# NicoNeureiter/sBayes

Hardware: AMD Instinct MI355X
Metric: log-likelihood evals/sec at 1000 sites x 200 feats x 10 states; 1/2/4/8-GPU chains (higher is better)
Workload: dtype f64; 1 GPU; headline synthetic 1000x200x10, K=5, C=2 (BASELINE.json configs[2]); chains_per_gpu=4096, kernel=packed, log_mode=product, parallelism=1 independent engine(s), one per GPU, no collectives

## Files before the change

### sbayes_amd/csrc/sbe_engine_internal.hip.h

```cpp
#pragma once
#include "sbe_kernels.hip.h"
#include "sbe_unit.hip.h"
#include "../../include/sbe_engine.h"
#include "../../include/sbe_engine_steps.h"
#include "../../include/sbe_engine_diag.h"
#include "sbe_host_helpers.h"
#include "sbe_pool.h"

#include <sched.h>
#include <algorithm>
#include <cstdarg>
#include <cstdio>
#include <cstring>
#include <chrono>
#include <atomic>
#include <condition_variable>
#include <functional>
#include <mutex>
#include <string>
#include <thread>
#include <vector>

using namespace sbe;

inline thread_local std::string g_last_error;

namespace {

struct Slot {
    std::vector<uint16_t> h_gid;
    std::vector<uint8_t> h_pid;
    std::vector<uint32_t> patterns;
    int n_tuples = 0;
    std::vector<uint8_t> h_tid;
    std::vector<uint32_t> h_toff;
    std::vector<uint16_t> h_tuple_g;
    std::vector<uint8_t> h_tuple_p;
    bool share_ok = false;
    bool groups_set = false, weights_set = false, source_set = false;
    std::vector<uint8_t> probs_set, counts_set;
    bool patterns_dirty = true;
    uint32_t gid_pending = 0;
    bool tables_follow = false;
    std::vector<int32_t> pat_cnt;
    std::vector<int32_t> tup_cnt;
    bool inc_ok = false;
    uint64_t group_epoch = 0;
    uint32_t overlap_mask = 0;
    int32_t ov_obj = -1, ov_g1 = 0, ov_g2 = 0, ov_comp = 0;
};

}

static int fuse_tables_default() {
    static const int on = [] { const char* v = getenv("SBE_FUSE_TABLES"); return (v && atoi(v) == 0) ? 0 : 1; }();
    return on;
}

struct sbe_engine : sbe::MixShape {
    int device = 0;
    hipStream_t stream = nullptr;
    hipEvent_t ev0 = nullptr, ev1 = nullptr;
    std::vector<hipEvent_t> ev_pool;
    bool ev_timing = false;  int ev_used = 0;
    int Fp = 0, rs_pitch = 0;
    uint64_t rng_seed = 0, rng_draw = 0;
    std::vector<int> G, goff;
    int64_t n_na = 0;
    int64_t hbm_bytes = 0;
    std::string last_error;
    char device_name[64] = {0};
    char last_kernel[128] = "none";

    sbe::MixTuning tune;
    int opt_log = SBE_LOG_PRODUCT;
    int opt_fuse_tables = fuse_tables_default();
    bool ws_lds_allowed[2] = {false, false};

    uint8_t* d_onehot = nullptr;
    uint8_t* d_state = nullptr;
    uint8_t* d_state_q = nullptr;
    float* d_probs_t = nullptr;
    double* d_wpat_t = nullptr;
    uint16_t* d_gid = nullptr;
    uint8_t* d_pid = nullptr;
    uint8_t* d_src = nullptr;
    int32_t* d_counts = nullptr;
    float* d_probs = nullptr;
    float* d_weights = nullptr;
    float* d_wpat = nullptr;
    uint32_t* d_patbits = nullptr;
    uint16_t* d_state_h = nullptr;
    double2* d_logtab = nullptr;
    uint32_t* d_toff = nullptr;
    uint32_t* d_rowoff = nullptr;
    std::vector<uint64_t> rowoff_epoch;
    uint32_t* d_rowoff_s = nullptr;  int rs_nq_max = 0;
    int32_t* d_rs_nq = nullptr;
    uint8_t* d_state_s = nullptr;
    std::vector<uint64_t> rowsort_epoch;
    std::atomic<uint64_t> epoch_counter{0};
    double2* d_logtab_fine = nullptr;
    unsigned* d_arrive = nullptr;
    uint8_t* d_xt = nullptr;
    int xt_NT = 0, xt_KBp = 0;  size_t xt_bytes = 0;
    uint8_t* d_tid = nullptr;
    uint16_t* d_tuple_g = nullptr;
    uint8_t* d_tuple_p = nullptr;
    double* d_conc = nullptr;
    double* d_unif = nullptr;
    double* d_lg_conc = nullptr; double* d_sum_a = nullptr; double* d_lg_sum_a = nullptr;
    double* d_unif_res = nullptr;  bool unif_set = false;
    int32_t* d_comp_of_group = nullptr;
    std::vector<uint8_t> conc_set;
    double* d_partials = nullptr;
    double* d_results = nullptr;
    double* h_results = nullptr;
    int* d_status = nullptr;
    int* h_status = nullptr;
    int* h_flag = nullptr;  int* d_flag = nullptr;
    unsigned long long* h_done = nullptr;  unsigned long long* d_done = nullptr;
    unsigned* d_ticket = nullptr;  unsigned long long done_seq = 0;
    static constexpr int kMaxChunks = 16;
    unsigned long long* h_chunk_flags = nullptr;  unsigned long long* d_chunk_flags = nullptr;
    unsigned* d_chunk_tickets = nullptr;  unsigned long long chunk_seq = 0;
    uint8_t* h_stream = nullptr;  uint8_t* d_stream = nullptr;  size_t stream_bytes = 0;
    uint8_t* d_changed = nullptr;
    uint32_t* d_step_stamp = nullptr;  uint32_t step_id = 0;
    float* d_step_pf = nullptr;
    double* d_step_pg = nullptr;
    struct StepLayout { size_t ids, pid, tid, toff, tuple_g, tuple_p, patbits, weights, row_of, subset, stale, objects, rows, total; } sl{};
    int step_max_rows = 0;
    uint8_t* h_step_payload = nullptr; uint8_t* d_step_payload = nullptr;
    uint8_t* h_io = nullptr; uint8_t* d_io = nullptr; size_t io_bytes = 0;
    uint8_t* h_step = nullptr;     uint8_t* d_step_host = nullptr;
    struct Lane { uint8_t* h_payload; uint8_t* d_payload; uint8_t* h_step; uint8_t* d_step_host; float* d_pf;
                  uint32_t* d_stamp; uint32_t step_id;
                  int* d_status; };
    std::vector<Lane> lanes;
    uint8_t* d_batch_meta = nullptr; size_t batch_meta_bytes = 0;
    uint8_t* h_batch_payload = nullptr; uint8_t* d_batch_payload = nullptr; size_t batch_payload_bytes = 0;
    std::vector<Slot> batch_cands;
    std::vector<std::vector<int32_t>> batch_moved;
    std::vector<int32_t> step_moved;
    struct Pool;
    Pool* pool = nullptr;
    uint8_t* d_scratch = nullptr;  size_t scratch_bytes = 0;
    uint8_t* h_pinned = nullptr;   size_t pinned_bytes = 0;
    uint8_t* h_arena = nullptr;    uint8_t* d_arena = nullptr;   size_t arena_bytes = 0, arena_off = 0;
    SetterJobs* batch = nullptr;
    int opt_step_form = 0;
    int opt_step_derive = 0;
    int opt_deferred = 0;
    bool status_pending = false;
    const char* pending_origin[2] = {nullptr, nullptr};
    int pending_calls = 0;
    std::vector<Slot> slots;
    struct SrcSync { uint64_t version = 1; int peer = -1; uint64_t peer_version = 0, own_version = 0; std::vector<int32_t> diff; };
    std::vector<SrcSync> src_sync;
    std::vector<SrcSync> ids_sync;

    int64_t probs_t_elems() const { return (int64_t)n_ftiles * tile_tab_elems(); }
    int64_t wpat_tile_elems() const { return (int64_t)Pmax * C * ft; }
    int64_t wpat_t_elems() const { return (int64_t)n_ftiles * wpat_tile_elems(); }
};

namespace {
inline void bump_src(sbe_engine* e, int slot) { ++e->src_sync[slot].version; }
inline void bump_ids(sbe_engine* e, int slot) { ++e->ids_sync[slot].version; }
}

struct sbe_engine::Pool : sbe_host::StepPool { using sbe_host::StepPool::StepPool; };

namespace {

int fail(sbe_engine* e, int code, const char* fmt, ...) {
    char buf[512];
    va_list ap;
    va_start(ap, fmt);
    vsnprintf(buf, sizeof buf, fmt, ap);
    va_end(ap);
    g_last_error = buf;
    if (e) e->last_error = buf;
    return code;
}

#define CHECK_ENGINE(e) \
    if (!(e)) return fail(nullptr, SBE_ERR_ARG, "null engine handle")
#define CHECK_SLOT(e, s) \
    if ((s) < 0 || (s) >= (e)->n_slots) return fail(e, SBE_ERR_ARG, "slot %d out of range [0,%d)", (s), (e)->n_slots)
#define CHECK_COMP(e, c) \
    if ((c) < 0 || (c) >= (e)->C) return fail(e, SBE_ERR_ARG, "component %d out of range [0,%d)", (c), (e)->C)
#define CHECK_PTR(e, p) \
    if (!(p)) return fail(e, SBE_ERR_ARG, "null pointer argument: %s", #p)

inline int round_up(int a, int b) { return (a + b - 1) / b * b; }

template <class T>
int dmalloc(sbe_engine* e, T** p, int64_t n) {
    const size_t bytes = std::max<int64_t>(n, 1) * sizeof(T);
    HIPCHK(e, hipMalloc((void**)p, bytes));
    e->hbm_bytes += (int64_t)bytes;
    return SBE_OK;
}

inline size_t al256(size_t v) { return (v + 255) / 256 * 256; }

int ensure_scratch(sbe_engine* e, size_t bytes) {
    if (bytes <= e->scratch_bytes) return SBE_OK;
    if (e->d_scratch) { HIPCHK(e, hipStreamSynchronize(e->stream)); HIPCHK(e, hipFree(e->d_scratch)); }
    e->scratch_bytes = bytes + bytes / 4 + 4096;
    HIPCHK(e, hipMalloc((void**)&e->d_scratch, e->scratch_bytes));
    return SBE_OK;
}

int ensure_io(sbe_engine* e, size_t bytes) {
    if (bytes <= e->io_bytes) return SBE_OK;
    if (e->h_io) { HIPCHK(e, hipStreamSynchronize(e->stream)); HIPCHK(e, hipHostFree(e->h_io)); e->h_io = nullptr; e->io_bytes = 0; }
    const size_t want = bytes + bytes / 4 + 4096;
    HIPCHK(e, hipHostMalloc((void**)&e->h_io, want, hipHostMallocMapped));
    HIPCHK(e, hipHostGetDevicePointer((void**)&e->d_io, e->h_io, 0));
    e->io_bytes = want;
    return SBE_OK;
}

int ensure_pinned(sbe_engine* e, size_t bytes) {
    if (bytes <= e->pinned_bytes) return SBE_OK;
    if (e->h_pinned) { HIPCHK(e, hipStreamSynchronize(e->stream)); HIPCHK(e, hipHostFree(e->h_pinned)); }
    e->pinned_bytes = bytes + bytes / 4 + 4096;
    HIPCHK(e, hipHostMalloc((void**)&e->h_pinned, e->pinned_bytes, hipHostMallocDefault));
    return SBE_OK;
}

int upload(sbe_engine* e, void* dst_dev, const void* src, size_t bytes);
int synced(sbe_engine* e);

int ensure_step_pool(sbe_engine* e);

int ensure_stream(sbe_engine* e, size_t bytes) {
    if (bytes <= e->stream_bytes) return SBE_OK;
    if (e->h_stream) { HIPCHK(e, hipStreamSynchronize(e->stream)); HIPCHK(e, hipHostFree(e->h_stream)); e->h_stream = nullptr; e->stream_bytes = 0; }
    const size_t want = bytes + bytes / 4 + 4096;
    HIPCHK(e, hipHostMalloc((void**)&e->h_stream, want, hipHostMallocMapped));
    HIPCHK(e, hipHostGetDevicePointer((void**)&e->d_stream, e->h_stream, 0));
    e->stream_bytes = want;
    return SBE_OK;
}

struct StreamPlan { ChunkSig sig; int n_chunks; size_t chunk_bytes; size_t bytes; unsigned grid; };

StreamPlan plan_stream(sbe_engine* e, unsigned n_blocks, size_t bytes_per_block, size_t bytes) {
    static const int max_chunks = [] { const char* v = getenv("SBE_STREAM_CHUNKS"); const int n = v ? atoi(v) : 0;
                                       return n >= 1 && n <= sbe_engine::kMaxChunks ? n : 8; }();
    unsigned per = std::max<unsigned>(1, (unsigned)div_up((int64_t)n_blocks, max_chunks));
    per = std::max<unsigned>(per, (unsigned)div_up((int64_t)128 << 10, (int64_t)bytes_per_block));
    const int n_chunks = (int)div_up((int64_t)n_blocks, (int64_t)per);
    static const bool ordered = [] { const char* v = getenv("SBE_STREAM_ORDERED"); return !(v && atoi(v) == 0); }();
    ChunkSig sig{e->d_chunk_tickets, e->d_chunk_flags, ++e->chunk_seq, per, n_blocks, (unsigned)n_chunks, 0};
    unsigned grid = n_blocks;
    if (ordered && n_chunks > 1) {
        sig.chunk_elems = (long long)per * (long long)(bytes_per_block / sizeof(double));
        grid = per;
    }
    return StreamPlan{sig, n_chunks, (size_t)per * bytes_per_block, bytes, grid};
}

template <class JobBegin, class JobEnd, class Work>
int stream_result(sbe_engine* e, const StreamPlan& plan, int n_jobs, JobBegin job_begin, JobEnd job_end, Work work) {
    static const bool single_thread = [] { const char* v = getenv("SBE_D2H_THREADS"); return v && atoi(v) == 1; }();
    if (!single_thread) { int rc = ensure_step_pool(e); if (rc) return rc; }
    std::atomic<bool> all_landed{false};
    hipError_t sync_err = hipSuccess;
    const volatile unsigned long long* flags = e->h_chunk_flags;
    const unsigned long long seq = plan.sig.seq;
    const size_t chunk_bytes = plan.chunk_bytes;
    const auto t_limit = std::chrono::steady_clock::now() + std::chrono::microseconds(2000 + (int64_t)(plan.bytes / 10000));
    unsigned spins = 0;
    sbe_host::run_as_chunks_land(
        single_thread ? nullptr : e->pool, n_jobs,
        [=](int j) { return (int)(job_begin(j) / chunk_bytes); },
        [=](int j) { return (int)((job_end(j) - 1) / chunk_bytes); },
        [&, flags, seq](int k) { return flags[k] == seq || all_landed.load(std::memory_order_acquire); },
        [&] {
            if ((++spins & 1023u) == 0 && !all_landed.load(std::memory_order_relaxed) && std::chrono::steady_clock::now() > t_limit) {
                sync_err = hipStreamSynchronize(e->stream);
                all_landed.store(true, std::memory_order_release);
            }
        },
        work);
    if (sync_err != hipSuccess) return fail(e, SBE_ERR_HIP, "hipStreamSynchronize (streamed result): %s", hipGetErrorString(sync_err));
    return SBE_OK;
}

int d2h(sbe_engine* e, void* dst, const void* src_dev, size_t bytes) {
    int rc = ensure_pinned(e, bytes);
    if (rc) return rc;
    HIPCHK(e, hipMemcpyAsync(e->h_pinned, src_dev, bytes, hipMemcpyDeviceToHost, e->stream));
    HIPCHK(e, hipStreamSynchronize(e->stream));
    static const bool single_copy = [] { const char* v = getenv("SBE_D2H_THREADS"); return v && atoi(v) == 1; }();
    if (bytes >= ((size_t)1 << 20) && !single_copy) {
        rc = ensure_step_pool(e);
        if (rc) return rc;
        constexpr size_t kJob = (size_t)64 << 10;
        uint8_t* out = (uint8_t*)dst;
        const uint8_t* stage = e->h_pinned;
        e->pool->run((int)((bytes + kJob - 1) / kJob),
                     [=](int j) { const size_t o = (size_t)j * kJob; memcpy(out + o, stage + o, std::min(kJob, bytes - o)); });
        return synced(e);
    }
    memcpy(dst, e->h_pinned, bytes);
    return synced(e);
}

constexpr size_t kMappedOutMax = (size_t)1 << 18;
int out_target(sbe_engine* e, size_t bytes, void* dev_fallback, void** target) {
    *target = dev_fallback;
    if (bytes > kMappedOutMax) return SBE_OK;
    int rc = ensure_io(e, bytes);
    if (rc) return rc;
    *target = e->d_io;
    return SBE_OK;
}
int wait_done(sbe_engine* e, const DoneSig& d);
DoneSig next_done(sbe_engine* e, unsigned n_blocks);
DoneSig out_done(sbe_engine* e, const void* target, unsigned n_blocks) {
    return target == (const void*)e->d_io ? next_done(e, n_blocks) : DoneSig{};
}
int out_fetch(sbe_engine* e, void* host_out, const void* target, size_t bytes, const DoneSig& done = DoneSig{}) {
    if (target != (const void*)e->d_io) return d2h(e, host_out, target, bytes);
    int rc = wait_done(e, done);
    if (rc) return rc;
    memcpy(host_out, e->h_io, bytes);
    return synced(e);
}

int h2d(sbe_engine* e, void* dst_dev, const void* src, size_t bytes) { return upload(e, dst_dev, src, bytes); }

int upload(sbe_engine* e, void* dst_dev, const void* src, size_t bytes) {
    if (bytes == 0) return SBE_OK;
    if (e->h_arena && bytes <= e->arena_bytes / 4) {
        const size_t need = (bytes + 63) / 64 * 64;
        if (e->arena_off + need > e->arena_bytes) {
            HIPCHK(e, hipStreamSynchronize(e->stream));
            e->arena_off = 0;
        }
        uint8_t* stage = e->h_arena + e->arena_off;
        e->arena_off += need;
        memcpy(stage, src, bytes);
        HIPCHK(e, hipMemcpyAsync(dst_dev, stage, bytes, hipMemcpyHostToDevice, e->stream));
        return SBE_OK;
    }
    HIPCHK(e, hipMemcpyAsync(dst_dev, src, bytes, hipMemcpyHostToDevice, e->stream));
    HIPCHK(e, hipStreamSynchronize(e->stream));
    return SBE_OK;
}

int stage(sbe_engine* e, const void* src, size_t bytes, void* dev_fallback, const void** out) {
    constexpr size_t kDirect = (size_t)64 << 10;
    *out = dev_fallback;
    if (bytes == 0) return SBE_OK;
    if (!e->d_arena || bytes > kDirect) return upload(e, dev_fallback, src, bytes);
    const size_t need = (bytes + 63) / 64 * 64;
    if (e->arena_off + need > e->arena_bytes) {
        HIPCHK(e, hipStreamSynchronize(e->stream));
        e->arena_off = 0;
    }
    memcpy(e->h_arena + e->arena_off, src, bytes);
    *out = e->d_arena + e->arena_off;
    e->arena_off += need;
    return SBE_OK;
}

struct UploadSeg { void* dst; const void* src; size_t bytes; };
struct FusedWeightPatterns { WeightPatternArgs args; int bits_seg; const float* new_weights; bool done; };
int upload_segments(sbe_engine* e, const UploadSeg* segs, int n, FusedWeightPatterns* wp = nullptr) {
    size_t total = 0, largest = 0;
    for (int i = 0; i < n; ++i) { total += (segs[i].bytes + 63) / 64 * 64; largest = std::max(largest, segs[i].bytes); }
    if (wp) wp->done = false;
    if (total == 0) return SBE_OK;
    if (!e->d_arena || n > 8 || total > ((size_t)64 << 10)) {
        for (int i = 0; i < n; ++i) { int rc = upload(e, segs[i].dst, segs[i].src, segs[i].bytes); if (rc) return rc; }
        return SBE_OK;
    }
    const size_t w_bytes = wp && wp->new_weights ? (size_t)wp->args.F * wp->args.C * sizeof(float) : 0;
    const bool fuse = wp && segs[wp->bits_seg].bytes > 0 && w_bytes <= ((size_t)64 << 10);
    const size_t reserve = total + (fuse ? (w_bytes + 63) / 64 * 64 : 0);
    if (e->arena_off + reserve > e->arena_bytes) {
        HIPCHK(e, hipStreamSynchronize(e->stream));
        e->arena_off = 0;
    }
    ScatterSegs sg{};
    size_t off = 0;
    for (int i = 0; i < n; ++i) {
        if (segs[i].bytes == 0) continue;
        memcpy(e->h_arena + e->arena_off + off, segs[i].src, segs[i].bytes);
        sg.dst[sg.n] = (uint8_t*)segs[i].dst; sg.off[sg.n] = (uint32_t)off; sg.bytes[sg.n] = (uint32_t)segs[i].bytes;
        ++sg.n;
        if (fuse && i == wp->bits_seg) wp->args.pattern_bits = (const uint32_t*)(e->d_arena + e->arena_off + off);
        off += (segs[i].bytes + 63) / 64 * 64;
    }
    const unsigned sx = (unsigned)std::min<size_t>(div_up((int64_t)largest, 1024), 16);
    unsigned wx = 0;
    if (fuse) {
        if (w_bytes) {
            memcpy(e->h_arena + e->arena_off + off, wp->new_weights, w_bytes);
            wp->args.weights = (const float*)(e->d_arena + e->arena_off + off);
        }
        wx = (unsigned)div_up((int64_t)wp->args.P * wp->args.F, 256);
        wp->done = true;
    }
    if (e->batch && e->batch->n_group_blocks == 0 && (fuse || !wp)) {
        SetterJobs& j = *e->batch;
        j.group_base = e->d_arena + e->arena_off; j.sg = sg; j.has_wp = fuse ? 1 : 0;
        if (fuse) j.wp = wp->args;
        j.group_gx = std::max(sx, wx); j.n_group_blocks = j.group_gx * (unsigned)(sg.n + (fuse ? 1 : 0));
    } else if (fuse) {
        k_scatter_weight_patterns<<<dim3(std::max(sx, wx), sg.n + 1), 256, 0, e->stream>>>(e->d_arena + e->arena_off, sg, wp->args);
    } else {
        k_scatter_bytes<<<dim3(sx, sg.n), 256, 0, e->stream>>>(e->d_arena + e->arena_off, sg);
    }
    HIPCHK(e, hipGetLastError());
    e->arena_off += reserve;
    return SBE_OK;
}

bool poll_done_enabled() {
    static const bool on = [] { const char* v = getenv("SBE_POLL_DONE"); return !(v && atoi(v) == 0); }();
    return on;
}
DoneSig next_done(sbe_engine* e, unsigned n_blocks) {
    if (!poll_done_enabled()) return DoneSig{};
    return DoneSig{e->d_ticket, e->d_done, ++e->done_seq, n_blocks};
}
int wait_done(sbe_engine* e, const DoneSig& d) {
    if (d.flag) {
        const volatile unsigned long long* f = e->h_done;
        const auto t0 = std::chrono::steady_clock::now();
        for (unsigned spins = 1;; ++spins) {
            if (*f == d.seq) { std::atomic_thread_fence(std::memory_order_acquire); return SBE_OK; }
            if ((spins & 127u) == 0u) sched_yield(); else __builtin_ia32_pause();
            if ((spins & 255u) == 0 && std::chrono::steady_clock::now() - t0 > std::chrono::microseconds(300)) break;
        }
    }
    HIPCHK(e, hipStreamSynchronize(e->stream));
    return SBE_OK;
}

bool status_raised(const sbe_engine* e) {
    const volatile int* f = e->h_flag;
    return (f[ST_BAD_NORMALIZE] | f[ST_MULTI_SOURCE]) != 0;
}

int fetch_and_clear_status(sbe_engine* e) {
    HIPCHK(e, hipMemcpyAsync(e->h_status, e->d_status, ST_FLAG_PTR * sizeof(int), hipMemcpyDeviceToHost, e->stream));
    HIPCHK(e, hipMemsetAsync(e->d_status + ST_BAD_NORMALIZE, 0, 2 * sizeof(int), e->stream));
    HIPCHK(e, hipStreamSynchronize(e->stream));
    e->h_flag[ST_BAD_NORMALIZE] = e->h_flag[ST_MULTI_SOURCE] = 0;
    return SBE_OK;
}

int report_status(sbe_engine* e, bool deferred = false) {
    const int n_calls = e->pending_calls;
    const char* origin[2] = {e->pending_origin[0], e->pending_origin[1]};
    e->pending_calls = 0;
    e->pending_origin[0] = e->pending_origin[1] = nullptr;
    if (!status_raised(e)) return SBE_OK;
    int rc = fetch_and_clear_status(e);
    if (rc) return rc;
    const int bad_norm = e->h_status[ST_BAD_NORMALIZE], multi_src = e->h_status[ST_MULTI_SOURCE];
    e->h_status[ST_BAD_NORMALIZE] = e->h_status[ST_MULTI_SOURCE] = 0;
    char where[200] = "";
    const char* who = origin[bad_norm ? 0 : 1];
    if (deferred && who)
        snprintf(where, sizeof where, " [deferred data check: raised by %s (%d state-setting call%s queued since the last report), "
                 "reported by the first call that waited for the device]", who, n_calls, n_calls == 1 ? "" : "s");
    if (bad_norm)
        return fail(e, SBE_ERR_DATA, "normalize: %d rows have a non-positive sum (sbayes/util.py:1006 assert)%s", bad_norm, where);
    return fail(e, SBE_ERR_DATA, "source is not one-hot over components in %d observations%s", multi_src, where);
}

int check_after(sbe_engine* e, int word, const char* who = __builtin_FUNCTION()) {
    if (e->opt_deferred) {
        e->status_pending = true;
        e->pending_origin[word == ST_BAD_NORMALIZE ? 0 : 1] = who;
        ++e->pending_calls;
        return SBE_OK;
    }
    HIPCHK(e, hipStreamSynchronize(e->stream));
    e->status_pending = false;
    return report_status(e);
}

int synced(sbe_engine* e) {
    if (!e->status_pending) return SBE_OK;
    e->status_pending = false;
    return report_status(e, true);
}

int read_status(sbe_engine* e) {
    HIPCHK(e, hipStreamSynchronize(e->stream));
    int rc = synced(e);
    if (rc) return rc;
    e->h_status[ST_BAD_NORMALIZE] = e->h_status[ST_MULTI_SOURCE] = 0;
    if (status_raised(e)) return fetch_and_clear_status(e);
    return SBE_OK;
}

int take_status(sbe_engine* e) {
    e->h_status[ST_BAD_NORMALIZE] = e->h_status[ST_MULTI_SOURCE] = 0;
    if (status_raised(e)) return fetch_and_clear_status(e);
    return SBE_OK;
}

int clear_status_word(sbe_engine* e, int word) {
    if (e->status_pending) return SBE_OK;
    if (!e->h_flag[word]) return SBE_OK;
    HIPCHK(e, hipStreamSynchronize(e->stream));
    HIPCHK(e, hipMemsetAsync(e->d_status + word, 0, sizeof(int), e->stream));
    e->h_flag[word] = 0;
    return SBE_OK;
}

void derive_patterns(sbe_engine* e, Slot& s) {
    const int N = e->N, C = e->C;
    static thread_local std::vector<uint8_t> bits;
    bits.resize(N);
    bool seen[256] = {false};
    s.pat_cnt.assign(256, 0);
    for (int n = 0; n < N; ++n) {
        uint32_t b = 0;
        for (int c = 0; c < C; ++c)
            if (s.h_gid[(size_t)c * N + n] != kNoGroup) b |= 1u << c;
        bits[n] = (uint8_t)b;
        seen[b] = true;
        ++s.pat_cnt[b];
    }
    auto key = [C](uint32_t b) {
        uint32_t k = 0;
        for (int c = 0; c < C; ++c) k |= ((b >> c) & 1u) << (C - 1 - c);
        return k;
    };
    std::vector<uint32_t> uniq;
    for (uint32_t b = 0; b < 256; ++b) if (seen[b]) uniq.push_back(b);
    std::sort(uniq.begin(), uniq.end(), [&](uint32_t a, uint32_t b) { return key(a) < key(b); });
    uint8_t index_of[256] = {0};
    for (size_t i = 0; i < uniq.size(); ++i) index_of[uniq[i]] = (uint8_t)i;
    s.patterns = uniq;
    s.h_pid.resize(N);
    for (int n = 0; n < N; ++n) s.h_pid[n] = index_of[bits[n]];
}

bool tuples_share_operands(const sbe_engine* e, const Slot& s) {
    if (e->C != 2 || s.n_tuples == 0 || (int)s.h_tuple_p.size() != kMaxTuples) return false;
    int first = -1, pb = -1;
    for (int t = 0; t < kMaxTuples; ++t) {
        const int pat = s.h_tuple_p[t];
        if (pat == 0xFF) continue;
        if (first < 0) { first = t; continue; }
        if (s.h_tuple_g[(size_t)t * kMaxComponents + 1] != s.h_tuple_g[(size_t)first * kMaxComponents + 1]) return false;
        const int pa = s.h_tuple_p[first];
        if (pat != pa) {
            if (pb < 0) pb = pat;
            else if (pat != pb) return false;
        }
    }
    return first >= 0;
}

void derive_tuples(sbe_engine* e, Slot& s) {
    const int N = e->N, C = e->C;
    s.h_tid.assign(e->Np, 0);
    s.h_toff.assign(e->Np, 0);
    s.h_tuple_g.assign((size_t)kMaxTuples * kMaxComponents, (uint16_t)e->Gtot);
    s.h_tuple_p.assign(kMaxTuples, 0xFF);
    uint16_t tuples[kMaxTuples][kMaxComponents];
    int n_tup = 0;
    bool ok = true;
    s.tup_cnt.assign(kMaxTuples, 0);
    uint64_t packed[kMaxTuples];
    int last = 0;
    for (int n = 0; n < N && ok; ++n) {
        uint16_t key[kMaxComponents];
        for (int c = 0; c < C; ++c) key[c] = s.h_gid[(size_t)c * N + n];
        int t = 0;
        if (C <= 4) {
            uint64_t k64 = 0;
            for (int c = 0; c < C; ++c) k64 |= (uint64_t)key[c] << (16 * c);
            if (n_tup && packed[last] == k64) t = last;
            else for (; t < n_tup; ++t) if (packed[t] == k64) break;
            if (t == n_tup && n_tup < kMaxTuples) packed[n_tup] = k64;
        } else {
            for (; t < n_tup; ++t) if (memcmp(tuples[t], key, (size_t)C * sizeof(uint16_t)) == 0) break;
        }
        last = t;
        if (t == n_tup) {
            if (n_tup == kMaxTuples) { ok = false; break; }
            memcpy(tuples[n_tup++], key, (size_t)C * sizeof(uint16_t));
            for (int c = 0; c < C; ++c) s.h_tuple_g[(size_t)t * kMaxComponents + c] = key[c] == kNoGroup ? (uint16_t)e->Gtot : key[c];
            s.h_tuple_p[t] = s.h_pid[n];
        }
        s.h_tid[n] = (uint8_t)t;
        s.h_toff[n] = (uint32_t)t * (uint32_t)(e->S + 1) * 512u;
        ++s.tup_cnt[t];
    }
    s.n_tuples = ok ? n_tup : 0;
    s.inc_ok = ok;
    s.share_ok = tuples_share_operands(e, s);
}

bool update_patterns_and_tuples(sbe_engine* e, Slot& s, const int32_t* moved, const uint16_t* old_gid0, int n_moved) {
    const int N = e->N, C = e->C;
    if (!s.inc_ok || s.n_tuples == 0 || (int)s.pat_cnt.size() != 256 || (int)s.tup_cnt.size() != kMaxTuples) return false;
    auto bits_rest = [&](int n) { uint32_t b = 0; for (int c = 1; c < C; ++c) if (s.h_gid[(size_t)c * N + n] != kNoGroup) b |= 1u << c; return b; };
    for (int i = 0; i < n_moved; ++i) {
        const int n = moved[i];
        const uint32_t rest = bits_rest(n);
        const uint32_t b0 = rest | (old_gid0[i] != kNoGroup ? 1u : 0u), b1 = rest | (s.h_gid[n] != kNoGroup ? 1u : 0u);
        if (b0 == b1) continue;
        --s.pat_cnt[b0]; ++s.pat_cnt[b1];
    }
    {
        size_t live = 0;
        for (uint32_t b = 0; b < 256; ++b) if (s.pat_cnt[b] > 0) ++live;
        bool same = live == s.patterns.size();
        for (size_t i = 0; same && i < s.patterns.size(); ++i) same = s.pat_cnt[s.patterns[i]] > 0;
        if (!same) return false;
    }
    uint8_t rank_of[256];
    for (size_t i = 0; i < s.patterns.size(); ++i) rank_of[s.patterns[i]] = (uint8_t)i;
    for (int i = 0; i < n_moved; ++i) {
        const int n = moved[i];
        const uint32_t b1 = bits_rest(n) | (s.h_gid[n] != kNoGroup ? 1u : 0u);
        s.h_pid[n] = rank_of[b1];
        uint16_t key[kMaxComponents];
        for (int c = 0; c < C; ++c) { const uint16_t g = s.h_gid[(size_t)c * N + n]; key[c] = g == kNoGroup ? (uint16_t)e->Gtot : g; }
        const int t0 = s.h_tid[n];
        int t1 = -1, free_t = -1;
        for (int t = 0; t < s.n_tuples; ++t) {
            if (s.tup_cnt[t] == 0) { if (free_t < 0 && t != t0) free_t = t; continue; }
            if (memcmp(&s.h_tuple_g[(size_t)t * kMaxComponents], key, (size_t)C * sizeof(uint16_t)) == 0) { t1 = t; break; }
        }
        if (t1 < 0) {
            if (s.tup_cnt[t0] == 1) t1 = t0;
            else if (free_t >= 0) t1 = free_t;
            else if (s.n_tuples < kMaxTuples) t1 = s.n_tuples++;
            else return false;
            for (int c = 0; c < C; ++c) s.h_tuple_g[(size_t)t1 * kMaxComponents + c] = key[c];
        }
        if (t1 != t0) {
            if (--s.tup_cnt[t0] == 0) s.h_tuple_p[t0] = 0xFF;
            ++s.tup_cnt[t1];
        }
        s.h_tuple_p[t1] = s.h_pid[n];
        s.h_tid[n] = (uint8_t)t1;
        s.h_toff[n] = (uint32_t)t1 * (uint32_t)(e->S + 1) * 512u;
    }
    while (s.n_tuples > 0 && s.tup_cnt[s.n_tuples - 1] == 0) --s.n_tuples;
    s.share_ok = tuples_share_operands(e, s);
    for (int t = 0; t < s.n_tuples; ++t)
        if (s.tup_cnt[t] == 0) return false;
    return s.n_tuples > 0;
}

int upload_patterns_and_weights(sbe_engine* e, int slot, const float* new_weights = nullptr, bool eager = false) {
    Slot& s = e->slots[slot];
    float* d_w = e->d_weights + (int64_t)slot * e->F * e->C;
    auto gid_seg = [&](int c) { return UploadSeg{e->d_gid + ((int64_t)slot * e->C + c) * e->Np, s.h_gid.data() + (size_t)c * e->N, (size_t)e->N * sizeof(uint16_t)}; };
    bool patterns_done = false;
    if (s.patterns_dirty) {
        const bool follow = s.tables_follow;
        s.tables_follow = false;
        if (!follow) derive_patterns(e, s);
        if ((int)s.patterns.size() > e->Pmax) {
            if (eager) {
                for (int c = 0; c < e->C; ++c)
                    if (s.gid_pending >> c & 1u) { const UploadSeg g = gid_seg(c); int rc = upload(e, g.dst, g.src, g.bytes); if (rc) return rc; }
                s.gid_pending = 0;
                return SBE_OK;
            }
            return fail(e, SBE_ERR_ARG, "%zu distinct has_components patterns exceed capacity %d",
                        s.patterns.size(), e->Pmax);
        }
        if (!follow) derive_tuples(e, s);
        UploadSeg segs[6 + kMaxComponents] = {{e->d_pid + (int64_t)slot * e->Np, s.h_pid.data(), (size_t)e->N},
                                              {e->d_patbits + (int64_t)slot * e->Pmax, s.patterns.data(), s.patterns.size() * sizeof(uint32_t)}};
        int n_segs = 2;
        if (s.n_tuples) {
            segs[n_segs++] = {e->d_tid + (int64_t)slot * e->Np, s.h_tid.data(), (size_t)e->Np};
            segs[n_segs++] = {e->d_toff + (int64_t)slot * e->Np, s.h_toff.data(), (size_t)e->Np * sizeof(uint32_t)};
            segs[n_segs++] = {e->d_tuple_g + (int64_t)slot * kMaxTuples * kMaxComponents, s.h_tuple_g.data(), s.h_tuple_g.size() * sizeof(uint16_t)};
            segs[n_segs++] = {e->d_tuple_p + (int64_t)slot * kMaxTuples, s.h_tuple_p.data(), s.h_tuple_p.size()};
        }
        for (int c = 0; c < e->C; ++c) if (s.gid_pending >> c & 1u) segs[n_segs++] = gid_seg(c);
        const int P = (int)s.patterns.size();
        FusedWeightPatterns wp{};
        const bool want_wp = (s.weights_set || new_weights) && P > 0;
        if (want_wp) {
            wp.args = WeightPatternArgs{d_w, nullptr, e->d_wpat + (int64_t)slot * e->Pmax * e->F * e->C, new_weights ? d_w : nullptr,
                                        e->d_wpat_t + (int64_t)slot * e->wpat_t_elems(), P, e->F, e->C, e->Pmax, e->ft};
            wp.bits_seg = 1;
            wp.new_weights = new_weights;
        }
        { int _urc = upload_segments(e, segs, n_segs, want_wp ? &wp : nullptr); if (_urc) return _urc; }
        patterns_done = wp.done;
        s.patterns_dirty = false;
        s.gid_pending = 0;
    }
    const int P = (int)s.patterns.size();
    if (new_weights && P == 0) {
        int rc = upload(e, d_w, new_weights, (size_t)e->F * e->C * sizeof(float));
        if (rc) return rc;
    }
    if ((s.weights_set || new_weights) && P > 0 && !patterns_done) {
        const void* w_in = d_w;
        if (new_weights) { int rc = stage(e, new_weights, (size_t)e->F * e->C * sizeof(float), d_w, &w_in); if (rc) return rc; }
        k_weight_patterns<<<div_up((int64_t)P * e->F, 256), 256, 0, e->stream>>>(
            (const float*)w_in, e->d_patbits + (int64_t)slot * e->Pmax, e->d_wpat + (int64_t)slot * e->Pmax * e->F * e->C, P, e->F, e->C,
            w_in != d_w ? d_w : nullptr, e->d_wpat_t + (int64_t)slot * e->wpat_t_elems(), e->Pmax, e->ft);
        HIPCHK(e, hipGetLastError());
    }
    return SBE_OK;
}

int retile_probs(sbe_engine* e, int slot, int component) {
    const int g_lo = e->goff[component], g_hi = g_lo + e->G[component];
    const int64_t n = (int64_t)(g_hi - g_lo) * e->S * e->ft * e->n_ftiles;
    if (n == 0) return SBE_OK;
    k_tile_probs<<<div_up(n, 256), 256, 0, e->stream>>>(
        e->d_probs + (int64_t)slot * e->table_elems(), e->d_probs_t + (int64_t)slot * e->probs_t_elems(),
        g_lo, g_hi, e->Gtot, e->F, e->S, e->ft, e->n_ftiles);
    HIPCHK(e, hipGetLastError());
    return SBE_OK;
}

int check_slot_ready(sbe_engine* e, int slot, bool need_weights) {
    Slot& s = e->slots[slot];
    if (!s.groups_set) return fail(e, SBE_ERR_STATE, "slot %d: groups not set for every component", slot);
    for (int c = 0; c < e->C; ++c)
        if (!s.probs_set[c]) return fail(e, SBE_ERR_STATE, "slot %d: probability tables of component %d not set", slot, c);
    if (need_weights && !s.weights_set) return fail(e, SBE_ERR_STATE, "slot %d: weights not set", slot);
    return SBE_OK;
}

int check_collapsed_ready(sbe_engine* e, int slot, int c_lo, int c_hi) {
    Slot& s = e->slots[slot];
    for (int c = c_lo; c < c_hi; ++c) {
        if (e->G[c] == 0) continue;
        if (!s.counts_set[c]) return fail(e, SBE_ERR_STATE, "slot %d: counts of component %d not set", slot, c);
        if (!e->conc_set[c]) return fail(e, SBE_ERR_STATE, "concentration of component %d not set", c);
    }
    return SBE_OK;
}

constexpr size_t kCollapsedLdsMax = (size_t)96 << 10;
inline size_t collapsed_lds_bytes(const sbe_engine* e) { return (size_t)e->F * e->S * sizeof(double) + (size_t)e->F * sizeof(float); }

template <class TC>
int enqueue_dcl(sbe_engine* e, const TC* counts, const double* conc, int conc_per_group, int g_lo, int G, float* d_pf, double* d_pg) {
    k_dcl<TC><<<div_up((int64_t)G * e->F, 256), 256, 0, e->stream>>>(counts, conc, d_pf, g_lo, g_lo + G, e->F, e->S, conc_per_group);
    HIPCHK(e, hipGetLastError());
    if (!d_pg) return SBE_OK;
    k_group_sum_f32<<<div_up((int64_t)G * 8, 64), 64, 0, e->stream>>>(d_pf, d_pg, G, e->F);
    HIPCHK(e, hipGetLastError());
    return SBE_OK;
}

int ensure_xt(sbe_engine* e) {
    if (e->d_xt) return SBE_OK;
    const int NT = div_up((int64_t)e->F * e->S, 32), KBp = round_up(div_up(e->N, kTupleMfmaKBlockObjects), 4);
    const size_t bytes = ((size_t)(NT + 1) * KBp + 4) * 1024;
    uint8_t* xt = nullptr;
    double2* logtab = nullptr;
    auto build = [&]() -> int {
        HIPCHK(e, hipMalloc((void**)&xt, bytes));
        HIPCHK(e, hipMemsetAsync(xt, 0, bytes, e->stream));
        std::vector<double> tab(2 * kFineLogEntries);
        fine_log_table(tab.data());
        HIPCHK(e, hipMalloc((void**)&logtab, tab.size() * sizeof(double) + column_tables_bytes(NT)));
        HIPCHK(e, hipMemcpy(logtab, tab.data(), tab.size() * sizeof(double), hipMemcpyHostToDevice));
        launch_column_tables(e->d_state, reinterpret_cast<int32_t*>(logtab + kFineLogEntries), e->N, e->F, e->S, e->Fp, NT, e->stream);
        HIPCHK(e, hipGetLastError());
        launch_xt_frags(e->d_state, xt, e->N, e->F, e->S, e->Fp, NT, KBp, e->stream);
        HIPCHK(e, hipGetLastError());
        return SBE_OK;
    };
    const int rc = build();
    if (rc) {
        (void)hipStreamSynchronize(e->stream);
        if (xt) (void)hipFree(xt);
        if (logtab) (void)hipFree(logtab);
        return rc;
    }
    e->d_xt = xt; e->d_logtab_fine = logtab;
    e->hbm_bytes += (int64_t)bytes;
    e->xt_NT = NT; e->xt_KBp = KBp; e->xt_bytes = bytes;
    return SBE_OK;
}

int next_timing_events(sbe_engine* e, hipEvent_t* ev_a, hipEvent_t* ev_b) {
    *ev_a = *ev_b = nullptr;
    if (!e->ev_timing) return SBE_OK;
    while ((int)e->ev_pool.size() < 2 * (e->ev_used + 1)) {
        hipEvent_t ev;
        HIPCHK(e, hipEventCreate(&ev));
        e->ev_pool.push_back(ev);
    }
    *ev_a = e->ev_pool[2 * e->ev_used]; *ev_b = e->ev_pool[2 * e->ev_used + 1];
    ++e->ev_used;
    return SBE_OK;
}

struct MixCall {
    int first_slot = 0, n = 1;
    const int32_t* slots = nullptr;  const int32_t* d_slots = nullptr;
    const StepFinish* fin = nullptr;
    const StepFinish* d_fins = nullptr;
    DoneSig* done_out = nullptr;
    hipEvent_t ev_a = nullptr, ev_b = nullptr;
    int slot_at(int i) const { return slots ? (int)slots[i] : first_slot + i; }
};

MixFacts mixture_facts(const sbe_engine* e, const MixCall& c) {
    MixFacts f;
    f.n = c.n;
    f.share_ok = true;
    bool tuples = true;
    for (int i = 0; i < c.n; ++i) {
        const Slot& s = e->slots[c.slot_at(i)];
        f.P = std::max<int>(f.P, (int)s.patterns.size());
        f.KT = std::max(f.KT, s.n_tuples);
        tuples &= s.n_tuples != 0;
        f.share_ok &= s.share_ok;
    }
    if (!tuples) f.KT = 0;
    f.epilogue = c.fin || c.d_fins;
    f.waits = c.done_out != nullptr;
    return f;
}

MixTuning launch_tuning(const sbe_engine* e, const MixFacts& f) {
    MixTuning t = e->tune;
    if (considers_tuple_mfma(*e, t, f))
        if (const char* env = getenv("SBE_MFMA_SPLIT")) t.mfma_split = atoi(env);
    t.shared_allowed = tuple_mfma_shared();
    static const bool in_kernel_opt = !(getenv("SBE_REDUCE_IN_KERNEL") && atoi(getenv("SBE_REDUCE_IN_KERNEL")) == 0);
    t.in_kernel_allowed = in_kernel_opt;
    return t;
}

int prepare_mixture(sbe_engine* e, const MixPlan& pl, const MixCall& c) {
    if (pl.form == MixForm::TupleMfma) return ensure_xt(e);
    if (pl.form != MixForm::Rows && pl.form != MixForm::RowsSorted) return SBE_OK;
    const bool sorted = pl.form == MixForm::RowsSorted;
    const int rft = pl.ft;
    if (sorted && !e->d_rowoff_s) {
        e->rs_nq_max = pl.rs_nq_max;
        int rc = dmalloc(e, &e->d_rowoff_s, (int64_t)e->n_slots * e->rs_nq_max * (e->C + 1) * 4); if (rc) return rc;
        rc = dmalloc(e, &e->d_rs_nq, e->n_slots); if (rc) return rc;
        rc = dmalloc(e, &e->d_state_s, (int64_t)(e->N + 1) * e->Fq); if (rc) return rc;
        launch_state_s(e->d_state, e->d_state_s, e->N, e->F, e->Fp, e->Fq, e->S, e->stream);
        HIPCHK(e, hipGetLastError());
        e->rowsort_epoch.assign(e->n_slots, ~0ull);
    }
    std::vector<uint64_t>& built = sorted ? e->rowsort_epoch : e->rowoff_epoch;
    bool stale = false;
    for (int i = 0; i < c.n; ++i) stale |= built[c.slot_at(i)] != e->slots[c.slot_at(i)].group_epoch;
    if (!stale) return SBE_OK;
    if (sorted) {
        launch_rowsort(e->d_gid, e->d_pid, e->d_rowoff_s, e->d_rs_nq, (int64_t)e->C * e->Np, e->Np,
                       (int64_t)e->rs_nq_max * (e->C + 1) * 4, c.first_slot, c.d_slots, c.n, e->N, e->Np, e->C, e->Gtot, e->Pmax,
                       (uint32_t)((e->S + 1) * rft * 4), (uint32_t)e->Fq, 4 * (kWave / rft), e->stream);
    } else {
        const int cells = (e->C + 1) * e->Np;
        k_rowoff<<<dim3(div_up(cells, 256), c.n), 256, 0, e->stream>>>(
            e->d_gid, e->d_pid, e->d_rowoff, (int64_t)e->C * e->Np, e->Np, (int64_t)cells, c.first_slot, c.d_slots, e->N, e->Np,
            e->C, e->Gtot, (uint32_t)((e->S + 1) * rft * 4), (uint32_t)(((e->C + 1) / 2) * rft * 16));
    }
    HIPCHK(e, hipGetLastError());
    for (int i = 0; i < c.n; ++i) built[c.slot_at(i)] = e->slots[c.slot_at(i)].group_epoch;
    return SBE_OK;
}

int launch_mfma_form(sbe_engine* e, const MixCall& c, const MixPlan& pl, const DoneSig& done) {
    MfmaMixParams p{};
    p.F = e->F; p.S = e->S; p.FS = e->F * e->S; p.Gtot = e->Gtot; p.Np = e->Np;
    p.NT = e->xt_NT; p.KBp = e->xt_KBp; p.KT = pl.KT; p.SL = pl.SL; p.shared = pl.shared ? 1 : 0;
    p.n_batch = c.n; p.n_split = pl.n_split; p.nt_per_split = pl.nt_per_split;
    p.first_slot = c.first_slot; p.slot_list = c.d_slots;
    p.xt = e->d_xt; p.xt_bytes = (uint32_t)e->xt_bytes;
    p.tid = e->d_tid; p.tid_stride = e->Np;
    p.tuple_g = e->d_tuple_g; p.tuple_g_stride = (int64_t)kMaxTuples * kMaxComponents;
    p.tuple_p = e->d_tuple_p; p.tuple_p_stride = kMaxTuples;
    p.probs = e->d_probs; p.probs_stride = e->table_elems();
    p.probs_ones_off = (uint32_t)((int64_t)e->n_slots * e->table_elems() * 4);
    p.probs_bytes = p.probs_ones_off + (uint32_t)(e->F * e->S * 4);
    p.wpat = e->d_wpat; p.wpat_stride = (int64_t)e->Pmax * e->F * e->C;
    p.wpat_ones_off = (uint32_t)((int64_t)e->n_slots * e->Pmax * e->F * e->C * 4);
    p.wpat_bytes = p.wpat_ones_off + (uint32_t)(e->F * e->C * 4);
    p.logtab = e->d_logtab_fine;
    p.colcount = reinterpret_cast<const int32_t*>(e->d_logtab_fine + kFineLogEntries);
    p.colfeat = p.colcount + (size_t)(e->xt_NT + 1) * 32;
    p.tile_prefix = p.colcount + (size_t)(e->xt_NT + 1) * 64;
    p.partials = e->d_partials; p.partials_stride = e->partials_stride;
    if (pl.in_kernel) { p.results = e->d_results; p.arrive = e->d_arrive; p.done = done; }
    if (!launch_tuple_mfma(e->C, p, dim3(pl.grid_x), pl.lds_bytes, e->stream))
        return fail(e, SBE_ERR_STATE, "k_mixture_tuple_mfma was built with static LDS: its log table must sit at LDS address 0 "
                                      "(toolchain change; rebuild without static __shared__ in sbe_mixture_mfma.hip)");
    return SBE_OK;
}

void launch_tile_form(sbe_engine* e, const MixCall& c, const MixPlan& pl, const DoneSig& done) {
    Mix2Params p{};
    p.N = e->N; p.NQ = e->NQ; p.Np = e->Np; p.F = e->F; p.Fq = e->Fq; p.S = e->S; p.C = e->C;
    p.Gtot = e->Gtot; p.P = pl.P; p.n_ftiles = pl.n_ftiles; p.quads_per_chunk = pl.quads_per_chunk;
    p.state_q = reinterpret_cast<const uint32_t*>(e->d_state_q);
    p.onehot = e->d_onehot; p.rs_pitch = e->rs_pitch;
    p.gid = e->d_gid; p.gid_stride = (int64_t)e->C * e->Np;
    p.pid = e->d_pid; p.pid_stride = e->Np;
    p.probs_t = e->d_probs_t; p.probs_t_stride = e->probs_t_elems();
    p.wpat_t = e->d_wpat_t; p.wpat_t_stride = e->wpat_t_elems(); p.wpat_tile_stride = (int)e->wpat_tile_elems();
    p.partials = e->d_partials; p.partials_stride = e->partials_stride; p.first_slot = c.first_slot;
    if (pl.in_kernel) { p.results = e->d_results; p.arrive = e->d_arrive; p.done = done; }
    p.slot_list = c.d_slots;
    p.n_work = pl.n_partials; p.n_batch = c.n;
    p.slot_groups = pl.slot_groups; p.slots_per_group = pl.slots_per_group;
    p.tid = e->d_tid; p.tid_stride = e->Np;
    p.state_h = reinterpret_cast<const uint2*>(e->d_state_h);
    p.toff = e->d_toff; p.toff_stride = e->Np;
    p.logtab = e->d_logtab;
    p.ragged_w = pl.ragged_w; p.gen_slots = pl.gen_slots;
    p.tuple_g = e->d_tuple_g; p.tuple_g_stride = (int64_t)kMaxTuples * kMaxComponents;
    p.tuple_p = e->d_tuple_p; p.tuple_p_stride = kMaxTuples;
    p.combo_w_off = pl.combo_w_off; p.combo_tab_off = pl.combo_tab_off;
    p.KT = pl.KT;
    p.eft = e->ft;
    p.wpat = e->d_wpat; p.wpat_stride = (int64_t)e->Pmax * e->F * e->C;
    p.rowoff = e->d_rowoff; p.rowoff_stride = (int64_t)(e->C + 1) * e->Np;
    p.rowoff_s = e->d_rowoff_s; p.rowoff_s_stride = (int64_t)e->rs_nq_max * (e->C + 1) * 4;
    p.rs_nq = e->d_rs_nq; p.state_s = e->d_state_s; p.state_s_pitch = e->Fq;
    {
        constexpr int split[4] = {450, 270, 170, 110};
        p.rows_cum[0] = 0;
        for (int i = 0; i < 4; ++i) p.rows_cum[i + 1] = p.rows_cum[i] + split[i];
    }
    const int mode = e->opt_log == SBE_LOG_PRODUCT ? LOG_PRODUCT : LOG_PER_OBS;
    const dim3 grid(pl.grid_x, 1);
    switch (pl.form) {
        case MixForm::Tuple64: launch_tuple64(e->C, p, grid, pl.lds_bytes, e->stream); break;
        case MixForm::Combo: launch_combo(pl.onehot, pl.ft, e->C, p, grid, pl.lds_bytes, e->stream); break;
        case MixForm::Rows: case MixForm::RowsSorted:
            launch_rows(mode, pl.ft, e->C, p, grid, pl.lds_bytes, e->stream, pl.form == MixForm::RowsSorted); break;
        case MixForm::OnehotV2: launch_oh2(mode, pl.ft, e->C, p, grid, pl.lds_bytes, e->stream, e->direct); break;
        default: launch_v2(mode, pl.ft, e->C, p, grid, pl.lds_bytes, e->stream, e->direct); break;
    }
}

int launch_mixture(sbe_engine* e, const MixCall& c) {
    const MixFacts facts = mixture_facts(e, c);
    const MixPlan pl = plan_mixture(*e, launch_tuning(e, facts), facts);
    if (pl.err) return fail(e, pl.err, "%s", pl.msg);
    int rc = prepare_mixture(e, pl, c);
    if (rc) return rc;
    if (c.ev_a) HIPCHK(e, hipEventRecord(c.ev_a, e->stream));
    DoneSig done_k{};
    if (pl.in_kernel && c.done_out) *c.done_out = done_k = next_done(e, pl.done_blocks);
    plan_name(pl, *e, e->last_kernel, sizeof e->last_kernel);
    if (pl.form == MixForm::TupleMfma) { rc = launch_mfma_form(e, c, pl, done_k); if (rc) return rc; }
    else launch_tile_form(e, c, pl, done_k);
    if (c.ev_b) HIPCHK(e, hipEventRecord(c.ev_b, e->stream));
    HIPCHK(e, hipGetLastError());
    if (pl.in_kernel) return SBE_OK;
    const unsigned n_red = (unsigned)(c.n + (c.d_fins ? c.n : (c.fin ? 1 : 0)));
    const DoneSig done = c.done_out ? next_done(e, n_red) : DoneSig{};
    if (c.done_out) *c.done_out = done;
    k_reduce_partials<<<n_red, kBlock, 0, e->stream>>>(e->d_partials, e->partials_stride, pl.n_partials,
                                                       e->d_results, c.first_slot, c.n, c.fin ? *c.fin : StepFinish{},
                                                       c.d_slots, c.d_fins, done);
    HIPCHK(e, hipGetLastError());
    return SBE_OK;
}

int enqueue_mixture(sbe_engine* e, int first_slot, int n, DoneSig* done_out = nullptr) {
    for (int s = first_slot; s < first_slot + n; ++s) {
        int rc = check_slot_ready(e, s, true);
        if (rc) return rc;
        if (e->slots[s].patterns_dirty) { rc = upload_patterns_and_weights(e, s); if (rc) return rc; }
    }
    MixCall c;
    c.first_slot = first_slot; c.n = n; c.done_out = done_out;
    { int rc = next_timing_events(e, &c.ev_a, &c.ev_b); if (rc) return rc; }
    return launch_mixture(e, c);
}

int counts_launch(sbe_engine* e, int slot_a, int sign_a, int slot_b, int sign_b, const int32_t* d_objects,
                  int n_listed, int dst_slot, bool single_chunk, uint8_t* d_changed) {
    CountSide A{e->d_gid + (int64_t)slot_a * e->C * e->Np, e->d_src + (int64_t)slot_a * e->N * e->Fp, sign_a};
    CountSide B{e->d_gid + (int64_t)slot_b * e->C * e->Np, e->d_src + (int64_t)slot_b * e->N * e->Fp, sign_b};
    int32_t* counts = e->d_counts + (int64_t)dst_slot * e->table_elems();
    int ft = 32;
    auto lds_for = [&](int t) { return (size_t)e->Gtot * t * e->S * sizeof(int32_t); };
    while (ft > 4 && lds_for(ft) > 96 * 1024) ft >>= 1;
    if (lds_for(ft) > 150 * 1024) {
        k_counts_global<<<div_up((int64_t)n_listed * e->F, 256), 256, 0, e->stream>>>(
            e->d_state, A, B, d_objects, n_listed, e->Np, e->F, e->S, e->C, e->Fp, counts, d_changed);
        HIPCHK(e, hipGetLastError());
        return SBE_OK;
    }
    const int n_ftiles = div_up(e->F, ft);
    int chunks = 1;
    if (!single_chunk) chunks = std::max(1, std::min(div_up(n_listed, 32), div_up(2 * e->compute_units, n_ftiles)));
    const int opc = div_up(n_listed, chunks);
    chunks = div_up(n_listed, opc);
    k_counts<<<dim3(n_ftiles, chunks), kBlock, lds_for(ft), e->stream>>>(
        e->d_state, A, B, d_objects, n_listed, opc, e->Np, e->F, e->S, e->C, e->Fp, e->Gtot, ft, counts, d_changed);
    HIPCHK(e, hipGetLastError());
    return SBE_OK;
}

}

namespace {

int set_gid_common(sbe_engine* e, int slot, int component, const std::vector<uint16_t>& ids) {
    Slot& s = e->slots[slot];
    s.tables_follow = false;
    static const bool follow_on = [] { const char* v = getenv("SBE_FOLLOW_TABLES"); return !(v && atoi(v) == 0); }();
    if (follow_on && component == 0 && !s.patterns_dirty && s.inc_ok) {
        static thread_local std::vector<int32_t> moved;
        static thread_local std::vector<uint16_t> old_ids;
        moved.clear(); old_ids.clear();
        const int N = e->N;
        for (int n = 0; n < N; ++n)
            if (ids[n] != s.h_gid[n]) { moved.push_back(n); old_ids.push_back(s.h_gid[n]); }
        std::copy(ids.begin(), ids.end(), s.h_gid.begin());
        s.tables_follow = (int)moved.size() * 8 <= N &&
                          update_patterns_and_tuples(e, s, moved.data(), old_ids.data(), (int)moved.size());
    } else {
        std::copy(ids.begin(), ids.end(), s.h_gid.begin() + (size_t)component * e->N);
    }
    s.gid_pending |= 1u << component;
    s.patterns_dirty = true;
    s.group_epoch = ++e->epoch_counter;
    bump_ids(e, slot);
    s.groups_set = true;
    return upload_patterns_and_weights(e, slot, nullptr, true);
}

void overlap_message(char* buf, size_t len, int n, int g1, int g2, int component) {
    snprintf(buf, len, "object %d is in groups %d and %d of component %d: resident slot state keeps one group id per object "
             "and component (counts.py:28-30 would count it in both); counts of overlapping groups come from the caller or "
             "the stateless sbe_effect_counts", n, g1, g2, component);
}

struct OverlapNote { bool found = false; int obj = -1, g1 = 0, g2 = 0; };

bool matrix_to_ids(const uint8_t* groups, int G, int N, int off, int component, uint16_t* ids, char* msg, size_t msg_len,
                   OverlapNote* note = nullptr) {
    std::fill(ids, ids + N, kNoGroup);
    auto hit = [&](int n, int g) -> bool {
        if (ids[n] != kNoGroup) {
            if (!note) { overlap_message(msg, msg_len, n, (int)ids[n] - off, g, component); return false; }
            if (!note->found) { note->found = true; note->obj = n; note->g1 = (int)ids[n] - off; note->g2 = g; }
        }
        ids[n] = (uint16_t)(off + g);
        return true;
    };
    for (int g = 0; g < G; ++g) {
        const uint8_t* row = groups + (size_t)g * N;
        int n = 0;
        for (; n + 8 <= N; n += 8) {
            uint64_t w8;
            memcpy(&w8, row + n, 8);
            if (!w8) continue;
            for (int k = 0; k < 8; ++k) if (row[n + k] && !hit(n + k, g)) return false;
        }
        for (; n < N; ++n) if (row[n] && !hit(n, g)) return false;
    }
    return true;
}

int reject_overlap(sbe_engine* e, int slot, const char* what) {
    const Slot& s = e->slots[slot];
    if (!s.overlap_mask) return SBE_OK;
    char msg[320];
    overlap_message(msg, sizeof msg, s.ov_obj, s.ov_g1, s.ov_g2, s.ov_comp);
    return fail(e, SBE_ERR_DATA, "%s (slot %d, %s)", msg, slot, what);
}


int enqueue_lh_exact(sbe_engine* e, int slot, const char* who) {
    Slot& s = e->slots[slot];
    if (!s.groups_set || !s.source_set || !s.weights_set) return fail(e, SBE_ERR_STATE, "slot %d: groups / source / weights not set", slot);
    { int orc = reject_overlap(e, slot, who); if (orc) return orc; }
    for (int c = 0; c < e->C; ++c)
        if (!s.counts_set[c] || !e->conc_set[c]) return fail(e, SBE_ERR_STATE, "slot %d: counts / concentration of component %d not set", slot, c);
    HIPCHK(e, hipSetDevice(e->device));
    int rc = SBE_OK;
    if (s.patterns_dirty) { rc = upload_patterns_and_weights(e, slot); if (rc) return rc; }
    const int64_t n = (int64_t)e->N * e->F;
    rc = ensure_scratch(e, n * sizeof(double));
    if (rc) return rc;
    rc = clear_status_word(e, ST_BAD_NORMALIZE);
    if (rc) return rc;
    k_lh_exact<<<div_up(n, 256), 256, 0, e->stream>>>(
        e->d_state, e->d_src + (int64_t)slot * e->N * e->Fp, e->d_gid + (int64_t)slot * e->C * e->Np,
        e->d_counts + (int64_t)slot * e->table_elems(), e->d_conc, (double*)e->d_scratch, e->N, e->Np, e->F, e->S, e->C,
        e->Fp, e->d_status, e->d_wpat + (int64_t)slot * e->Pmax * e->F * e->C, e->d_pid + (int64_t)slot * e->Np);
    HIPCHK(e, hipGetLastError());
    return SBE_OK;
}

int lh_exact_report(sbe_engine* e) {
    int rc = read_status(e);
    if (rc) return rc;
    if (e->h_status[ST_BAD_NORMALIZE]) return fail(e, SBE_ERR_DATA, "normalize: non-positive row sum in leave-one-out tables (sbayes/util.py:1006 assert)");
    return SBE_OK;
}

int sync_and_report(sbe_engine* e, const DoneSig& done = DoneSig{}) {
    { int rc = wait_done(e, done); if (rc) return rc; }
    const bool was_pending = e->status_pending;
    e->status_pending = false;
    return report_status(e, was_pending);
}

int check_objects(sbe_engine* e, const int32_t* objects, int n) {
    for (int i = 0; i < n; ++i)
        if (objects[i] < 0 || objects[i] >= e->N) return fail(e, SBE_ERR_ARG, "object index %d out of range", objects[i]);
    return SBE_OK;
}

SrcPostArgs src_post_args(sbe_engine* e, int slot, const int32_t* d_objects, int n_sub, double temperature, double prior_temperature,
                          int from_prior) {
    const double inv_t = 1.0 / temperature, inv_tp = 1.0 / prior_temperature;
    return SrcPostArgs{e->d_state, e->d_gid + (int64_t)slot * e->C * e->Np, e->d_pid + (int64_t)slot * e->Np,
                       e->d_probs + (int64_t)slot * e->table_elems(), e->d_wpat + (int64_t)slot * e->Pmax * e->F * e->C,
                       d_objects, n_sub, e->Np, e->F, e->S, e->C, e->Fp, inv_t, (float)inv_tp, inv_t != 1.0, inv_tp != 1.0,
                       from_prior != 0};
}

ClusterOpArgs cluster_op_args(sbe_engine* e, int slot, double prior_temperature, const int32_t* d_objects, int n, double* d_out) {
    const double inv = 1.0 / prior_temperature;
    return ClusterOpArgs{e->d_state, e->d_gid + (int64_t)slot * e->C * e->Np, e->d_pid + (int64_t)slot * e->Np,
                         e->d_weights + (int64_t)slot * e->F * e->C, e->d_patbits + (int64_t)slot * e->Pmax, (float)inv,
                         inv != 1.0 ? 1 : 0, d_objects, n, d_out, reinterpret_cast<const f64x2_t*>(e->d_logtab),
                         e->Np, e->F, e->S, e->C, e->Fp};
}

constexpr size_t kGuFusedLdsMax = (size_t)96 << 10;

}

namespace {
int ensure_step_pool(sbe_engine* e) {
    if (!e->pool) {
        int nt = 7;
        if (const char* env = getenv("SBE_STEP_THREADS")) nt = std::max(0, atoi(env) - 1);
        int cpus = (int)std::thread::hardware_concurrency();
        cpu_set_t set;
        if (sched_getaffinity(0, sizeof set, &set) == 0) cpus = std::min(cpus > 0 ? cpus : CPU_COUNT(&set), CPU_COUNT(&set));
        if (FILE* f = fopen("/sys/fs/cgroup/cpu.max", "r")) {
            long long quota = 0, period = 0;
            if (fscanf(f, "%lld %lld", &quota, &period) == 2 && quota > 0 && period > 0)
                cpus = std::min<int>(cpus, (int)std::max<long long>(1, quota / period));
            fclose(f);
        }
        int local_world = 1;
        if (const char* env = getenv("LOCAL_WORLD_SIZE")) local_world = std::max(1, atoi(env));
        nt = std::min<int>(nt, std::max(0, cpus / local_world - 1));
        e->pool = new sbe_engine::Pool(nt);
    }
    return SBE_OK;
}
}
```

### sbayes_amd/csrc/sbe_engine_steps.hip

```cpp
#include "sbe_engine_internal.hip.h"

extern "C" {

namespace {
struct CoreInputs {
    const void* ids_new = nullptr;
    const void* pid = nullptr; const void* tid = nullptr; const void* toff = nullptr;
    const void* tuple_g = nullptr; const void* tuple_p = nullptr; const void* patbits = nullptr;
    const void* weights = nullptr;
    const int16_t* row_of = nullptr;
    const uint8_t* rows = nullptr; const int32_t* objects = nullptr; int n_changed = 0;
    const uint8_t* src_new = nullptr;
    const int32_t* subset = nullptr; int n_subset = 0;
    int P = 1;
    bool full_src_copy = true; const int32_t* stale = nullptr; int n_stale = 0;
    const int32_t* patch_n = nullptr; const uint16_t* patch_gid = nullptr; const uint8_t* patch_pid = nullptr;
    const uint8_t* patch_tid = nullptr; int n_patch = -1;
    const int16_t* sub_row = nullptr; const uint16_t* sub_gid0 = nullptr;
};

sbe_engine::Lane lane0(sbe_engine* e) {
    return sbe_engine::Lane{e->h_step_payload, e->d_step_payload, e->h_step, e->d_step_host, e->d_step_pf, e->d_step_stamp, e->step_id,
                            e->d_status};
}

int build_step_core(sbe_engine* e, sbe_engine::Lane& lane, int cur_slot, int cand_slot, const CoreInputs& in,
                    StepCore& a, size_t& lds_out, int& n_blocks_out, int n_chains = 1) {
    const int N = e->N, Np = e->Np, F = e->F, C = e->C;
    const bool regroup = in.ids_new != nullptr;
    a = StepCore{};
    uint32_t run = 0;
    auto seg = [&](auto* base, int64_t elems, const void* other_src) {
        const int64_t bytes = elems * (int64_t)sizeof(*base);
        a.cs.src[a.cs.n] = other_src ? reinterpret_cast<const uint32_t*>(other_src)
                                     : reinterpret_cast<const uint32_t*>(base + (int64_t)cur_slot * elems);
        a.cs.dst[a.cs.n] = reinterpret_cast<uint32_t*>(base + (int64_t)cand_slot * elems);
        run += (uint32_t)(bytes / 4);
        a.cs.end[a.cs.n++] = run;
    };
    uint16_t* g_cur = e->d_gid + (int64_t)cur_slot * C * Np;
    const bool delta = in.n_patch >= 0;
    if (!delta) {
        uint16_t* g_cand = e->d_gid + (int64_t)cand_slot * C * Np;
        a.cs.src[a.cs.n] = reinterpret_cast<const uint32_t*>(regroup ? in.ids_new : (const void*)g_cur);
        a.cs.dst[a.cs.n] = reinterpret_cast<uint32_t*>(g_cand);
        run += (uint32_t)(Np * 2 / 4); a.cs.end[a.cs.n++] = run;
        if (C > 1) {
            a.cs.src[a.cs.n] = reinterpret_cast<const uint32_t*>(g_cur + Np);
            a.cs.dst[a.cs.n] = reinterpret_cast<uint32_t*>(g_cand + Np);
            run += (uint32_t)((int64_t)(C - 1) * Np * 2 / 4); a.cs.end[a.cs.n++] = run;
        }
        seg(e->d_pid, (int64_t)Np, regroup ? in.pid : nullptr);
        seg(e->d_tid, (int64_t)Np, regroup ? in.tid : nullptr);
        seg(e->d_toff, (int64_t)Np, regroup ? in.toff : nullptr);
    }
    a.n_patch = in.n_patch; a.patch_n = in.patch_n; a.patch_gid = in.patch_gid; a.patch_pid = in.patch_pid; a.patch_tid = in.patch_tid;
    a.gid_dst = e->d_gid + (int64_t)cand_slot * C * Np; a.pid_dst = e->d_pid + (int64_t)cand_slot * Np;
    a.tid_dst = e->d_tid + (int64_t)cand_slot * Np; a.toff_dst = e->d_toff + (int64_t)cand_slot * Np;
    a.toff_mul = (uint32_t)(e->S + 1) * 512u;
    a.sub_row = in.sub_row; a.sub_gid0 = in.sub_gid0;
    seg(e->d_tuple_g, (int64_t)kMaxTuples * kMaxComponents, in.tuple_g);
    seg(e->d_tuple_p, (int64_t)kMaxTuples, in.tuple_p);
    seg(e->d_patbits, (int64_t)e->Pmax, in.patbits);
    seg(e->d_weights, (int64_t)F * C, in.weights);
    a.src_seg = a.cs.n;
    if (in.full_src_copy) seg(e->d_src, (int64_t)N * e->Fp, nullptr);
    a.stale = in.stale; a.n_stale = in.full_src_copy ? 0 : in.n_stale;
    a.src_cur_rows = e->d_src + (int64_t)cur_slot * N * e->Fp;
    a.row_of = in.row_of;
    a.rows = in.rows;
    a.objects = in.objects;
    a.src_dst = e->d_src + (int64_t)cand_slot * N * e->Fp;
    a.n_changed = in.n_changed; a.F = F; a.C = C; a.Fp = e->Fp; a.status = lane.d_status;
    a.state = e->d_state; a.gid_cur = g_cur;
    a.ids_new = reinterpret_cast<const uint16_t*>(in.ids_new);
    a.src_cur = e->d_src + (int64_t)cur_slot * N * e->Fp;
    a.src_new = in.src_new;
    a.subset = in.subset; a.n_subset = in.n_subset;
    a.counts_cur = e->d_counts + (int64_t)cur_slot * e->table_elems();
    a.counts_new = e->d_counts + (int64_t)cand_slot * e->table_elems();
    a.conc = e->d_conc; a.lg_conc = e->d_lg_conc; a.sum_a = e->d_sum_a; a.lg_sum_a = e->d_lg_sum_a;
    a.probs = e->d_probs + (int64_t)cand_slot * e->table_elems();
    a.probs_t = e->d_probs_t + (int64_t)cand_slot * e->probs_t_elems();
    a.per_feature = lane.d_pf;
    if (++lane.step_id == 0) {
        HIPCHK(e, hipMemsetAsync(lane.d_stamp, 0, e->Gtot * sizeof(uint32_t), e->stream));
        lane.step_id = 1;
    }
    a.stamp = lane.d_stamp; a.step_id = lane.step_id;
    a.Np = Np; a.S = e->S; a.Gtot = e->Gtot; a.ft = e->ft;
    a.ftc = (int)std::max<int64_t>(1, std::min<int64_t>(8, 2048 / ((int64_t)e->Gtot * e->S)));
    a.n_tile_blocks = div_up(F, a.ftc);
    a.weights = in.weights ? reinterpret_cast<const float*>(in.weights) : e->d_weights + (int64_t)cur_slot * F * C;
    a.pattern_bits = in.patbits ? reinterpret_cast<const uint32_t*>(in.patbits) : e->d_patbits + (int64_t)cur_slot * e->Pmax;
    a.wpat = e->d_wpat + (int64_t)cand_slot * e->Pmax * F * C;
    a.wpat_t = e->d_wpat_t + (int64_t)cand_slot * e->wpat_t_elems();
    a.P = in.P; a.Pmax = e->Pmax; a.n_weight_blocks = div_up((int64_t)in.P * F, kBlock);
    const int64_t E = (int64_t)e->Gtot * a.ftc * e->S, R = (int64_t)e->Gtot * a.ftc;
    const size_t lds = (size_t)((E * 4 + 15) / 16 * 16) + (size_t)(2 * E + R) * sizeof(double);
    a.n_copy_blocks = std::max(1, (int)std::min<int64_t>(div_up(run, 1024), std::max(4, 2 * e->compute_units / std::max(1, n_chains))));
    lds_out = lds;
    n_blocks_out = a.n_tile_blocks + a.n_weight_blocks + a.n_copy_blocks;
    return SBE_OK;
}

int launch_step_core(sbe_engine* e, int cur_slot, int cand_slot, const CoreInputs& in) {
    sbe_engine::Lane lane = lane0(e);
    StepCore a; size_t lds = 0; int n_blocks = 0;
    int rc = build_step_core(e, lane, cur_slot, cand_slot, in, a, lds, n_blocks);
    e->step_id = lane.step_id;
    if (rc) return rc;
    k_step_core<<<n_blocks, kBlock, lds, e->stream>>>(a);
    HIPCHK(e, hipGetLastError());
    return SBE_OK;
}

inline size_t step_host_lq_offset(const sbe_engine* e) {
    return ((size_t)e->Gtot * sizeof(double) + ST_WORDS * sizeof(int) + (size_t)e->Gtot + 7) / 8 * 8;
}

StepFinish make_step_finish_lane(sbe_engine* e, const sbe_engine::Lane& lane) {
    StepFinish fin{};
    fin.per_feature = lane.d_pf;
    fin.group_out = reinterpret_cast<double*>(lane.d_step_host);
    fin.status = lane.d_status;
    fin.status_out = reinterpret_cast<int*>(lane.d_step_host + (size_t)e->Gtot * sizeof(double));
    fin.changed = nullptr; fin.stamp = lane.d_stamp; fin.step_id = lane.step_id;
    fin.changed_out = lane.d_step_host + (size_t)e->Gtot * sizeof(double) + ST_WORDS * sizeof(int);
    fin.Gtot = e->Gtot; fin.F = e->F;
    return fin;
}
StepFinish make_step_finish(sbe_engine* e) { return make_step_finish_lane(e, lane0(e)); }

int read_step_results_lane(sbe_engine* e, const uint8_t* h_step, int cand_slot, double* group_logliks_out, double* mixture_out,
                      uint8_t* changed_groups_out, const char* bad_norm_what, int* d_status = nullptr, int chain = -1) {
    const int* hst = reinterpret_cast<const int*>(h_step + (size_t)e->Gtot * sizeof(double));
    if (hst[ST_BAD_NORMALIZE] || hst[ST_MULTI_SOURCE]) {
        const int bad_norm = hst[ST_BAD_NORMALIZE], multi_src = hst[ST_MULTI_SOURCE];
        (void)hipMemsetAsync((d_status ? d_status : e->d_status) + ST_BAD_NORMALIZE, 0, 2 * sizeof(int), e->stream);
        if (!d_status || d_status == e->d_status) e->h_flag[ST_BAD_NORMALIZE] = e->h_flag[ST_MULTI_SOURCE] = 0;
        char who[32] = "";
        if (chain >= 0) snprintf(who, sizeof who, "chain %d: ", chain);
        if (bad_norm) return fail(e, SBE_ERR_DATA, "%snormalize: %d %s have a non-positive sum (sbayes/util.py:1006 assert)", who, bad_norm, bad_norm_what);
        return fail(e, SBE_ERR_DATA, "%ssource is not one-hot over components in %d observations", who, multi_src);
    }
    memcpy(group_logliks_out, h_step, (size_t)e->Gtot * sizeof(double));
    if (changed_groups_out) memcpy(changed_groups_out, h_step + (size_t)e->Gtot * sizeof(double) + ST_WORDS * sizeof(int), (size_t)e->Gtot);
    *mixture_out = e->h_results[cand_slot];
    return SBE_OK;
}
int read_step_results(sbe_engine* e, int cand_slot, double* group_logliks_out, double* mixture_out,
                      uint8_t* changed_groups_out, const char* bad_norm_what) {
    return read_step_results_lane(e, e->h_step, cand_slot, group_logliks_out, mixture_out, changed_groups_out, bad_norm_what);
}

}

static int step_lean(sbe_engine* e, int cur_slot, int cand_slot, const uint8_t* clusters, const int32_t* changed_objects,
                     int n_changed, const uint8_t* source_rows, const float* weights, double* group_logliks_out,
                     double* mixture_out, uint8_t* changed_groups_out);
static int step_general(sbe_engine* e, int cur_slot, int cand_slot, const uint8_t* clusters, const int32_t* changed_objects,
                        int n_changed, const uint8_t* source_rows, const float* weights, double* group_logliks_out,
                        double* mixture_out, uint8_t* changed_groups_out);

int sbe_step(sbe_engine* e, int cur_slot, int cand_slot, const uint8_t* clusters, const int32_t* changed_objects,
             int n_changed, const uint8_t* source_rows, const float* weights, double* group_logliks_out,
             double* mixture_out, uint8_t* changed_groups_out) {
    CHECK_ENGINE(e); CHECK_SLOT(e, cur_slot); CHECK_SLOT(e, cand_slot);
    CHECK_PTR(e, group_logliks_out); CHECK_PTR(e, mixture_out);
    if (cur_slot == cand_slot) return fail(e, SBE_ERR_ARG, "current and candidate slot must differ");
    if (n_changed < 0 || (n_changed > 0 && (!changed_objects || !source_rows)))
        return fail(e, SBE_ERR_ARG, "changed_objects / source_rows missing for n_changed=%d", n_changed);
    Slot& cur = e->slots[cur_slot];
    if (!cur.groups_set || !cur.source_set || !cur.weights_set) return fail(e, SBE_ERR_STATE, "slot %d: groups / source / weights not set", cur_slot);
    { int orc = reject_overlap(e, cur_slot, "one-call step"); if (orc) return orc; }
    for (int c = 0; c < e->C; ++c)
        if (!cur.counts_set[c] || !e->conc_set[c]) return fail(e, SBE_ERR_STATE, "slot %d: counts / concentration of component %d not set", cur_slot, c);
    for (int i = 0; i < n_changed; ++i)
        if (changed_objects[i] < 0 || changed_objects[i] >= e->N) return fail(e, SBE_ERR_ARG, "object index %d out of range", changed_objects[i]);
    HIPCHK(e, hipSetDevice(e->device));
    static const bool force_general = getenv("SBE_STEP_GENERAL") && atoi(getenv("SBE_STEP_GENERAL")) == 1;
    if (!force_general && e->opt_step_form == 0 && n_changed <= e->step_max_rows && !cur.patterns_dirty &&
        (int64_t)e->Gtot * e->S * 28 <= 60 * 1024)
        return step_lean(e, cur_slot, cand_slot, clusters, changed_objects, n_changed, source_rows, weights,
                         group_logliks_out, mixture_out, changed_groups_out);
    return step_general(e, cur_slot, cand_slot, clusters, changed_objects, n_changed, source_rows, weights,
                        group_logliks_out, mixture_out, changed_groups_out);
}

static int prepare_step(sbe_engine* e, const sbe_engine::Lane& lane, int cur_slot, int cand_slot, const uint8_t* clusters,
                        const int32_t* changed_objects, int n_changed, const uint8_t* source_rows, const float* weights,
                        Slot& cd, CoreInputs& in, std::string* err, std::vector<int32_t>* moved_out = nullptr) {
    const int N = e->N, Np = e->Np, F = e->F, C = e->C;
    const Slot& cur = e->slots[cur_slot];
    cd = cur;
    static thread_local std::vector<int32_t> mv;
    static thread_local std::vector<uint16_t> mv_old;
    mv.clear(); mv_old.clear();
    bool full_derive = false;
    const bool regroup = clusters != nullptr;
    if (regroup) {
        const int K = e->G[0];
        uint16_t* ids = cd.h_gid.data();
        {
            char msg[320];
            if (!matrix_to_ids(clusters, K, N, 0, 0, ids, msg, sizeof msg)) { *err = msg; return SBE_ERR_DATA; }
        }
        const uint16_t* old_ids = cur.h_gid.data();
        for (int n = 0; n < N; ++n) if (ids[n] != old_ids[n]) { mv.push_back(n); mv_old.push_back(old_ids[n]); }
        if (e->opt_step_derive == 1 || (int)mv.size() > N / 8 ||
            !update_patterns_and_tuples(e, cd, mv.data(), mv_old.data(), (int)mv.size())) {
            full_derive = true;
            derive_patterns(e, cd);
            if ((int)cd.patterns.size() > e->Pmax) {
                char buf[160];
                snprintf(buf, sizeof buf, "%zu distinct has_components patterns exceed capacity %d", cd.patterns.size(), e->Pmax);
                *err = buf;
                return SBE_ERR_ARG;
            }
            derive_tuples(e, cd);
        }
        cd.patterns_dirty = false;
        cd.group_epoch = ++e->epoch_counter;
    }
    if (moved_out) {
        *moved_out = mv;
        if (full_derive) moved_out->assign(1, -1);
    }
    const auto& L = e->sl;
    uint8_t* st = lane.h_payload;
    int n_subset = 0;
    {
        int32_t* sub = reinterpret_cast<int32_t*>(st + L.subset);
        if (n_changed == 0) { memcpy(sub, mv.data(), mv.size() * sizeof(int32_t)); n_subset = (int)mv.size(); }
        else {
            static thread_local std::vector<int32_t> ch;
            ch.assign(changed_objects, changed_objects + n_changed);
            std::sort(ch.begin(), ch.end());
            ch.erase(std::unique(ch.begin(), ch.end()), ch.end());
            n_subset = (int)(std::set_union(mv.begin(), mv.end(), ch.begin(), ch.end(), sub) - sub);
        }
    }
    if (regroup) {
        memcpy(st + L.ids, cd.h_gid.data(), (size_t)N * 2);
        if (Np > N) memset(st + L.ids + (size_t)N * 2, 0xFF, (size_t)(Np - N) * 2);
        memset(st + L.pid, 0, Np); memcpy(st + L.pid, cd.h_pid.data(), N);
        memcpy(st + L.tid, cd.h_tid.data(), Np);
        memcpy(st + L.toff, cd.h_toff.data(), (size_t)Np * 4);
        memcpy(st + L.tuple_g, cd.h_tuple_g.data(), (size_t)kMaxTuples * kMaxComponents * 2);
        memcpy(st + L.tuple_p, cd.h_tuple_p.data(), kMaxTuples);
        memset(st + L.patbits, 0, (size_t)e->Pmax * 4);
        memcpy(st + L.patbits, cd.patterns.data(), cd.patterns.size() * 4);
    }
    if (weights) memcpy(st + L.weights, weights, (size_t)F * C * 4);
    if (n_changed > 0) {
        int16_t* row_of = reinterpret_cast<int16_t*>(st + L.row_of);
        std::fill(row_of, row_of + Np, (int16_t)-1);
        for (int i = 0; i < n_changed; ++i) row_of[changed_objects[i]] = (int16_t)i;
        memcpy(st + L.objects, changed_objects, (size_t)n_changed * 4);
        memcpy(st + L.rows, source_rows, (size_t)n_changed * F * C);
    }
    const uint8_t* pl = lane.d_payload;
    in = CoreInputs{};
    if (regroup) {
        in.ids_new = pl + L.ids; in.pid = pl + L.pid; in.tid = pl + L.tid; in.toff = pl + L.toff;
        in.tuple_g = pl + L.tuple_g; in.tuple_p = pl + L.tuple_p; in.patbits = pl + L.patbits;
    }
    if (weights) in.weights = pl + L.weights;
    if (n_changed > 0) {
        in.row_of = reinterpret_cast<const int16_t*>(pl + L.row_of);
        in.rows = pl + L.rows;
        in.objects = reinterpret_cast<const int32_t*>(pl + L.objects);
        in.n_changed = n_changed;
    }
    in.subset = reinterpret_cast<const int32_t*>(pl + L.subset); in.n_subset = n_subset;
    in.P = (int)cd.patterns.size();
    {
        const sbe_engine::SrcSync& rec = e->src_sync[cand_slot];
        const sbe_engine::SrcSync& cs = e->src_sync[cur_slot];
        if (rec.peer == cur_slot && rec.peer_version == cs.version && rec.own_version == rec.version &&
            (int)rec.diff.size() <= e->step_max_rows) {
            int32_t* stale = reinterpret_cast<int32_t*>(st + L.stale);
            const int16_t* row_of = n_changed > 0 ? reinterpret_cast<const int16_t*>(st + L.row_of) : nullptr;
            int ns = 0;
            for (int32_t n : rec.diff)
                if (!row_of || row_of[n] < 0) stale[ns++] = n;
            in.full_src_copy = false;
            in.stale = reinterpret_cast<const int32_t*>(pl + L.stale);
            in.n_stale = ns;
        }
    }
    std::fill(cd.probs_set.begin(), cd.probs_set.end(), 1);
    cd.weights_set = true;
    return SBE_OK;
}

static void commit_ids_sync(sbe_engine* e, int cur_slot, int cand_slot, const std::vector<int32_t>& moved) {
    sbe_engine::SrcSync& rc = e->ids_sync[cand_slot];
    sbe_engine::SrcSync& cu = e->ids_sync[cur_slot];
    ++rc.version;
    if (moved.size() == 1 && moved[0] < 0) {
        rc.peer = cu.peer = -1;
        rc.diff.clear(); cu.diff.clear();
        return;
    }
    rc.peer = cur_slot; rc.peer_version = cu.version; rc.own_version = rc.version; rc.diff = moved;
    cu.peer = cand_slot; cu.peer_version = rc.version; cu.own_version = cu.version; cu.diff = moved;
}

static void commit_src_sync(sbe_engine* e, int cur_slot, int cand_slot, const int32_t* changed_objects, int n_changed) {
    sbe_engine::SrcSync& rc = e->src_sync[cand_slot];
    sbe_engine::SrcSync& cu = e->src_sync[cur_slot];
    ++rc.version;
    rc.peer = cur_slot; rc.peer_version = cu.version; rc.own_version = rc.version;
    rc.diff.assign(changed_objects, changed_objects + n_changed);
    cu.peer = cand_slot; cu.peer_version = rc.version; cu.own_version = cu.version;
    cu.diff = rc.diff;
}

static int step_lean(sbe_engine* e, int cur_slot, int cand_slot, const uint8_t* clusters, const int32_t* changed_objects,
                     int n_changed, const uint8_t* source_rows, const float* weights, double* group_logliks_out,
                     double* mixture_out, uint8_t* changed_groups_out) {
    if (e->status_pending) {
        HIPCHK(e, hipStreamSynchronize(e->stream));
        int rc = synced(e);
        if (rc) return rc;
    }
    static const bool timing = getenv("SBE_STEP_TIMING") && atoi(getenv("SBE_STEP_TIMING")) == 1;
    static double t_acc[3] = {0, 0, 0};
    static int t_n = 0;
    const auto t0 = std::chrono::steady_clock::now();
    Slot cd;
    CoreInputs in;
    {
        std::string err;
        int rc = prepare_step(e, lane0(e), cur_slot, cand_slot, clusters, changed_objects, n_changed, source_rows, weights, cd, in, &err,
                              &e->step_moved);
        if (rc) return fail(e, rc, "%s", err.c_str());
    }
    const auto t1 = std::chrono::steady_clock::now();
    int rc = launch_step_core(e, cur_slot, cand_slot, in);
    if (rc) return rc;
    commit_src_sync(e, cur_slot, cand_slot, changed_objects, n_changed);
    commit_ids_sync(e, cur_slot, cand_slot, e->step_moved);
    e->slots[cand_slot] = cd;
    StepFinish fin = make_step_finish(e);
    DoneSig done;
    MixCall mix;
    mix.first_slot = cand_slot; mix.fin = &fin; mix.done_out = &done;
    rc = launch_mixture(e, mix);
    if (rc) return rc;
    const auto t2 = std::chrono::steady_clock::now();
    rc = wait_done(e, done);
    if (rc) return rc;
    if (timing) {
        const auto t3 = std::chrono::steady_clock::now();
        t_acc[0] += std::chrono::duration<double, std::micro>(t1 - t0).count();
        t_acc[1] += std::chrono::duration<double, std::micro>(t2 - t1).count();
        t_acc[2] += std::chrono::duration<double, std::micro>(t3 - t2).count();
        if (++t_n == 2000) {
            fprintf(stderr, "[sbe_step] host prepare %.1f us, enqueue %.1f us, wait %.1f us per step\n", t_acc[0] / t_n, t_acc[1] / t_n, t_acc[2] / t_n);
            t_acc[0] = t_acc[1] = t_acc[2] = 0; t_n = 0;
        }
    }
    return read_step_results(e, cand_slot, group_logliks_out, mixture_out, changed_groups_out, "rows");
}

namespace {
int ensure_lanes(sbe_engine* e, int n) {
    const size_t hb = step_host_lq_offset(e) + 2 * sizeof(double);
    while ((int)e->lanes.size() < n) {
        sbe_engine::Lane ln{};
        HIPCHK(e, hipHostMalloc((void**)&ln.h_step, hb, hipHostMallocMapped));
        memset(ln.h_step, 0, hb);
        HIPCHK(e, hipHostGetDevicePointer((void**)&ln.d_step_host, ln.h_step, 0));
        HIPCHK(e, hipMalloc((void**)&ln.d_pf, (size_t)e->Gtot * e->F * sizeof(float)));
        HIPCHK(e, hipMalloc((void**)&ln.d_stamp, (size_t)e->Gtot * sizeof(uint32_t)));
        HIPCHK(e, hipMemsetAsync(ln.d_stamp, 0, (size_t)e->Gtot * sizeof(uint32_t), e->stream));
        HIPCHK(e, hipMalloc((void**)&ln.d_status, ST_WORDS * sizeof(int)));
        HIPCHK(e, hipMemsetAsync(ln.d_status, 0, ST_WORDS * sizeof(int), e->stream));
        ln.step_id = 0;
        e->lanes.push_back(ln);
    }
    return SBE_OK;
}
}


int sbe_step_batch(sbe_engine* e, int n_chains, const int32_t* cur_slots, const int32_t* cand_slots,
                   const uint8_t* clusters, const uint8_t* clusters_mask, const int32_t* rows_ptr,
                   const int32_t* changed_objects, const uint8_t* source_rows, const float* weights,
                   const uint8_t* weights_mask, double* group_logliks_out, double* mixture_out,
                   uint8_t* changed_groups_out) {
    CHECK_ENGINE(e); CHECK_PTR(e, cur_slots); CHECK_PTR(e, cand_slots); CHECK_PTR(e, rows_ptr);
    CHECK_PTR(e, group_logliks_out); CHECK_PTR(e, mixture_out);
    if (n_chains < 1 || n_chains > e->n_slots / 2) return fail(e, SBE_ERR_ARG, "n_chains=%d (1..%d: two slots per chain)", n_chains, e->n_slots / 2);
    if ((int64_t)e->Gtot * e->S * 28 > 60 * 1024) return fail(e, SBE_ERR_ARG, "sbe_step_batch: tables too large for the one-launch step (G_total=%d, S=%d)", e->Gtot, e->S);
    const int N = e->N, F = e->F, C = e->C, K = e->G[0];
    if (rows_ptr[0] != 0) return fail(e, SBE_ERR_ARG, "rows_ptr[0] must be 0");
    static const bool timing = getenv("SBE_STEP_TIMING") && atoi(getenv("SBE_STEP_TIMING")) != 0;
    using clk = std::chrono::steady_clock;
    clk::time_point tp[12]; int ntp = 0;
    auto mark = [&] { if (timing && ntp < 12) tp[ntp++] = clk::now(); };
    mark();
    {
        std::vector<uint8_t> used(e->n_slots, 0);
        for (int i = 0; i < n_chains; ++i) {
            const int a = cur_slots[i], b = cand_slots[i];
            if (a < 0 || a >= e->n_slots || b < 0 || b >= e->n_slots || a == b) return fail(e, SBE_ERR_ARG, "chain %d: bad slots (%d, %d)", i, a, b);
            if (used[a] || used[b]) return fail(e, SBE_ERR_ARG, "chain %d: slot used by another chain of the batch", i);
            used[a] = used[b] = 1;
            const int nr = rows_ptr[i + 1] - rows_ptr[i];
            if (nr < 0 || nr > e->step_max_rows) return fail(e, SBE_ERR_ARG, "chain %d: %d changed source rows (0..%d per chain in a batched step)", i, nr, e->step_max_rows);
            if (nr > 0 && (!changed_objects || !source_rows)) return fail(e, SBE_ERR_ARG, "changed_objects / source_rows missing");
            for (int k = rows_ptr[i]; k < rows_ptr[i + 1]; ++k)
                if (changed_objects[k] < 0 || changed_objects[k] >= N) return fail(e, SBE_ERR_ARG, "chain %d: object index %d out of range", i, changed_objects[k]);
            const Slot& cur = e->slots[a];
            if (!cur.groups_set || !cur.source_set || !cur.weights_set) return fail(e, SBE_ERR_STATE, "slot %d: groups / source / weights not set", a);
            { int orc = reject_overlap(e, a, "one-call step"); if (orc) return orc; }
            for (int c = 0; c < C; ++c)
                if (!cur.counts_set[c] || !e->conc_set[c]) return fail(e, SBE_ERR_STATE, "slot %d: counts / concentration of component %d not set", a, c);
        }
    }
    HIPCHK(e, hipSetDevice(e->device));
    if (e->status_pending) {
        HIPCHK(e, hipStreamSynchronize(e->stream));
        int rc = synced(e);
        if (rc) return rc;
    }
    for (int i = 0; i < n_chains; ++i)
        if (e->slots[cur_slots[i]].patterns_dirty) { int rc = upload_patterns_and_weights(e, cur_slots[i]); if (rc) return rc; }
    int rc = ensure_lanes(e, n_chains);
    if (rc) return rc;
    rc = ensure_step_pool(e);
    if (rc) return rc;
    mark();
    if ((int)e->batch_cands.size() < n_chains) e->batch_cands.resize(n_chains);
    if ((int)e->batch_moved.size() < n_chains) e->batch_moved.resize(n_chains);
    std::vector<Slot>& cds = e->batch_cands;
    std::vector<CoreInputs> ins(n_chains);
    std::vector<size_t> pay_off(n_chains + 1, 0);
    for (int i = 0; i < n_chains; ++i)
        pay_off[i + 1] = pay_off[i] + (e->sl.rows + (size_t)(rows_ptr[i + 1] - rows_ptr[i]) * F * C + 255) / 256 * 256;
    if (pay_off[n_chains] > e->batch_payload_bytes) {
        HIPCHK(e, hipStreamSynchronize(e->stream));
        if (e->h_batch_payload) { HIPCHK(e, hipHostFree(e->h_batch_payload)); e->h_batch_payload = nullptr; }
        if (e->d_batch_payload) { HIPCHK(e, hipFree(e->d_batch_payload)); e->d_batch_payload = nullptr; }
        e->batch_payload_bytes = pay_off[n_chains] + pay_off[n_chains] / 2;
        HIPCHK(e, hipHostMalloc((void**)&e->h_batch_payload, e->batch_payload_bytes, hipHostMallocDefault));
        HIPCHK(e, hipMalloc((void**)&e->d_batch_payload, e->batch_payload_bytes));
    }
    int n_parts = n_chains >= 128 ? 2 : 1;
    if (const char* env = getenv("SBE_STEP_PARTS")) n_parts = std::max(1, std::min(atoi(env), n_chains));
    const int per_part = div_up(n_chains, n_parts);
    const size_t part_cores = ((size_t)per_part * sizeof(StepCore) + 255) / 256 * 256;
    const size_t part_fins = ((size_t)per_part * sizeof(StepFinish) + 255) / 256 * 256;
    const size_t part_bytes = part_cores + part_fins + ((size_t)per_part * sizeof(int32_t) + 255) / 256 * 256;
    const size_t meta_bytes = part_bytes * n_parts;
    if (meta_bytes > e->batch_meta_bytes) {
        if (e->d_batch_meta) { HIPCHK(e, hipStreamSynchronize(e->stream)); HIPCHK(e, hipFree(e->d_batch_meta)); }
        e->batch_meta_bytes = meta_bytes + meta_bytes / 2;
        HIPCHK(e, hipMalloc((void**)&e->d_batch_meta, e->batch_meta_bytes));
    }
    std::vector<uint8_t> meta(meta_bytes);
    std::vector<int> rcs(n_chains, SBE_OK);
    std::vector<std::string> errs(n_chains);
    DoneSig batch_done{};
    for (int part = 0; part < n_parts; ++part) {
        const int i0 = part * per_part, i1 = std::min(n_chains, i0 + per_part), np = i1 - i0;
        if (np <= 0) break;
        constexpr int kCopyChunk = 16;
        const int n_copy_chunks = div_up(np, kCopyChunk);
        std::vector<std::atomic<int>> chunk_done(n_copy_chunks);
        for (auto& c : chunk_done) c.store(0, std::memory_order_relaxed);
        int next_copy = 0;
        hipError_t copy_err = hipSuccess;
        auto send_ready = [&]() {
            while (next_copy < n_copy_chunks) {
                const int c0 = i0 + next_copy * kCopyChunk, c1 = std::min(i1, c0 + kCopyChunk);
                if (chunk_done[next_copy].load(std::memory_order_acquire) < c1 - c0) break;
                const hipError_t he = hipMemcpyAsync(e->d_batch_payload + pay_off[c0], e->h_batch_payload + pay_off[c0],
                                                     pay_off[c1] - pay_off[c0], hipMemcpyHostToDevice, e->stream);
                if (he != hipSuccess) copy_err = he;
                ++next_copy;
            }
        };
        const std::function<void()> poll = send_ready;
        e->pool->run(np, [&](int j) {
            const int i = i0 + j;
            const bool regroup = clusters && (!clusters_mask || clusters_mask[i]);
            const bool reweight = weights && (!weights_mask || weights_mask[i]);
            const int r0 = rows_ptr[i], nr = rows_ptr[i + 1] - r0;
            sbe_engine::Lane lane = e->lanes[i];
            lane.h_payload = e->h_batch_payload + pay_off[i];
            lane.d_payload = e->d_batch_payload + pay_off[i];
            rcs[i] = prepare_step(e, lane, cur_slots[i], cand_slots[i], regroup ? clusters + (size_t)i * K * N : nullptr,
                                  nr ? changed_objects + r0 : nullptr, nr, nr ? source_rows + (size_t)r0 * F * C : nullptr,
                                  reweight ? weights + (size_t)i * F * C : nullptr, cds[i], ins[i], &errs[i], &e->batch_moved[i]);
            chunk_done[j / kCopyChunk].fetch_add(1, std::memory_order_release);
        }, &poll);
        send_ready();
        HIPCHK(e, copy_err);
        for (int i = i0; i < i1; ++i)
            if (rcs[i]) { (void)hipStreamSynchronize(e->stream); return fail(e, rcs[i], "chain %d: %s", i, errs[i].c_str()); }
        if (part == 0) mark();
        uint8_t* pm = meta.data() + (size_t)part * part_bytes;
        StepCore* cores = reinterpret_cast<StepCore*>(pm);
        StepFinish* fins = reinterpret_cast<StepFinish*>(pm + part_cores);
        int32_t* slot_list = reinterpret_cast<int32_t*>(pm + part_cores + part_fins);
        size_t lds = 0; int max_blocks = 0;
        for (int i = i0; i < i1; ++i) {
            size_t l = 0; int nb = 0;
            rc = build_step_core(e, e->lanes[i], cur_slots[i], cand_slots[i], ins[i], cores[i - i0], l, nb, n_chains);
            if (rc) return rc;
            lds = std::max(lds, l); max_blocks = std::max(max_blocks, nb);
            fins[i - i0] = make_step_finish_lane(e, e->lanes[i]);
            slot_list[i - i0] = cand_slots[i];
        }
        if (part == 0) mark();
        uint8_t* dm = e->d_batch_meta + (size_t)part * part_bytes;
        rc = upload(e, dm, pm, part_bytes);
        if (rc) return rc;
        if (part == 0) mark();
        k_step_core_batch<<<dim3(max_blocks, np), kBlock, lds, e->stream>>>(reinterpret_cast<const StepCore*>(dm));
        HIPCHK(e, hipGetLastError());
        if (part == 0) mark();
        for (int i = i0; i < i1; ++i) {
            commit_src_sync(e, cur_slots[i], cand_slots[i], changed_objects ? changed_objects + rows_ptr[i] : nullptr,
                            rows_ptr[i + 1] - rows_ptr[i]);
            commit_ids_sync(e, cur_slots[i], cand_slots[i], e->batch_moved[i]);
            std::swap(e->slots[cand_slots[i]], cds[i]);
        }
        if (part == 0) mark();
        MixCall mix;
        mix.n = np; mix.slots = cand_slots + i0; mix.d_slots = reinterpret_cast<const int32_t*>(dm + part_cores + part_fins);
        mix.d_fins = reinterpret_cast<const StepFinish*>(dm + part_cores); mix.done_out = part == n_parts - 1 ? &batch_done : nullptr;
        rc = launch_mixture(e, mix);
        if (rc) return rc;
    }
    mark();
    { int wrc = wait_done(e, batch_done); if (wrc) return wrc; }
    mark();
    int first_bad = SBE_OK;
    std::string first_msg;
    for (int i = 0; i < n_chains; ++i) {
        rc = read_step_results_lane(e, e->lanes[i].h_step, cand_slots[i], group_logliks_out + (size_t)i * e->Gtot, mixture_out + i,
                               changed_groups_out ? changed_groups_out + (size_t)i * e->Gtot : nullptr, "rows", e->lanes[i].d_status, i);
        if (rc && !first_bad) { first_bad = rc; first_msg = e->last_error; }
    }
    if (first_bad) return fail(e, first_bad, "%s", first_msg.c_str());
    mark();
    if (timing && ntp == 10) {
        auto us = [&](int a, int b) { return std::chrono::duration<double, std::micro>(tp[b] - tp[a]).count(); };
        fprintf(stderr, "[sbe_step_batch] %d chains (first part): checks %.1f | prepare (pool) %.1f | step cores %.1f | upload %.1f | launch core %.1f | "
                        "slot moves %.1f | mixture + reduce launches and the other parts %.1f | wait for the device %.1f | read results %.1f us\n", n_chains,
                us(0, 1), us(1, 2), us(2, 3), us(3, 4), us(4, 5), us(5, 6), us(6, 7), us(7, 8), us(8, 9));
    }
    return SBE_OK;
}

namespace {

struct DeltaPlan {
    size_t subset, sub_row, sub_gid0, patch_n, patch_gid, patch_pid, patch_tid, stale, objects, tuple_g, tuple_p, patbits, weights, rows, total;
};

inline size_t al16(size_t v) { return (v + 15) / 16 * 16; }

DeltaPlan plan_delta(const sbe_engine* e, int n_mv, int n_changed, int n_last_ids, int n_last_src, bool reweight) {
    DeltaPlan p{};
    const size_t n_sub = (size_t)n_mv + n_changed, n_patch = (size_t)n_mv + n_last_ids;
    size_t o = 0;
    p.subset = o;    o = al16(o + n_sub * 4);
    p.sub_row = o;   o = al16(o + n_sub * 2);
    p.sub_gid0 = o;  o = al16(o + n_sub * 2);
    p.patch_n = o;   o = al16(o + n_patch * 4);
    p.patch_gid = o; o = al16(o + n_patch * 2);
    p.patch_pid = o; o = al16(o + n_patch);
    p.patch_tid = o; o = al16(o + n_patch);
    p.stale = o;     o = al16(o + (size_t)n_last_src * 4);
    p.objects = o;   o = al16(o + (size_t)n_changed * 4);
    p.tuple_g = o;   o = al16(o + (size_t)kMaxTuples * kMaxComponents * 2);
    p.tuple_p = o;   o = al16(o + (size_t)kMaxTuples);
    p.patbits = o;   o = al16(o + (size_t)e->Pmax * 4);
    p.weights = o;   o = al16(o + (reweight ? (size_t)e->F * e->C * 4 : 0));
    p.rows = o;      o = al16(o + (size_t)n_changed * e->F * e->C);
    p.total = (o + 255) / 256 * 256;
    return p;
}

int prepare_step_delta(sbe_engine* e, uint8_t* h_base, const uint8_t* d_base, const DeltaPlan& L, int cur_slot, int cand_slot,
                       const int32_t* mv_objects, const int32_t* mv_cluster, int n_mv, const int32_t* changed_objects, int n_changed,
                       const uint8_t* source_rows, const float* weights, CoreInputs& in, std::vector<int32_t>& moved_out) {
    const int F = e->F, C = e->C;
    const Slot& cur = e->slots[cur_slot];
    Slot& cd = e->slots[cand_slot];
    const sbe_engine::SrcSync& irec = e->ids_sync[cand_slot];
    for (int32_t n : irec.diff) {
        cd.h_gid[n] = cur.h_gid[n]; cd.h_pid[n] = cur.h_pid[n]; cd.h_tid[n] = cur.h_tid[n]; cd.h_toff[n] = cur.h_toff[n];
    }
    cd.patterns = cur.patterns; cd.n_tuples = cur.n_tuples;
    cd.h_tuple_g = cur.h_tuple_g; cd.h_tuple_p = cur.h_tuple_p; cd.pat_cnt = cur.pat_cnt; cd.tup_cnt = cur.tup_cnt;
    cd.share_ok = cur.share_ok;
    cd.inc_ok = cur.inc_ok; cd.patterns_dirty = false;
    cd.groups_set = cur.groups_set; cd.weights_set = true; cd.source_set = cur.source_set;
    cd.counts_set = cur.counts_set;
    static thread_local std::vector<int32_t> mv;
    static thread_local std::vector<uint16_t> mv_old;
    mv.clear(); mv_old.clear();
    for (int i = 0; i < n_mv; ++i) {
        const int n = mv_objects[i];
        const uint16_t g_new = mv_cluster[i] < 0 ? kNoGroup : (uint16_t)mv_cluster[i];
        if (cd.h_gid[n] == g_new) continue;
        mv.push_back(n); mv_old.push_back(cd.h_gid[n]);
        cd.h_gid[n] = g_new;
    }
    if (!mv.empty()) {
        if (e->opt_step_derive == 1 || !update_patterns_and_tuples(e, cd, mv.data(), mv_old.data(), (int)mv.size())) return 1;
        cd.group_epoch = ++e->epoch_counter;
    } else cd.group_epoch = cur.group_epoch;
    std::fill(cd.probs_set.begin(), cd.probs_set.end(), 1);
    moved_out = mv;
    uint8_t* st = h_base;
    in = CoreInputs{};
    int32_t* sub = reinterpret_cast<int32_t*>(st + L.subset);
    int16_t* sub_row = reinterpret_cast<int16_t*>(st + L.sub_row);
    uint16_t* sub_gid0 = reinterpret_cast<uint16_t*>(st + L.sub_gid0);
    int n_subset = 0;
    {
        static thread_local std::vector<std::pair<int32_t, int32_t>> ch;
        ch.clear();
        for (int i = 0; i < n_changed; ++i) ch.emplace_back(changed_objects[i], i);
        std::sort(ch.begin(), ch.end());
        std::sort(mv.begin(), mv.end());
        size_t a = 0, b = 0;
        while (a < mv.size() || b < ch.size()) {
            int32_t n; int r = -1;
            if (b == ch.size() || (a < mv.size() && mv[a] < ch[b].first)) n = mv[a++];
            else { n = ch[b].first; r = ch[b].second; if (a < mv.size() && mv[a] == n) ++a; ++b; }
            sub[n_subset] = n; sub_row[n_subset] = (int16_t)r; sub_gid0[n_subset] = cd.h_gid[n];
            ++n_subset;
        }
    }
    int n_patch = 0;
    {
        int32_t* pn = reinterpret_cast<int32_t*>(st + L.patch_n);
        uint16_t* pg = reinterpret_cast<uint16_t*>(st + L.patch_gid);
        uint8_t* pp = st + L.patch_pid; uint8_t* pt = st + L.patch_tid;
        auto put = [&](int32_t n) { pn[n_patch] = n; pg[n_patch] = cd.h_gid[n]; pp[n_patch] = cd.h_pid[n]; pt[n_patch] = cd.h_tid[n]; ++n_patch; };
        for (int32_t n : irec.diff) put(n);
        for (int32_t n : mv) put(n);
    }
    const bool tables_changed = cd.patterns != cur.patterns || cd.h_tuple_p != cur.h_tuple_p || cd.h_tuple_g != cur.h_tuple_g;
    if (tables_changed) {
        memcpy(st + L.tuple_g, cd.h_tuple_g.data(), (size_t)kMaxTuples * kMaxComponents * 2);
        memcpy(st + L.tuple_p, cd.h_tuple_p.data(), kMaxTuples);
        memset(st + L.patbits, 0, (size_t)e->Pmax * 4);
        memcpy(st + L.patbits, cd.patterns.data(), cd.patterns.size() * 4);
        in.tuple_g = d_base + L.tuple_g; in.tuple_p = d_base + L.tuple_p; in.patbits = d_base + L.patbits;
    }
    if (weights) { memcpy(st + L.weights, weights, (size_t)F * C * 4); in.weights = d_base + L.weights; }
    if (n_changed > 0) {
        memcpy(st + L.objects, changed_objects, (size_t)n_changed * 4);
        memcpy(st + L.rows, source_rows, (size_t)n_changed * F * C);
        in.rows = d_base + L.rows;
        in.objects = reinterpret_cast<const int32_t*>(d_base + L.objects);
        in.n_changed = n_changed;
    }
    in.subset = reinterpret_cast<const int32_t*>(d_base + L.subset); in.n_subset = n_subset;
    in.sub_row = reinterpret_cast<const int16_t*>(d_base + L.sub_row);
    in.sub_gid0 = reinterpret_cast<const uint16_t*>(d_base + L.sub_gid0);
    in.patch_n = reinterpret_cast<const int32_t*>(d_base + L.patch_n);
    in.patch_gid = reinterpret_cast<const uint16_t*>(d_base + L.patch_gid);
    in.patch_pid = d_base + L.patch_pid; in.patch_tid = d_base + L.patch_tid; in.n_patch = n_patch;
    in.P = (int)cd.patterns.size();
    {
        const sbe_engine::SrcSync& rec = e->src_sync[cand_slot];
        int32_t* stale = reinterpret_cast<int32_t*>(st + L.stale);
        int ns = 0;
        for (int32_t n : rec.diff) {
            bool rewritten = false;
            for (int i = 0; i < n_changed && !rewritten; ++i) rewritten = changed_objects[i] == n;
            if (!rewritten) stale[ns++] = n;
        }
        in.full_src_copy = false;
        in.stale = reinterpret_cast<const int32_t*>(d_base + L.stale);
        in.n_stale = ns;
    }
    return 0;
}

bool sync_valid(const sbe_engine::SrcSync& rec, const sbe_engine::SrcSync& peer, int peer_slot, int cap) {
    return rec.peer == peer_slot && rec.peer_version == peer.version && rec.own_version == rec.version && (int)rec.diff.size() <= cap;
}

}

int sbe_step_batch_delta(sbe_engine* e, int n_chains, const int32_t* cur_slots, const int32_t* cand_slots,
                         const int32_t* moved_ptr, const int32_t* moved_objects, const int32_t* moved_cluster,
                         const int32_t* rows_ptr, const int32_t* changed_objects, const uint8_t* source_rows,
                         const float* weights, const uint8_t* weights_mask, double* group_logliks_out, double* mixture_out,
                         uint8_t* changed_groups_out) {
    CHECK_ENGINE(e); CHECK_PTR(e, cur_slots); CHECK_PTR(e, cand_slots); CHECK_PTR(e, moved_ptr); CHECK_PTR(e, rows_ptr);
    CHECK_PTR(e, group_logliks_out); CHECK_PTR(e, mixture_out);
    const auto t_start = std::chrono::steady_clock::now();
    std::chrono::steady_clock::time_point tq[8]; int nq = 0;
    auto markd = [&] { if (nq < 8) tq[nq++] = std::chrono::steady_clock::now(); };
    if (n_chains < 1 || n_chains > e->n_slots / 2) return fail(e, SBE_ERR_ARG, "n_chains=%d (1..%d: two slots per chain)", n_chains, e->n_slots / 2);
    if ((int64_t)e->Gtot * e->S * 28 > 60 * 1024) return fail(e, SBE_ERR_ARG, "sbe_step_batch_delta: tables too large for the one-launch step (G_total=%d, S=%d)", e->Gtot, e->S);
    const int N = e->N, F = e->F, C = e->C, K = e->G[0];
    if (rows_ptr[0] != 0 || moved_ptr[0] != 0) return fail(e, SBE_ERR_ARG, "rows_ptr[0] / moved_ptr[0] must be 0");
    {
        std::vector<uint8_t> used(e->n_slots, 0);
        std::vector<uint32_t> seen(N, 0), seen_mv(N, 0);
        for (int i = 0; i < n_chains; ++i) {
            const int a = cur_slots[i], b = cand_slots[i];
            if (a < 0 || a >= e->n_slots || b < 0 || b >= e->n_slots || a == b) return fail(e, SBE_ERR_ARG, "chain %d: bad slots (%d, %d)", i, a, b);
            if (used[a] || used[b]) return fail(e, SBE_ERR_ARG, "chain %d: slot used by another chain of the batch", i);
            used[a] = used[b] = 1;
            const int nr = rows_ptr[i + 1] - rows_ptr[i], nm = moved_ptr[i + 1] - moved_ptr[i];
            if (nr < 0 || nr > e->step_max_rows) return fail(e, SBE_ERR_ARG, "chain %d: %d changed source rows (0..%d per chain in a batched step)", i, nr, e->step_max_rows);
            if (nm < 0 || nm > N) return fail(e, SBE_ERR_ARG, "chain %d: %d moved objects", i, nm);
            if ((nr > 0 && (!changed_objects || !source_rows)) || (nm > 0 && (!moved_objects || !moved_cluster))) return fail(e, SBE_ERR_ARG, "chain %d: delta arrays missing", i);
            for (int k = rows_ptr[i]; k < rows_ptr[i + 1]; ++k) {
                const int n = changed_objects[k];
                if (n < 0 || n >= N) return fail(e, SBE_ERR_ARG, "chain %d: object index %d out of range", i, n);
                if (seen[n] == (uint32_t)(2 * i + 1)) return fail(e, SBE_ERR_ARG, "chain %d: object %d listed twice in changed_objects", i, n);
                seen[n] = (uint32_t)(2 * i + 1);
            }
            for (int k = moved_ptr[i]; k < moved_ptr[i + 1]; ++k) {
                const int n = moved_objects[k];
                if (n < 0 || n >= N) return fail(e, SBE_ERR_ARG, "chain %d: moved object index %d out of range", i, n);
                if (moved_cluster[k] < -1 || moved_cluster[k] >= K) return fail(e, SBE_ERR_ARG, "chain %d: cluster %d out of range [-1,%d)", i, moved_cluster[k], K);
                if (seen_mv[n] == (uint32_t)(i + 1)) return fail(e, SBE_ERR_ARG, "chain %d: object %d listed twice in moved_objects", i, n);
                seen_mv[n] = (uint32_t)(i + 1);
            }
            const Slot& cur = e->slots[a];
            if (!cur.groups_set || !cur.source_set || !cur.weights_set) return fail(e, SBE_ERR_STATE, "slot %d: groups / source / weights not set", a);
            { int orc = reject_overlap(e, a, "one-call step"); if (orc) return orc; }
            for (int c = 0; c < C; ++c)
                if (!cur.counts_set[c] || !e->conc_set[c]) return fail(e, SBE_ERR_STATE, "slot %d: counts / concentration of component %d not set", a, c);
        }
    }
    HIPCHK(e, hipSetDevice(e->device));
    if (e->status_pending) {
        HIPCHK(e, hipStreamSynchronize(e->stream));
        int rc = synced(e);
        if (rc) return rc;
    }
    for (int i = 0; i < n_chains; ++i)
        if (e->slots[cur_slots[i]].patterns_dirty) { int rc = upload_patterns_and_weights(e, cur_slots[i]); if (rc) return rc; }
    int rc = ensure_lanes(e, n_chains);
    if (rc) return rc;
    rc = ensure_step_pool(e);
    if (rc) return rc;
    if ((int)e->batch_moved.size() < n_chains) e->batch_moved.resize(n_chains);
    markd();
    std::vector<int> fast, slow;
    std::vector<DeltaPlan> plans(n_chains);
    std::vector<size_t> pay_off(n_chains + 1, 0);
    for (int i = 0; i < n_chains; ++i) {
        const int a = cur_slots[i], b = cand_slots[i];
        const bool ok = sync_valid(e->ids_sync[b], e->ids_sync[a], a, e->step_max_rows) &&
                        sync_valid(e->src_sync[b], e->src_sync[a], a, e->step_max_rows) &&
                        e->slots[a].inc_ok && e->slots[a].n_tuples > 0 && e->slots[b].h_gid.size() == e->slots[a].h_gid.size();
        if (ok) {
            const bool reweight = weights && (!weights_mask || weights_mask[i]);
            plans[i] = plan_delta(e, moved_ptr[i + 1] - moved_ptr[i], rows_ptr[i + 1] - rows_ptr[i], (int)e->ids_sync[b].diff.size(),
                                  (int)e->src_sync[b].diff.size(), reweight);
            pay_off[i + 1] = pay_off[i] + plans[i].total;
            fast.push_back(i);
        } else { pay_off[i + 1] = pay_off[i]; slow.push_back(i); }
    }
    auto run_classic = [&](const std::vector<int>& which, int& rc_out, std::string& msg_out) {
        rc_out = SBE_OK;
        if (which.empty()) return;
        const int ns = (int)which.size();
        std::vector<int32_t> s_cur(ns), s_cand(ns), s_ptr(ns + 1, 0), s_objs;
        std::vector<uint8_t> s_cl((size_t)ns * K * N, 0), s_rows, s_wm(ns, 0);
        std::vector<float> s_w(weights ? (size_t)ns * F * C : 0);
        for (int j = 0; j < ns; ++j) {
            const int i = which[j];
            s_cur[j] = cur_slots[i]; s_cand[j] = cand_slots[i];
            const Slot& cur = e->slots[cur_slots[i]];
            std::vector<uint16_t> ids(cur.h_gid.begin(), cur.h_gid.begin() + N);
            for (int k = moved_ptr[i]; k < moved_ptr[i + 1]; ++k) ids[moved_objects[k]] = moved_cluster[k] < 0 ? kNoGroup : (uint16_t)moved_cluster[k];
            uint8_t* cl = s_cl.data() + (size_t)j * K * N;
            for (int n = 0; n < N; ++n) if (ids[n] != kNoGroup) cl[(size_t)ids[n] * N + n] = 1;
            const int r0 = rows_ptr[i], nr = rows_ptr[i + 1] - r0;
            s_ptr[j + 1] = s_ptr[j] + nr;
            if (nr) {
                s_objs.insert(s_objs.end(), changed_objects + r0, changed_objects + r0 + nr);
                s_rows.insert(s_rows.end(), source_rows + (size_t)r0 * F * C, source_rows + (size_t)(r0 + nr) * F * C);
            }
            if (weights && (!weights_mask || weights_mask[i])) { s_wm[j] = 1; memcpy(&s_w[(size_t)j * F * C], weights + (size_t)i * F * C, (size_t)F * C * 4); }
        }
        std::vector<double> s_glh((size_t)ns * e->Gtot), s_mix(ns);
        std::vector<uint8_t> s_chg((size_t)ns * e->Gtot);
        rc_out = sbe_step_batch(e, ns, s_cur.data(), s_cand.data(), s_cl.data(), nullptr, s_ptr.data(), s_objs.empty() ? nullptr : s_objs.data(),
                                s_rows.empty() ? nullptr : s_rows.data(), weights ? s_w.data() : nullptr, weights ? s_wm.data() : nullptr,
                                s_glh.data(), s_mix.data(), s_chg.data());
        if (rc_out) { msg_out = e->last_error; return; }
        for (int j = 0; j < ns; ++j) {
            const int i = which[j];
            memcpy(group_logliks_out + (size_t)i * e->Gtot, &s_glh[(size_t)j * e->Gtot], (size_t)e->Gtot * sizeof(double));
            mixture_out[i] = s_mix[j];
            if (changed_groups_out) memcpy(changed_groups_out + (size_t)i * e->Gtot, &s_chg[(size_t)j * e->Gtot], (size_t)e->Gtot);
        }
    };
    int slow_rc = SBE_OK; std::string slow_msg;
    run_classic(slow, slow_rc, slow_msg);
    markd();
    std::vector<CoreInputs> ins(n_chains);
    std::vector<int> fb(n_chains, 0);
    const int nf = (int)fast.size();
    const size_t part_cores = ((size_t)std::max(nf, 1) * sizeof(StepCore) + 255) / 256 * 256;
    const size_t part_fins = ((size_t)std::max(nf, 1) * sizeof(StepFinish) + 255) / 256 * 256;
    const size_t meta_bytes = part_cores + part_fins + ((size_t)std::max(nf, 1) * sizeof(int32_t) + 255) / 256 * 256;
    const size_t meta_off = pay_off[n_chains];
    if (meta_off + meta_bytes > e->batch_payload_bytes) {
        HIPCHK(e, hipStreamSynchronize(e->stream));
        if (e->h_batch_payload) { HIPCHK(e, hipHostFree(e->h_batch_payload)); e->h_batch_payload = nullptr; }
        if (e->d_batch_payload) { HIPCHK(e, hipFree(e->d_batch_payload)); e->d_batch_payload = nullptr; }
        e->batch_payload_bytes = (meta_off + meta_bytes) * 3 / 2;
        HIPCHK(e, hipHostMalloc((void**)&e->h_batch_payload, e->batch_payload_bytes, hipHostMallocDefault));
        HIPCHK(e, hipMalloc((void**)&e->d_batch_payload, e->batch_payload_bytes));
    }
    if (nf > 0) {
        e->pool->run(nf, [&](int j) {
            const int i = fast[j];
            const bool reweight = weights && (!weights_mask || weights_mask[i]);
            const int r0 = rows_ptr[i], nr = rows_ptr[i + 1] - r0, m0 = moved_ptr[i], nm = moved_ptr[i + 1] - m0;
            fb[i] = prepare_step_delta(e, e->h_batch_payload + pay_off[i], e->d_batch_payload + pay_off[i], plans[i], cur_slots[i], cand_slots[i],
                                       nm ? moved_objects + m0 : nullptr, nm ? moved_cluster + m0 : nullptr, nm,
                                       nr ? changed_objects + r0 : nullptr, nr, nr ? source_rows + (size_t)r0 * F * C : nullptr,
                                       reweight ? weights + (size_t)i * F * C : nullptr, ins[i], e->batch_moved[i]);
        });
    }
    markd();
    std::vector<int> go, late;
    for (int i : fast) { if (fb[i]) { late.push_back(i); bump_ids(e, cand_slots[i]); } else go.push_back(i); }
    const int ng = (int)go.size();
    DoneSig fast_done{};
    if (ng > 0) {
        uint8_t* pm = e->h_batch_payload + meta_off;
        uint8_t* dm = e->d_batch_payload + meta_off;
        StepCore* cores = reinterpret_cast<StepCore*>(pm);
        StepFinish* fins = reinterpret_cast<StepFinish*>(pm + part_cores);
        int32_t* slot_list = reinterpret_cast<int32_t*>(pm + part_cores + part_fins);
        std::vector<int32_t> cand_go(ng);
        size_t lds = 0; int max_blocks = 0;
        for (int j = 0; j < ng; ++j) {
            const int i = go[j];
            size_t l = 0; int nb = 0;
            rc = build_step_core(e, e->lanes[i], cur_slots[i], cand_slots[i], ins[i], cores[j], l, nb, ng);
            if (rc) return rc;
            lds = std::max(lds, l); max_blocks = std::max(max_blocks, nb);
            fins[j] = make_step_finish_lane(e, e->lanes[i]);
            slot_list[j] = cand_go[j] = cand_slots[i];
        }
        HIPCHK(e, hipMemcpyAsync(e->d_batch_payload, e->h_batch_payload, meta_off + meta_bytes, hipMemcpyHostToDevice, e->stream));
        k_step_core_batch<<<dim3(max_blocks, ng), kBlock, lds, e->stream>>>(reinterpret_cast<const StepCore*>(dm));
        HIPCHK(e, hipGetLastError());
        markd();
        MixCall mix;
        mix.n = ng; mix.slots = cand_go.data(); mix.d_slots = reinterpret_cast<const int32_t*>(dm + part_cores + part_fins);
        mix.d_fins = reinterpret_cast<const StepFinish*>(dm + part_cores); mix.done_out = &fast_done;
        rc = next_timing_events(e, &mix.ev_a, &mix.ev_b);
        if (rc) return rc;
        rc = launch_mixture(e, mix);
        for (int j = 0; j < ng; ++j) {
            const int i = go[j];
            commit_src_sync(e, cur_slots[i], cand_slots[i], changed_objects ? changed_objects + rows_ptr[i] : nullptr, rows_ptr[i + 1] - rows_ptr[i]);
            commit_ids_sync(e, cur_slots[i], cand_slots[i], e->batch_moved[i]);
        }
        if (rc) return rc;
    }
    static const bool timing_d = getenv("SBE_STEP_TIMING") && atoi(getenv("SBE_STEP_TIMING")) != 0;
    const auto t_enq = std::chrono::steady_clock::now();
    { int wrc = wait_done(e, fast_done); if (wrc) return wrc; }
    if (timing_d) {
        const auto t_done = std::chrono::steady_clock::now();
        auto us = [&](std::chrono::steady_clock::time_point a, std::chrono::steady_clock::time_point b) { return std::chrono::duration<double, std::micro>(b - a).count(); };
        fprintf(stderr, "[sbe_step_batch_delta] %d chains: %d patched, %d + %d through sbe_step_batch | checks %.1f | plans %.1f | host halves (pool) %.1f | cores + launch %.1f | "
                        "mixture launches + records %.1f | wait %.1f us\n", n_chains, ng, (int)slow.size(), (int)late.size(), nq > 0 ? us(t_start, tq[0]) : 0.0,
                nq > 1 ? us(tq[0], tq[1]) : 0.0, nq > 2 ? us(tq[1], tq[2]) : 0.0, nq > 3 ? us(tq[2], tq[3]) : 0.0, nq > 3 ? us(tq[3], t_enq) : 0.0, us(t_enq, t_done));
    }
    int first_bad = slow_rc; std::string first_msg = slow_msg;
    for (int i : go) {
        rc = read_step_results_lane(e, e->lanes[i].h_step, cand_slots[i], group_logliks_out + (size_t)i * e->Gtot, mixture_out + i,
                                    changed_groups_out ? changed_groups_out + (size_t)i * e->Gtot : nullptr, "rows", e->lanes[i].d_status, i);
        if (rc && !first_bad) { first_bad = rc; first_msg = e->last_error; }
    }
    if (!late.empty()) {
        int late_rc = SBE_OK; std::string late_msg;
        run_classic(late, late_rc, late_msg);
        if (late_rc && !first_bad) { first_bad = late_rc; first_msg = late_msg; }
    }
    if (first_bad) return fail(e, first_bad, "%s", first_msg.c_str());
    return SBE_OK;
}

int sbe_step_delta(sbe_engine* e, int cur_slot, int cand_slot, const int32_t* moved_objects, const int32_t* moved_cluster, int n_moved,
                   const int32_t* changed_objects, int n_changed, const uint8_t* source_rows, const float* weights,
                   double* group_logliks_out, double* mixture_out, uint8_t* changed_groups_out) {
    CHECK_ENGINE(e); CHECK_SLOT(e, cur_slot); CHECK_SLOT(e, cand_slot);
    CHECK_PTR(e, group_logliks_out); CHECK_PTR(e, mixture_out);
    if (cur_slot == cand_slot) return fail(e, SBE_ERR_ARG, "current and candidate slot must differ");
    const int N = e->N, C = e->C, K = e->G[0];
    if (n_moved < 0 || n_moved > N || (n_moved > 0 && (!moved_objects || !moved_cluster))) return fail(e, SBE_ERR_ARG, "moved_objects / moved_cluster missing for n_moved=%d", n_moved);
    if (n_changed < 0 || (n_changed > 0 && (!changed_objects || !source_rows))) return fail(e, SBE_ERR_ARG, "changed_objects / source_rows missing for n_changed=%d", n_changed);
    bool dup = false;
    {
        static thread_local std::vector<uint32_t> stamp;
        static thread_local uint32_t epoch = 0;
        if ((int)stamp.size() < N || ++epoch == 0) { stamp.assign(N, 0); epoch = 1; }
        for (int i = 0; i < n_moved; ++i) {
            if (moved_objects[i] < 0 || moved_objects[i] >= N) return fail(e, SBE_ERR_ARG, "moved object index %d out of range", moved_objects[i]);
            if (moved_cluster[i] < -1 || moved_cluster[i] >= K) return fail(e, SBE_ERR_ARG, "cluster %d out of range [-1,%d)", moved_cluster[i], K);
            dup = dup || stamp[moved_objects[i]] == epoch;
            stamp[moved_objects[i]] = epoch;
        }
    }
    for (int i = 0; i < n_changed; ++i) {
        if (changed_objects[i] < 0 || changed_objects[i] >= N) return fail(e, SBE_ERR_ARG, "object index %d out of range", changed_objects[i]);
        for (int j = 0; j < i && !dup && n_changed <= 64; ++j) dup = changed_objects[j] == changed_objects[i];
    }
    const Slot& cur = e->slots[cur_slot];
    if (!cur.groups_set || !cur.source_set || !cur.weights_set) return fail(e, SBE_ERR_STATE, "slot %d: groups / source / weights not set", cur_slot);
    { int orc = reject_overlap(e, cur_slot, "one-call step"); if (orc) return orc; }
    for (int c = 0; c < C; ++c)
        if (!cur.counts_set[c] || !e->conc_set[c]) return fail(e, SBE_ERR_STATE, "slot %d: counts / concentration of component %d not set", cur_slot, c);
    HIPCHK(e, hipSetDevice(e->device));
    auto classic = [&]() {
        std::vector<uint16_t> ids(cur.h_gid.begin(), cur.h_gid.begin() + N);
        for (int k = 0; k < n_moved; ++k) ids[moved_objects[k]] = moved_cluster[k] < 0 ? kNoGroup : (uint16_t)moved_cluster[k];
        std::vector<uint8_t> cl((size_t)std::max(K, 1) * N, 0);
        for (int n = 0; n < N; ++n) if (ids[n] != kNoGroup) cl[(size_t)ids[n] * N + n] = 1;
        return sbe_step(e, cur_slot, cand_slot, n_moved > 0 ? cl.data() : nullptr, changed_objects, n_changed, source_rows, weights,
                        group_logliks_out, mixture_out, changed_groups_out);
    };
    const bool ok = !dup && n_changed <= std::min(e->step_max_rows, 64) && e->opt_step_form == 0 && !cur.patterns_dirty &&
                    (int64_t)e->Gtot * e->S * 28 <= 60 * 1024 &&
                    sync_valid(e->ids_sync[cand_slot], e->ids_sync[cur_slot], cur_slot, e->step_max_rows) &&
                    sync_valid(e->src_sync[cand_slot], e->src_sync[cur_slot], cur_slot, e->step_max_rows) &&
                    cur.inc_ok && cur.n_tuples > 0 && e->slots[cand_slot].h_gid.size() == cur.h_gid.size();
    if (!ok) return classic();
    const DeltaPlan plan = plan_delta(e, n_moved, n_changed, (int)e->ids_sync[cand_slot].diff.size(), (int)e->src_sync[cand_slot].diff.size(), weights != nullptr);
    if (plan.total > e->sl.total) return classic();
    if (e->status_pending) {
        HIPCHK(e, hipStreamSynchronize(e->stream));
        int rc = synced(e);
        if (rc) return rc;
    }
    CoreInputs in;
    if (prepare_step_delta(e, e->h_step_payload, e->d_step_payload, plan, cur_slot, cand_slot, moved_objects, moved_cluster, n_moved,
                           changed_objects, n_changed, source_rows, weights, in, e->step_moved)) {
        bump_ids(e, cand_slot);
        return classic();
    }
    int rc = launch_step_core(e, cur_slot, cand_slot, in);
    if (rc) return rc;
    commit_src_sync(e, cur_slot, cand_slot, changed_objects, n_changed);
    commit_ids_sync(e, cur_slot, cand_slot, e->step_moved);
    StepFinish fin = make_step_finish(e);
    DoneSig done;
    MixCall mix;
    mix.first_slot = cand_slot; mix.fin = &fin; mix.done_out = &done;
    rc = launch_mixture(e, mix);
    if (rc) return rc;
    rc = wait_done(e, done);
    if (rc) return rc;
    return read_step_results(e, cand_slot, group_logliks_out, mixture_out, changed_groups_out, "rows");
}

static int gibbs_chain_check(sbe_engine* e, int cur_slot, int cand_slot, const int32_t* objects, int n_sub, double temperature,
                             double prior_temperature) {
    if (cur_slot == cand_slot) return fail(e, SBE_ERR_ARG, "current and candidate slot must differ");
    if (n_sub < 1) return fail(e, SBE_ERR_ARG, "n_sub=%d (nothing to resample)", n_sub);
    CHECK_PTR(e, objects);
    if (!(temperature > 0.0) || !(prior_temperature > 0.0)) return fail(e, SBE_ERR_ARG, "temperatures must be positive");
    Slot& cur = e->slots[cur_slot];
    if (!cur.groups_set || !cur.source_set || !cur.weights_set) return fail(e, SBE_ERR_STATE, "slot %d: groups / source / weights not set", cur_slot);
    { int orc = reject_overlap(e, cur_slot, "one-call step"); if (orc) return orc; }
    for (int c = 0; c < e->C; ++c)
        if (!cur.counts_set[c] || !e->conc_set[c] || !cur.probs_set[c])
            return fail(e, SBE_ERR_STATE, "slot %d: counts / concentration / probability tables of component %d not set", cur_slot, c);
    return check_objects(e, objects, n_sub);
}

static int gibbs_chain_ready(sbe_engine* e, int cur_slot) {
    HIPCHK(e, hipSetDevice(e->device));
    if (e->slots[cur_slot].patterns_dirty) { int rc = upload_patterns_and_weights(e, cur_slot); if (rc) return rc; }
    if (e->status_pending) {
        HIPCHK(e, hipStreamSynchronize(e->stream));
        return synced(e);
    }
    return SBE_OK;
}

struct GibbsChainBlock { size_t ob, rb, in_bytes; const int32_t* d_obj; const double* d_z; int nblk; double* d_part[2]; };

static int gibbs_chain_stage(sbe_engine* e, const int32_t* objects, int n_sub, const double* z, size_t xb, size_t out_bytes,
                             size_t front_bytes, GibbsChainBlock* b) {
    const int64_t n_obs = (int64_t)n_sub * e->F;
    b->ob = al256((size_t)n_sub * sizeof(int32_t)); b->rb = al256((size_t)e->Np * sizeof(int16_t));
    const size_t zbytes = z ? (size_t)n_obs * sizeof(double) : 0, z_at = b->ob + b->rb + xb;
    const bool z_mapped = zbytes <= ((size_t)1 << 19);
    b->in_bytes = z_at + (z_mapped ? al256(zbytes) : 0);
    int rc = ensure_io(e, b->in_bytes + out_bytes);
    if (rc) return rc;
    memcpy(e->h_io, objects, (size_t)n_sub * sizeof(int32_t));
    int16_t* row_of = reinterpret_cast<int16_t*>(e->h_io + b->ob);
    std::fill(row_of, row_of + e->Np, (int16_t)-1);
    for (int i = 0; i < n_sub; ++i) row_of[objects[i]] = 0;
    b->d_obj = reinterpret_cast<const int32_t*>(e->d_io);
    b->nblk = div_up(n_obs, kBlock);
    const size_t qb_bytes = al256((size_t)b->nblk * sizeof(double));
    rc = ensure_scratch(e, front_bytes + 2 * qb_bytes + (z_mapped ? 0 : al256(zbytes)));
    if (rc) return rc;
    b->d_part[0] = (double*)(e->d_scratch + front_bytes);
    b->d_part[1] = (double*)(e->d_scratch + front_bytes + qb_bytes);
    b->d_z = nullptr;
    if (z && z_mapped) { memcpy(e->h_io + z_at, z, zbytes); b->d_z = reinterpret_cast<const double*>(e->d_io + z_at); }
    else if (z) {
        double* dz = (double*)(e->d_scratch + front_bytes + 2 * qb_bytes);
        rc = upload(e, dz, z, zbytes); if (rc) return rc;
        b->d_z = dz;
    }
    return SBE_OK;
}

static int gibbs_chain_run(sbe_engine* e, int cur_slot, int cand_slot, const GibbsChainBlock& b, int n_sub, double temperature,
                           double prior_temperature, int from_prior, float* d_psel_f, float* d_psel_b) {
    uint8_t* src_cand = e->d_src + (int64_t)cand_slot * e->N * e->Fp;
    bump_src(e, cand_slot);
    bump_ids(e, cand_slot);
    k_sample_source<<<b.nblk, kBlock, 0, e->stream>>>(src_post_args(e, cur_slot, b.d_obj, n_sub, temperature, prior_temperature, from_prior),
                                                      b.d_z, e->rng_seed, e->rng_draw, src_cand, d_psel_f, e->d_status, b.d_part[0]);
    if (!b.d_z) ++e->rng_draw;
    HIPCHK(e, hipGetLastError());
    Slot cd = e->slots[cur_slot];
    {
        CoreInputs in;
        in.row_of = reinterpret_cast<const int16_t*>(e->d_io + b.ob);
        in.src_new = src_cand;
        in.subset = b.d_obj; in.n_subset = n_sub;
        in.P = (int)cd.patterns.size();
        int rc = launch_step_core(e, cur_slot, cand_slot, in);
        if (rc) return rc;
    }
    std::fill(cd.probs_set.begin(), cd.probs_set.end(), 1);
    e->slots[cand_slot] = cd;
    k_source_logprob<<<b.nblk, kBlock, 0, e->stream>>>(src_post_args(e, cand_slot, b.d_obj, n_sub, temperature, prior_temperature, from_prior),
                                                       e->d_src + (int64_t)cur_slot * e->N * e->Fp, d_psel_b, e->d_status, b.d_part[1]);
    HIPCHK(e, hipGetLastError());
    return SBE_OK;
}

int sbe_gibbs_step(sbe_engine* e, int cur_slot, int cand_slot, const int32_t* objects, int n_sub, double temperature,
                   double prior_temperature, int from_prior, const double* z, double* log_q_out, double* log_q_back_out,
                   double* group_logliks_out, double* mixture_out, uint8_t* changed_groups_out) {
    CHECK_ENGINE(e); CHECK_SLOT(e, cur_slot); CHECK_SLOT(e, cand_slot);
    CHECK_PTR(e, log_q_out); CHECK_PTR(e, log_q_back_out); CHECK_PTR(e, group_logliks_out); CHECK_PTR(e, mixture_out);
    int rc = gibbs_chain_check(e, cur_slot, cand_slot, objects, n_sub, temperature, prior_temperature);
    if (rc) return rc;
    if (!sbe_gibbs_propose_supported(e))
        return fail(e, SBE_ERR_ARG, "one-call Gibbs step: tables too large for the fused table kernel (G_total=%d, S=%d)", e->Gtot, e->S);
    rc = gibbs_chain_ready(e, cur_slot);
    if (rc) return rc;
    const size_t pb = al256((size_t)n_sub * e->F * sizeof(float));
    GibbsChainBlock b;
    rc = gibbs_chain_stage(e, objects, n_sub, z, 0, 0, 2 * pb, &b);
    if (rc) return rc;
    rc = gibbs_chain_run(e, cur_slot, cand_slot, b, n_sub, temperature, prior_temperature, from_prior, (float*)e->d_scratch,
                         (float*)(e->d_scratch + pb));
    if (rc) return rc;
    StepFinish fin = make_step_finish(e);
    fin.lq_partials[0] = b.d_part[0]; fin.lq_partials[1] = b.d_part[1]; fin.lq_n[0] = fin.lq_n[1] = b.nblk;
    fin.lq_out = reinterpret_cast<double*>(e->d_step_host + step_host_lq_offset(e));
    DoneSig done;
    MixCall mix;
    mix.first_slot = cand_slot; mix.fin = &fin; mix.done_out = &done;
    rc = launch_mixture(e, mix);
    if (rc) return rc;
    rc = wait_done(e, done);
    if (rc) return rc;
    rc = read_step_results(e, cand_slot, group_logliks_out, mixture_out, changed_groups_out, "posterior rows / table rows");
    if (rc) return rc;
    const double* lq = reinterpret_cast<const double*>(e->h_step + step_host_lq_offset(e));
    *log_q_out = lq[0];
    *log_q_back_out = lq[1];
    return SBE_OK;
}

static int step_general(sbe_engine* e, int cur_slot, int cand_slot, const uint8_t* clusters, const int32_t* changed_objects,
                        int n_changed, const uint8_t* source_rows, const float* weights, double* group_logliks_out,
                        double* mixture_out, uint8_t* changed_groups_out) {
    Slot& cur = e->slots[cur_slot];
    const int saved_deferred = e->opt_deferred;
    e->opt_deferred = 1;
    auto done = [&](int rc) { e->opt_deferred = saved_deferred; return rc; };
    int rc = sbe_copy_slot(e, cand_slot, cur_slot);
    if (rc) return done(rc);
    const int N = e->N;
    std::vector<uint8_t> moved(N, 0);
    for (int i = 0; i < n_changed; ++i) moved[changed_objects[i]] = 1;
    if (clusters) {
        const int K = e->G[0];
        std::vector<uint16_t> ids(N, kNoGroup);
        char msg[320];
        if (!matrix_to_ids(clusters, K, N, 0, 0, ids.data(), msg, sizeof msg)) return done(fail(e, SBE_ERR_DATA, "%s", msg));
        for (int n = 0; n < N; ++n) if (ids[n] != cur.h_gid[n]) moved[n] = 1;
        rc = set_gid_common(e, cand_slot, 0, ids);
        if (rc) return done(rc);
    }
    if (n_changed > 0) {
        rc = sbe_set_source_rows(e, cand_slot, changed_objects, n_changed, source_rows);
        if (rc) return done(rc);
    }
    if (weights) rc = sbe_set_weights(e, cand_slot, weights);
    else if (e->slots[cand_slot].patterns_dirty) rc = upload_patterns_and_weights(e, cand_slot);
    if (rc) return done(rc);
    std::vector<int32_t> subset;
    for (int n = 0; n < N; ++n) if (moved[n]) subset.push_back(n);
    rc = sbe_update_counts(e, cand_slot, cur_slot, subset.data(), (int)subset.size(), nullptr);
    if (rc) return done(rc);
    rc = clear_status_word(e, ST_BAD_NORMALIZE);
    if (rc) return done(rc);
    k_probs<int32_t><<<div_up((int64_t)e->Gtot * e->F, 256), 256, 0, e->stream>>>(
        e->d_counts + (int64_t)cand_slot * e->table_elems(), e->d_conc, nullptr,
        e->d_probs + (int64_t)cand_slot * e->table_elems(), 0, e->Gtot, e->F, e->S, 0.0, 0.0, 1, e->d_status);
    k_tile_probs<<<div_up((int64_t)e->Gtot * e->S * e->ft * e->n_ftiles, 256), 256, 0, e->stream>>>(
        e->d_probs + (int64_t)cand_slot * e->table_elems(), e->d_probs_t + (int64_t)cand_slot * e->probs_t_elems(),
        0, e->Gtot, e->Gtot, e->F, e->S, e->ft, e->n_ftiles);
    HIPCHK(e, hipGetLastError());
    std::fill(e->slots[cand_slot].probs_set.begin(), e->slots[cand_slot].probs_set.end(), 1);
    rc = check_after(e, ST_BAD_NORMALIZE);
    if (rc) return done(rc);
    rc = enqueue_dcl(e, e->d_counts + (int64_t)cand_slot * e->table_elems(), e->d_conc, 1, 0, e->Gtot, e->d_step_pf, e->d_step_pg);
    if (rc) return done(rc);
    rc = enqueue_mixture(e, cand_slot, 1);
    if (rc) return done(rc);
    const size_t pg_bytes = (size_t)e->Gtot * sizeof(double);
    rc = ensure_pinned(e, pg_bytes + (size_t)e->Gtot);
    if (rc) return done(rc);
    HIPCHK(e, hipMemcpyAsync(e->h_pinned, e->d_step_pg, pg_bytes, hipMemcpyDeviceToHost, e->stream));
    HIPCHK(e, hipMemcpyAsync(e->h_pinned + pg_bytes, e->d_changed, (size_t)e->Gtot, hipMemcpyDeviceToHost, e->stream));
    HIPCHK(e, hipStreamSynchronize(e->stream));
    memcpy(group_logliks_out, e->h_pinned, pg_bytes);
    if (changed_groups_out) memcpy(changed_groups_out, e->h_pinned + pg_bytes, (size_t)e->Gtot);
    *mixture_out = e->h_results[cand_slot];
    return done(synced(e));
}

int sbe_gibbs_propose_supported(sbe_engine* e) {
    CHECK_ENGINE(e);
    return ((int64_t)e->Gtot * e->S * 28 <= 60 * 1024) ? 1 : 0;
}

static int gibbs_propose_impl(sbe_engine* e, int cur_slot, int cand_slot, const int32_t* objects, int n_sub, double temperature,
                              double prior_temperature, int from_prior, const double* z, uint8_t* src_new_out, float* sel_out,
                              float* sel_back_out, int32_t* touched_out, int32_t* n_touched_out, float* diff_rows_out, int follow) {
    CHECK_ENGINE(e); CHECK_SLOT(e, cur_slot); CHECK_SLOT(e, cand_slot);
    CHECK_PTR(e, src_new_out); CHECK_PTR(e, sel_out); CHECK_PTR(e, sel_back_out); CHECK_PTR(e, touched_out); CHECK_PTR(e, n_touched_out);
    CHECK_PTR(e, diff_rows_out); CHECK_PTR(e, z);
    int rc = gibbs_chain_check(e, cur_slot, cand_slot, objects, n_sub, temperature, prior_temperature);
    if (rc) return rc;
    Slot& cur = e->slots[cur_slot];
    const int N = e->N, Np = e->Np, F = e->F, C = e->C, S = e->S;
    const int64_t n_obs = (int64_t)n_sub * F, fs = (int64_t)F * S;
    std::vector<uint8_t> seen((size_t)e->Gtot, 0);
    for (int c = 0; c < C; ++c)
        for (int i = 0; i < n_sub; ++i) {
            const uint16_t gg = cur.h_gid[(size_t)c * N + objects[i]];
            if (gg != kNoGroup) seen[gg] = 1;
        }
    int n_touched = 0;
    for (int g = 0; g < e->Gtot; ++g) if (seen[g]) touched_out[n_touched++] = g;
    *n_touched_out = n_touched;
    rc = gibbs_chain_ready(e, cur_slot);
    if (rc) return rc;
    {
        const size_t t_ob = al256((size_t)n_sub * sizeof(int32_t)), t_gb = al256((size_t)C * n_sub * sizeof(int32_t));
        const size_t t_tb = al256((size_t)std::max(n_touched, 1) * sizeof(int32_t));
        const size_t t_in = t_ob + t_gb + t_tb;
        const size_t t_lds = t_in + ((size_t)e->Gtot + (size_t)n_touched * 16 * S) * sizeof(int32_t) + (size_t)n_sub * 16;
        const size_t zbytes_t = (size_t)n_obs * sizeof(double);
        const bool z_map = zbytes_t <= ((size_t)1 << 19);
        const size_t t_zb = z_map ? al256(zbytes_t) : 0;
        const size_t t_idb = al256((size_t)n_obs), t_selb = al256((size_t)n_obs * sizeof(float));
        const size_t t_rowb = al256((size_t)std::max(n_touched, 1) * fs * sizeof(float));
        const size_t t_out = t_idb + 2 * t_selb + t_rowb;
        const bool chain_possible = sbe_gibbs_propose_supported(e) == 1;
        if (e->opt_fuse_tables && t_lds <= kGuFusedLdsMax && t_out <= ((size_t)8 << 20) && (n_sub <= 128 || !chain_possible)) {
            rc = ensure_io(e, t_in + t_zb + t_out);
            if (rc) return rc;
            uint8_t* h = e->h_io;
            memcpy(h, objects, (size_t)n_sub * sizeof(int32_t));
            int32_t* gl = reinterpret_cast<int32_t*>(h + t_ob);
            for (int c = 0; c < C; ++c)
                for (int i = 0; i < n_sub; ++i) {
                    const uint16_t gg = cur.h_gid[(size_t)c * N + objects[i]];
                    gl[(size_t)c * n_sub + i] = gg == kNoGroup ? -1 : (int32_t)gg;
                }
            memcpy(h + t_ob + t_gb, touched_out, (size_t)n_touched * sizeof(int32_t));
            const double* d_zt;
            if (z_map) { memcpy(h + t_in, z, zbytes_t); d_zt = reinterpret_cast<const double*>(e->d_io + t_in); }
            else {
                rc = ensure_scratch(e, al256(zbytes_t));
                if (rc) return rc;
                int urc = upload(e, e->d_scratch, z, zbytes_t); if (urc) return urc;
                d_zt = reinterpret_cast<const double*>(e->d_scratch);
            }
            rc = clear_status_word(e, ST_BAD_NORMALIZE);
            if (rc) return rc;
            uint8_t* d_o = e->d_io + t_in + t_zb;
            GibbsTileArgs ta{};
            ta.state = e->d_state; ta.gid = e->d_gid + (int64_t)cur_slot * C * Np; ta.pid = e->d_pid + (int64_t)cur_slot * Np;
            ta.src = e->d_src + (int64_t)cur_slot * N * e->Fp; ta.probs = e->d_probs + (int64_t)cur_slot * e->table_elems();
            ta.wpat = e->d_wpat + (int64_t)cur_slot * e->Pmax * F * C; ta.counts = e->d_counts + (int64_t)cur_slot * e->table_elems();
            ta.conc = e->d_conc;
            ta.mapped_in = reinterpret_cast<const uint32_t*>(e->d_io); ta.in_words = (int)(t_in / 4);
            ta.objects_word = 0; ta.gid_word = (int)(t_ob / 4); ta.touched_word = (int)((t_ob + t_gb) / 4);
            ta.z = d_zt;
            ta.ids_out = d_o; ta.sel_out = (float*)(d_o + t_idb); ta.back_out = (float*)(d_o + t_idb + t_selb);
            ta.rows_out = (float*)(d_o + t_idb + 2 * t_selb);
            ta.n_sub = n_sub; ta.n_touched = n_touched; ta.Gtot = e->Gtot; ta.Np = Np; ta.F = F; ta.S = S; ta.C = C; ta.Fp = e->Fp;
            const double inv_t = 1.0 / temperature, inv_tp = 1.0 / prior_temperature;
            ta.inv_t = inv_t; ta.inv_tp = (float)inv_tp; ta.pow_lh = inv_t != 1.0; ta.pow_w = inv_tp != 1.0; ta.from_prior = from_prior != 0;
            ta.status = e->d_status;
            if (follow && n_touched > 0) {
                ta.follow.counts = e->d_counts + (int64_t)cur_slot * e->table_elems();
                ta.follow.probs = e->d_probs + (int64_t)cur_slot * e->table_elems();
                ta.follow.probs_t = e->d_probs_t + (int64_t)cur_slot * e->probs_t_elems();
                ta.follow.ft = e->ft;
                ta.follow.src = e->d_src + (int64_t)cur_slot * N * e->Fp;
            }
            const unsigned blocks = (unsigned)div_up(F, 16);
            const DoneSig done = next_done(e, blocks);
            k_gibbs_propose_tile<<<blocks, kTileBlock, t_lds, e->stream>>>(ta, done);
            HIPCHK(e, hipGetLastError());
            rc = sync_and_report(e, done);
            if (rc) return rc;
            const uint8_t* ho = h + t_in + t_zb;
            memcpy(src_new_out, ho, (size_t)n_obs);
            memcpy(sel_out, ho + t_idb, (size_t)n_obs * sizeof(float));
            memcpy(sel_back_out, ho + t_idb + t_selb, (size_t)n_obs * sizeof(float));
            memcpy(diff_rows_out, ho + t_idb + 2 * t_selb, (size_t)n_touched * fs * sizeof(float));
            return SBE_OK;
        }
    }
    if (!sbe_gibbs_propose_supported(e))
        return fail(e, SBE_ERR_ARG, "sbe_gibbs_propose: tables too large for the fused table kernel (G_total=%d, S=%d)", e->Gtot, e->S);
    const size_t tb = al256((size_t)std::max(n_touched, 1) * sizeof(int32_t));
    const size_t idb = al256((size_t)n_obs), selb = al256((size_t)n_obs * sizeof(float));
    const size_t rowb = al256((size_t)std::max(n_touched, 1) * fs * sizeof(float));
    const size_t out_bytes = idb + 2 * selb + rowb;
    if (out_bytes > ((size_t)8 << 20)) return fail(e, SBE_ERR_ARG, "sbe_gibbs_propose: %d objects x %d features exceed the mapped result block", n_sub, F);
    GibbsChainBlock b;
    rc = gibbs_chain_stage(e, objects, n_sub, z, tb, out_bytes, 0, &b);
    if (rc) return rc;
    const size_t in_bytes = b.in_bytes;
    uint8_t* h = e->h_io;
    memcpy(h + b.ob + b.rb, touched_out, (size_t)n_touched * sizeof(int32_t));
    uint8_t* d_ids = e->d_io + in_bytes;
    float* d_rows = (float*)(d_ids + idb + 2 * selb);
    rc = clear_status_word(e, ST_BAD_NORMALIZE);
    if (rc) return rc;
    rc = gibbs_chain_run(e, cur_slot, cand_slot, b, n_sub, temperature, prior_temperature, from_prior, (float*)(d_ids + idb),
                         (float*)(d_ids + idb + selb));
    if (rc) return rc;
    const int64_t n_el = n_obs + (int64_t)n_touched * fs;
    const unsigned blocks = (unsigned)std::min<int64_t>(div_up(n_el, 256), 256);
    const DoneSig done = next_done(e, blocks);
    k_gibbs_fetch<<<blocks, 256, 0, e->stream>>>(e->d_src + (int64_t)cand_slot * N * e->Fp, b.d_obj, n_sub, d_ids,
                                                e->d_counts + (int64_t)cur_slot * e->table_elems(),
                                                e->d_counts + (int64_t)cand_slot * e->table_elems(),
                                                reinterpret_cast<const int32_t*>(e->d_io + b.ob + b.rb), n_touched, d_rows, F, S, e->Fp, done);
    HIPCHK(e, hipGetLastError());
    rc = sync_and_report(e, done);
    if (rc) return rc;
    memcpy(src_new_out, h + in_bytes, (size_t)n_obs);
    memcpy(sel_out, h + in_bytes + idb, (size_t)n_obs * sizeof(float));
    memcpy(sel_back_out, h + in_bytes + idb + selb, (size_t)n_obs * sizeof(float));
    memcpy(diff_rows_out, h + in_bytes + idb + 2 * selb, (size_t)n_touched * fs * sizeof(float));
    if (follow && n_touched > 0) return sbe_copy_slot(e, cur_slot, cand_slot);
    return SBE_OK;
}

int sbe_gibbs_propose(sbe_engine* e, int cur_slot, int cand_slot, const int32_t* objects, int n_sub, double temperature,
                      double prior_temperature, int from_prior, const double* z, uint8_t* src_new_out, float* sel_out,
                      float* sel_back_out, int32_t* touched_out, int32_t* n_touched_out, float* diff_rows_out) {
    return gibbs_propose_impl(e, cur_slot, cand_slot, objects, n_sub, temperature, prior_temperature, from_prior, z, src_new_out, sel_out,
                              sel_back_out, touched_out, n_touched_out, diff_rows_out, 0);
}

int sbe_gibbs_propose_apply(sbe_engine* e, int cur_slot, int cand_slot, const int32_t* objects, int n_sub, double temperature,
                            double prior_temperature, int from_prior, const double* z, uint8_t* src_new_out, float* sel_out,
                            float* sel_back_out, int32_t* touched_out, int32_t* n_touched_out, float* diff_rows_out) {
    return gibbs_propose_impl(e, cur_slot, cand_slot, objects, n_sub, temperature, prior_temperature, from_prior, z, src_new_out, sel_out,
                              sel_back_out, touched_out, n_touched_out, diff_rows_out, 1);
}

}
```

Before: 76.45 million evals/s.

## Parallelize batched delta-step host work across thread pool and reuse scratch

Reworks the batched delta step's host side. Per-chain validation and result copying now run in chunks on the worker pool, and the per-call vectors are replaced by a persistent scratch object. Duplicate and stale-row checks use epoch stamps instead of quadratic scans, and slot vectors are only assigned when their contents differ. With many chains, the per-step feature tile width is also raised (and can be overridden through an environment variable). Together these aim to cut serial CPU time per batched step when thousands of chains are in flight, at the cost of more complex error ordering and a larger LDS footprint per tile block.

New measurement: 75.02 million evals/s. -1.9%, worse.

```diff
diff --git a/sbayes_amd/csrc/sbe_engine_internal.hip.h b/sbayes_amd/csrc/sbe_engine_internal.hip.h
--- a/sbayes_amd/csrc/sbe_engine_internal.hip.h
+++ b/sbayes_amd/csrc/sbe_engine_internal.hip.h
@@ -16,6 +16,7 @@
 #include <atomic>
 #include <condition_variable>
 #include <functional>
+#include <memory>
 #include <mutex>
 #include <string>
 #include <thread>
@@ -143,6 +144,7 @@
     std::vector<Slot> batch_cands;
     std::vector<std::vector<int32_t>> batch_moved;
     std::vector<int32_t> step_moved;
+    std::shared_ptr<void> delta_scratch;
     struct Pool;
     Pool* pool = nullptr;
     uint8_t* d_scratch = nullptr;  size_t scratch_bytes = 0;
diff --git a/sbayes_amd/csrc/sbe_engine_steps.hip b/sbayes_amd/csrc/sbe_engine_steps.hip
--- a/sbayes_amd/csrc/sbe_engine_steps.hip
+++ b/sbayes_amd/csrc/sbe_engine_steps.hip
@@ -1,4 +1,5 @@
 #include "sbe_engine_internal.hip.h"
+#include "sbe_step_host.h"
 
 extern "C" {
 
@@ -24,8 +25,18 @@
                             e->d_status};
 }
 
+inline int step_copy_blocks(const sbe_engine* e, uint32_t run_dwords, int n_chains) {
+    return std::max(1, (int)std::min<int64_t>(div_up(run_dwords, 1024), std::max(4, 2 * e->compute_units / std::max(1, n_chains))));
+}
+
+inline int step_tile_features(int n_chains) {
+    static const int forced = getenv("SBE_STEP_FTC") ? atoi(getenv("SBE_STEP_FTC")) : 0;
+    if (forced > 0) return forced;
+    return n_chains >= 1024 ? 2048 : 8;
+}
+
 int build_step_core(sbe_engine* e, sbe_engine::Lane& lane, int cur_slot, int cand_slot, const CoreInputs& in,
-                    StepCore& a, size_t& lds_out, int& n_blocks_out, int n_chains = 1) {
+                    StepCore& a, size_t& lds_out, int& n_blocks_out, int n_chains = 1, bool* stamps_wrapped = nullptr) {
     const int N = e->N, Np = e->Np, F = e->F, C = e->C;
     const bool regroup = in.ids_new != nullptr;
     a = StepCore{};
@@ -84,12 +95,13 @@
     a.probs_t = e->d_probs_t + (int64_t)cand_slot * e->probs_t_elems();
     a.per_feature = lane.d_pf;
     if (++lane.step_id == 0) {
-        HIPCHK(e, hipMemsetAsync(lane.d_stamp, 0, e->Gtot * sizeof(uint32_t), e->stream));
+        if (stamps_wrapped) *stamps_wrapped = true;
+        else HIPCHK(e, hipMemsetAsync(lane.d_stamp, 0, e->Gtot * sizeof(uint32_t), e->stream));
         lane.step_id = 1;
     }
     a.stamp = lane.d_stamp; a.step_id = lane.step_id;
     a.Np = Np; a.S = e->S; a.Gtot = e->Gtot; a.ft = e->ft;
-    a.ftc = (int)std::max<int64_t>(1, std::min<int64_t>(8, 2048 / ((int64_t)e->Gtot * e->S)));
+    a.ftc = (int)std::max<int64_t>(1, std::min<int64_t>(step_tile_features(n_chains), 2048 / ((int64_t)e->Gtot * e->S)));
     a.n_tile_blocks = div_up(F, a.ftc);
     a.weights = in.weights ? reinterpret_cast<const float*>(in.weights) : e->d_weights + (int64_t)cur_slot * F * C;
     a.pattern_bits = in.patbits ? reinterpret_cast<const uint32_t*>(in.patbits) : e->d_patbits + (int64_t)cur_slot * e->Pmax;
@@ -98,7 +110,7 @@
     a.P = in.P; a.Pmax = e->Pmax; a.n_weight_blocks = div_up((int64_t)in.P * F, kBlock);
     const int64_t E = (int64_t)e->Gtot * a.ftc * e->S, R = (int64_t)e->Gtot * a.ftc;
     const size_t lds = (size_t)((E * 4 + 15) / 16 * 16) + (size_t)(2 * E + R) * sizeof(double);
-    a.n_copy_blocks = std::max(1, (int)std::min<int64_t>(div_up(run, 1024), std::max(4, 2 * e->compute_units / std::max(1, n_chains))));
+    a.n_copy_blocks = step_copy_blocks(e, run, n_chains);
     lds_out = lds;
     n_blocks_out = a.n_tile_blocks + a.n_weight_blocks + a.n_copy_blocks;
     return SBE_OK;
@@ -132,10 +144,20 @@
 }
 StepFinish make_step_finish(sbe_engine* e) { return make_step_finish_lane(e, lane0(e)); }
 
+inline bool step_results_flagged(const sbe_engine* e, const uint8_t* h_step) {
+    const int* hst = reinterpret_cast<const int*>(h_step + (size_t)e->Gtot * sizeof(double));
+    return hst[ST_BAD_NORMALIZE] || hst[ST_MULTI_SOURCE];
+}
+inline void copy_step_results(const sbe_engine* e, const uint8_t* h_step, int cand_slot, double* group_logliks_out, double* mixture_out,
+                              uint8_t* changed_groups_out) {
+    memcpy(group_logliks_out, h_step, (size_t)e->Gtot * sizeof(double));
+    if (changed_groups_out) memcpy(changed_groups_out, h_step + (size_t)e->Gtot * sizeof(double) + ST_WORDS * sizeof(int), (size_t)e->Gtot);
+    *mixture_out = e->h_results[cand_slot];
+}
 int read_step_results_lane(sbe_engine* e, const uint8_t* h_step, int cand_slot, double* group_logliks_out, double* mixture_out,
                       uint8_t* changed_groups_out, const char* bad_norm_what, int* d_status = nullptr, int chain = -1) {
     const int* hst = reinterpret_cast<const int*>(h_step + (size_t)e->Gtot * sizeof(double));
-    if (hst[ST_BAD_NORMALIZE] || hst[ST_MULTI_SOURCE]) {
+    if (step_results_flagged(e, h_step)) {
         const int bad_norm = hst[ST_BAD_NORMALIZE], multi_src = hst[ST_MULTI_SOURCE];
         (void)hipMemsetAsync((d_status ? d_status : e->d_status) + ST_BAD_NORMALIZE, 0, 2 * sizeof(int), e->stream);
         if (!d_status || d_status == e->d_status) e->h_flag[ST_BAD_NORMALIZE] = e->h_flag[ST_MULTI_SOURCE] = 0;
@@ -144,9 +166,7 @@
         if (bad_norm) return fail(e, SBE_ERR_DATA, "%snormalize: %d %s have a non-positive sum (sbayes/util.py:1006 assert)", who, bad_norm, bad_norm_what);
         return fail(e, SBE_ERR_DATA, "%ssource is not one-hot over components in %d observations", who, multi_src);
     }
-    memcpy(group_logliks_out, h_step, (size_t)e->Gtot * sizeof(double));
-    if (changed_groups_out) memcpy(changed_groups_out, h_step + (size_t)e->Gtot * sizeof(double) + ST_WORDS * sizeof(int), (size_t)e->Gtot);
-    *mixture_out = e->h_results[cand_slot];
+    copy_step_results(e, h_step, cand_slot, group_logliks_out, mixture_out, changed_groups_out);
     return SBE_OK;
 }
 int read_step_results(sbe_engine* e, int cand_slot, double* group_logliks_out, double* mixture_out,
@@ -561,37 +581,16 @@
 
 namespace {
 
-struct DeltaPlan {
-    size_t subset, sub_row, sub_gid0, patch_n, patch_gid, patch_pid, patch_tid, stale, objects, tuple_g, tuple_p, patbits, weights, rows, total;
-};
-
-inline size_t al16(size_t v) { return (v + 15) / 16 * 16; }
-
+using sbe_host::DeltaPlan;
+
+inline sbe_host::DeltaDims delta_dims(const sbe_engine* e) { return sbe_host::DeltaDims{e->N, e->G[0], e->F, e->C, e->Pmax, e->step_max_rows}; }
 DeltaPlan plan_delta(const sbe_engine* e, int n_mv, int n_changed, int n_last_ids, int n_last_src, bool reweight) {
-    DeltaPlan p{};
-    const size_t n_sub = (size_t)n_mv + n_changed, n_patch = (size_t)n_mv + n_last_ids;
-    size_t o = 0;
-    p.subset = o;    o = al16(o + n_sub * 4);
-    p.sub_row = o;   o = al16(o + n_sub * 2);
-    p.sub_gid0 = o;  o = al16(o + n_sub * 2);
-    p.patch_n = o;   o = al16(o + n_patch * 4);
-    p.patch_gid = o; o = al16(o + n_patch * 2);
-    p.patch_pid = o; o = al16(o + n_patch);
-    p.patch_tid = o; o = al16(o + n_patch);
-    p.stale = o;     o = al16(o + (size_t)n_last_src * 4);
-    p.objects = o;   o = al16(o + (size_t)n_changed * 4);
-    p.tuple_g = o;   o = al16(o + (size_t)kMaxTuples * kMaxComponents * 2);
-    p.tuple_p = o;   o = al16(o + (size_t)kMaxTuples);
-    p.patbits = o;   o = al16(o + (size_t)e->Pmax * 4);
-    p.weights = o;   o = al16(o + (reweight ? (size_t)e->F * e->C * 4 : 0));
-    p.rows = o;      o = al16(o + (size_t)n_changed * e->F * e->C);
-    p.total = (o + 255) / 256 * 256;
-    return p;
+    return sbe_host::plan_delta(delta_dims(e), n_mv, n_changed, n_last_ids, n_last_src, reweight);
 }
 
 int prepare_step_delta(sbe_engine* e, uint8_t* h_base, const uint8_t* d_base, const DeltaPlan& L, int cur_slot, int cand_slot,
                        const int32_t* mv_objects, const int32_t* mv_cluster, int n_mv, const int32_t* changed_objects, int n_changed,
-                       const uint8_t* source_rows, const float* weights, CoreInputs& in, std::vector<int32_t>& moved_out) {
+                       const uint8_t* source_rows, const float* weights, CoreInputs& in, std::vector<int32_t>& moved_out, uint64_t new_epoch) {
     const int F = e->F, C = e->C;
     const Slot& cur = e->slots[cur_slot];
     Slot& cd = e->slots[cand_slot];
@@ -599,8 +598,10 @@
     for (int32_t n : irec.diff) {
         cd.h_gid[n] = cur.h_gid[n]; cd.h_pid[n] = cur.h_pid[n]; cd.h_tid[n] = cur.h_tid[n]; cd.h_toff[n] = cur.h_toff[n];
     }
-    cd.patterns = cur.patterns; cd.n_tuples = cur.n_tuples;
-    cd.h_tuple_g = cur.h_tuple_g; cd.h_tuple_p = cur.h_tuple_p; cd.pat_cnt = cur.pat_cnt; cd.tup_cnt = cur.tup_cnt;
+    using sbe_host::assign_if_differs;
+    assign_if_differs(cd.patterns, cur.patterns); cd.n_tuples = cur.n_tuples;
+    assign_if_differs(cd.h_tuple_g, cur.h_tuple_g); assign_if_differs(cd.h_tuple_p, cur.h_tuple_p);
+    assign_if_differs(cd.pat_cnt, cur.pat_cnt); assign_if_differs(cd.tup_cnt, cur.tup_cnt);
     cd.share_ok = cur.share_ok;
     cd.inc_ok = cur.inc_ok; cd.patterns_dirty = false;
     cd.groups_set = cur.groups_set; cd.weights_set = true; cd.source_set = cur.source_set;
@@ -617,7 +618,7 @@
     }
     if (!mv.empty()) {
         if (e->opt_step_derive == 1 || !update_patterns_and_tuples(e, cd, mv.data(), mv_old.data(), (int)mv.size())) return 1;
-        cd.group_epoch = ++e->epoch_counter;
+        cd.group_epoch = new_epoch;
     } else cd.group_epoch = cur.group_epoch;
     std::fill(cd.probs_set.begin(), cd.probs_set.end(), 1);
     moved_out = mv;
@@ -677,12 +678,7 @@
     {
         const sbe_engine::SrcSync& rec = e->src_sync[cand_slot];
         int32_t* stale = reinterpret_cast<int32_t*>(st + L.stale);
-        int ns = 0;
-        for (int32_t n : rec.diff) {
-            bool rewritten = false;
-            for (int i = 0; i < n_changed && !rewritten; ++i) rewritten = changed_objects[i] == n;
-            if (!rewritten) stale[ns++] = n;
-        }
+        const int ns = sbe_host::stale_rows(rec.diff.data(), (int)rec.diff.size(), changed_objects, n_changed, e->N, sbe_host::worker_stamp(), stale);
         in.full_src_copy = false;
         in.stale = reinterpret_cast<const int32_t*>(d_base + L.stale);
         in.n_stale = ns;
@@ -692,6 +688,44 @@
 
 bool sync_valid(const sbe_engine::SrcSync& rec, const sbe_engine::SrcSync& peer, int peer_slot, int cap) {
     return rec.peer == peer_slot && rec.peer_version == peer.version && rec.own_version == rec.version && (int)rec.diff.size() <= cap;
+}
+
+struct DeltaScratch {
+    std::vector<uint32_t> slot_stamp; uint32_t slot_epoch = 0;
+    std::vector<uint8_t> state;
+    std::vector<uint32_t> total;
+    std::vector<size_t> pay_off;
+    std::vector<int> fast, slow, go, late;
+    std::vector<int> n_blocks;
+    std::vector<size_t> lds;
+    std::vector<int32_t> cand_go;
+};
+enum : uint8_t { kChainBad = 1, kChainPatched = 2, kChainDirty = 4, kChainLate = 8, kChainWrapped = 16 };
+
+DeltaScratch* delta_scratch(sbe_engine* e) {
+    if (!e->delta_scratch) e->delta_scratch = std::make_shared<DeltaScratch>();
+    return static_cast<DeltaScratch*>(e->delta_scratch.get());
+}
+
+int check_delta_chain(const sbe_engine* e, const sbe_host::DeltaDims& dims, int i, int cur_slot, const int32_t* rows_ptr, const int32_t* changed_objects,
+                      const uint8_t* source_rows, const int32_t* moved_ptr, const int32_t* moved_objects, const int32_t* moved_cluster,
+                      char* msg, size_t cap) {
+    const int r0 = rows_ptr[i], m0 = moved_ptr[i];
+    if (!sbe_host::check_chain_lists(dims, i, rows_ptr[i + 1] - r0, changed_objects ? changed_objects + r0 : nullptr, source_rows != nullptr,
+                                     moved_ptr[i + 1] - m0, moved_objects ? moved_objects + m0 : nullptr, moved_cluster ? moved_cluster + m0 : nullptr,
+                                     sbe_host::worker_stamp(), msg, cap))
+        return SBE_ERR_ARG;
+    const Slot& cur = e->slots[cur_slot];
+    if (!cur.groups_set || !cur.source_set || !cur.weights_set) { snprintf(msg, cap, "slot %d: groups / source / weights not set", cur_slot); return SBE_ERR_STATE; }
+    if (cur.overlap_mask) {
+        char ov[320];
+        overlap_message(ov, sizeof ov, cur.ov_obj, cur.ov_g1, cur.ov_g2, cur.ov_comp);
+        snprintf(msg, cap, "%s (slot %d, %s)", ov, cur_slot, "one-call step");
+        return SBE_ERR_DATA;
+    }
+    for (int c = 0; c < e->C; ++c)
+        if (!cur.counts_set[c] || !e->conc_set[c]) { snprintf(msg, cap, "slot %d: counts / concentration of component %d not set", cur_slot, c); return SBE_ERR_STATE; }
+    return SBE_OK;
 }
 
 }
@@ -710,68 +744,85 @@
     if ((int64_t)e->Gtot * e->S * 28 > 60 * 1024) return fail(e, SBE_ERR_ARG, "sbe_step_batch_delta: tables too large for the one-launch step (G_total=%d, S=%d)", e->Gtot, e->S);
     const int N = e->N, F = e->F, C = e->C, K = e->G[0];
     if (rows_ptr[0] != 0 || moved_ptr[0] != 0) return fail(e, SBE_ERR_ARG, "rows_ptr[0] / moved_ptr[0] must be 0");
-    {
-        std::vector<uint8_t> used(e->n_slots, 0);
-        std::vector<uint32_t> seen(N, 0), seen_mv(N, 0);
-        for (int i = 0; i < n_chains; ++i) {
-            const int a = cur_slots[i], b = cand_slots[i];
-            if (a < 0 || a >= e->n_slots || b < 0 || b >= e->n_slots || a == b) return fail(e, SBE_ERR_ARG, "chain %d: bad slots (%d, %d)", i, a, b);
-            if (used[a] || used[b]) return fail(e, SBE_ERR_ARG, "chain %d: slot used by another chain of the batch", i);
-            used[a] = used[b] = 1;
-            const int nr = rows_ptr[i + 1] - rows_ptr[i], nm = moved_ptr[i + 1] - moved_ptr[i];
-            if (nr < 0 || nr > e->step_max_rows) return fail(e, SBE_ERR_ARG, "chain %d: %d changed source rows (0..%d per chain in a batched step)", i, nr, e->step_max_rows);
-            if (nm < 0 || nm > N) return fail(e, SBE_ERR_ARG, "chain %d: %d moved objects", i, nm);
-            if ((nr > 0 && (!changed_objects || !source_rows)) || (nm > 0 && (!moved_objects || !moved_cluster))) return fail(e, SBE_ERR_ARG, "chain %d: delta arrays missing", i);
-            for (int k = rows_ptr[i]; k < rows_ptr[i + 1]; ++k) {
-                const int n = changed_objects[k];
-                if (n < 0 || n >= N) return fail(e, SBE_ERR_ARG, "chain %d: object index %d out of range", i, n);
-                if (seen[n] == (uint32_t)(2 * i + 1)) return fail(e, SBE_ERR_ARG, "chain %d: object %d listed twice in changed_objects", i, n);
-                seen[n] = (uint32_t)(2 * i + 1);
-            }
-            for (int k = moved_ptr[i]; k < moved_ptr[i + 1]; ++k) {
-                const int n = moved_objects[k];
-                if (n < 0 || n >= N) return fail(e, SBE_ERR_ARG, "chain %d: moved object index %d out of range", i, n);
-                if (moved_cluster[k] < -1 || moved_cluster[k] >= K) return fail(e, SBE_ERR_ARG, "chain %d: cluster %d out of range [-1,%d)", i, moved_cluster[k], K);
-                if (seen_mv[n] == (uint32_t)(i + 1)) return fail(e, SBE_ERR_ARG, "chain %d: object %d listed twice in moved_objects", i, n);
-                seen_mv[n] = (uint32_t)(i + 1);
-            }
-            const Slot& cur = e->slots[a];
-            if (!cur.groups_set || !cur.source_set || !cur.weights_set) return fail(e, SBE_ERR_STATE, "slot %d: groups / source / weights not set", a);
-            { int orc = reject_overlap(e, a, "one-call step"); if (orc) return orc; }
-            for (int c = 0; c < C; ++c)
-                if (!cur.counts_set[c] || !e->conc_set[c]) return fail(e, SBE_ERR_STATE, "slot %d: counts / concentration of component %d not set", a, c);
-        }
-    }
-    HIPCHK(e, hipSetDevice(e->device));
-    if (e->status_pending) {
-        HIPCHK(e, hipStreamSynchronize(e->stream));
-        int rc = synced(e);
-        if (rc) return rc;
-    }
-    for (int i = 0; i < n_chains; ++i)
-        if (e->slots[cur_slots[i]].patterns_dirty) { int rc = upload_patterns_and_weights(e, cur_slots[i]); if (rc) return rc; }
-    int rc = ensure_lanes(e, n_chains);
-    if (rc) return rc;
-    rc = ensure_step_pool(e);
-    if (rc) return rc;
-    if ((int)e->batch_moved.size() < n_chains) e->batch_moved.resize(n_chains);
-    markd();
-    std::vector<int> fast, slow;
-    std::vector<DeltaPlan> plans(n_chains);
-    std::vector<size_t> pay_off(n_chains + 1, 0);
+    DeltaScratch& sc = *delta_scratch(e);
+    using sbe_host::grow;
+    grow(sc.state, (size_t)n_chains); grow(sc.total, (size_t)n_chains); grow(sc.pay_off, (size_t)n_chains + 1);
+    grow(sc.n_blocks, (size_t)n_chains); grow(sc.lds, (size_t)n_chains); grow(sc.cand_go, (size_t)n_chains);
+    grow(sc.slot_stamp, (size_t)e->n_slots);
+    const sbe_host::DeltaDims dims = delta_dims(e);
+    int rc = ensure_step_pool(e);
+    if (rc) return rc;
+    const int n_threads = (int)e->pool->workers.size() + 1;
+    const int light_chunk = sbe_host::chunk_chains(n_chains, n_threads, 64);
+    int first_serial = n_chains, serial_kind = 0;
+    if (++sc.slot_epoch == 0) { std::fill(sc.slot_stamp.begin(), sc.slot_stamp.end(), 0u); sc.slot_epoch = 1; }
     for (int i = 0; i < n_chains; ++i) {
+        const int a = cur_slots[i], b = cand_slots[i];
+        if (a < 0 || a >= e->n_slots || b < 0 || b >= e->n_slots || a == b) { first_serial = i; serial_kind = 1; break; }
+        if (sc.slot_stamp[a] == sc.slot_epoch || sc.slot_stamp[b] == sc.slot_epoch) { first_serial = i; serial_kind = 2; break; }
+        sc.slot_stamp[a] = sc.slot_stamp[b] = sc.slot_epoch;
+        if (rows_ptr[i + 1] < rows_ptr[i] || moved_ptr[i + 1] < moved_ptr[i]) { first_serial = i; serial_kind = 3; break; }
+    }
+    std::atomic<int> n_bad{0}, n_dirty{0};
+    auto classify = [&](int i) {
         const int a = cur_slots[i], b = cand_slots[i];
         const bool ok = sync_valid(e->ids_sync[b], e->ids_sync[a], a, e->step_max_rows) &&
                         sync_valid(e->src_sync[b], e->src_sync[a], a, e->step_max_rows) &&
                         e->slots[a].inc_ok && e->slots[a].n_tuples > 0 && e->slots[b].h_gid.size() == e->slots[a].h_gid.size();
+        uint8_t st = e->slots[a].patterns_dirty ? kChainDirty : 0;
+        sc.total[i] = 0;
         if (ok) {
             const bool reweight = weights && (!weights_mask || weights_mask[i]);
-            plans[i] = plan_delta(e, moved_ptr[i + 1] - moved_ptr[i], rows_ptr[i + 1] - rows_ptr[i], (int)e->ids_sync[b].diff.size(),
-                                  (int)e->src_sync[b].diff.size(), reweight);
-            pay_off[i + 1] = pay_off[i] + plans[i].total;
-            fast.push_back(i);
-        } else { pay_off[i + 1] = pay_off[i]; slow.push_back(i); }
-    }
+            sc.total[i] = (uint32_t)plan_delta(e, moved_ptr[i + 1] - moved_ptr[i], rows_ptr[i + 1] - rows_ptr[i], (int)e->ids_sync[b].diff.size(),
+                                               (int)e->src_sync[b].diff.size(), reweight).total;
+            st |= kChainPatched;
+        }
+        sc.state[i] = st;
+    };
+    sbe_host::for_chunks(e->pool, first_serial, light_chunk, [&](int i0, int i1) {
+        char msg[512];
+        int bad = 0, dirty = 0;
+        for (int i = i0; i < i1; ++i) {
+            if (check_delta_chain(e, dims, i, cur_slots[i], rows_ptr, changed_objects, source_rows, moved_ptr, moved_objects, moved_cluster, msg, sizeof msg)) {
+                sc.state[i] = kChainBad; ++bad;
+                continue;
+            }
+            classify(i);
+            dirty += (sc.state[i] & kChainDirty) != 0;
+        }
+        if (bad) n_bad.fetch_add(bad, std::memory_order_relaxed);
+        if (dirty) n_dirty.fetch_add(dirty, std::memory_order_relaxed);
+    });
+    if (n_bad.load(std::memory_order_relaxed) > 0 || first_serial < n_chains) {
+        int i = 0;
+        while (i < first_serial && !(sc.state[i] & kChainBad)) ++i;
+        if (i == first_serial && serial_kind == 1) return fail(e, SBE_ERR_ARG, "chain %d: bad slots (%d, %d)", i, cur_slots[i], cand_slots[i]);
+        if (i == first_serial && serial_kind == 2) return fail(e, SBE_ERR_ARG, "chain %d: slot used by another chain of the batch", i);
+        char msg[512] = "";
+        const int code = check_delta_chain(e, dims, i, cur_slots[i], rows_ptr, changed_objects, source_rows, moved_ptr, moved_objects, moved_cluster, msg, sizeof msg);
+        return fail(e, code ? code : SBE_ERR_ARG, "%s", msg);
+    }
+    HIPCHK(e, hipSetDevice(e->device));
+    if (e->status_pending) {
+        HIPCHK(e, hipStreamSynchronize(e->stream));
+        int src = synced(e);
+        if (src) return src;
+    }
+    if (n_dirty.load(std::memory_order_relaxed) > 0)
+        for (int i = 0; i < n_chains; ++i)
+            if (sc.state[i] & kChainDirty) {
+                if (e->slots[cur_slots[i]].patterns_dirty) { rc = upload_patterns_and_weights(e, cur_slots[i]); if (rc) return rc; }
+                classify(i);
+            }
+    rc = ensure_lanes(e, n_chains);
+    if (rc) return rc;
+    if ((int)e->batch_moved.size() < n_chains) e->batch_moved.resize(n_chains);
+    markd();
+    std::vector<int>& fast = sc.fast; std::vector<int>& slow = sc.slow;
+    fast.clear(); slow.clear();
+    size_t* pay_off = sc.pay_off.data();
+    sbe_host::payload_offsets(sc.total.data(), n_chains, pay_off);
+    for (int i = 0; i < n_chains; ++i) ((sc.state[i] & kChainPatched) ? fast : slow).push_back(i);
     auto run_classic = [&](const std::vector<int>& which, int& rc_out, std::string& msg_out) {
         rc_out = SBE_OK;
         if (which.empty()) return;
@@ -811,8 +862,6 @@
     int slow_rc = SBE_OK; std::string slow_msg;
     run_classic(slow, slow_rc, slow_msg);
     markd();
-    std::vector<CoreInputs> ins(n_chains);
-    std::vector<int> fb(n_chains, 0);
     const int nf = (int)fast.size();
     const size_t part_cores = ((size_t)std::max(nf, 1) * sizeof(StepCore) + 255) / 256 * 256;
     const size_t part_fins = ((size_t)std::max(nf, 1) * sizeof(StepFinish) + 255) / 256 * 256;
@@ -826,76 +875,117 @@
         HIPCHK(e, hipHostMalloc((void**)&e->h_batch_payload, e->batch_payload_bytes, hipHostMallocDefault));
         HIPCHK(e, hipMalloc((void**)&e->d_batch_payload, e->batch_payload_bytes));
     }
-    if (nf > 0) {
-        e->pool->run(nf, [&](int j) {
-            const int i = fast[j];
+    uint8_t* pm = e->h_batch_payload + meta_off;
+    uint8_t* dm = e->d_batch_payload + meta_off;
+    StepCore* cores = reinterpret_cast<StepCore*>(pm);
+    StepFinish* fins = reinterpret_cast<StepFinish*>(pm + part_cores);
+    int32_t* slot_list = reinterpret_cast<int32_t*>(pm + part_cores + part_fins);
+    std::atomic<int> n_late{0}, n_wrapped{0};
+    sbe_host::for_chunks(e->pool, nf, sbe_host::chunk_chains(nf, n_threads, 1), [&](int j0, int j1) {
+        uint64_t epoch = e->epoch_counter.fetch_add((uint64_t)(j1 - j0));
+        int late_here = 0, wrapped_here = 0;
+        for (int j = j0; j < j1; ++j) {
+            const int i = fast[j], a = cur_slots[i], b = cand_slots[i];
             const bool reweight = weights && (!weights_mask || weights_mask[i]);
             const int r0 = rows_ptr[i], nr = rows_ptr[i + 1] - r0, m0 = moved_ptr[i], nm = moved_ptr[i + 1] - m0;
-            fb[i] = prepare_step_delta(e, e->h_batch_payload + pay_off[i], e->d_batch_payload + pay_off[i], plans[i], cur_slots[i], cand_slots[i],
-                                       nm ? moved_objects + m0 : nullptr, nm ? moved_cluster + m0 : nullptr, nm,
-                                       nr ? changed_objects + r0 : nullptr, nr, nr ? source_rows + (size_t)r0 * F * C : nullptr,
-                                       reweight ? weights + (size_t)i * F * C : nullptr, ins[i], e->batch_moved[i]);
-        });
-    }
+            const DeltaPlan plan = plan_delta(e, nm, nr, (int)e->ids_sync[b].diff.size(), (int)e->src_sync[b].diff.size(), reweight);
+            CoreInputs in;
+            if (prepare_step_delta(e, e->h_batch_payload + pay_off[i], e->d_batch_payload + pay_off[i], plan, a, b,
+                                   nm ? moved_objects + m0 : nullptr, nm ? moved_cluster + m0 : nullptr, nm,
+                                   nr ? changed_objects + r0 : nullptr, nr, nr ? source_rows + (size_t)r0 * F * C : nullptr,
+                                   reweight ? weights + (size_t)i * F * C : nullptr, in, e->batch_moved[i], ++epoch)) {
+                sc.state[i] |= kChainLate; ++late_here;
+                continue;
+            }
+            bool wrapped = false;
+            (void)build_step_core(e, e->lanes[i], a, b, in, cores[j], sc.lds[j], sc.n_blocks[j], nf, &wrapped);
+            if (wrapped) { sc.state[i] |= kChainWrapped; ++wrapped_here; }
+            fins[j] = make_step_finish_lane(e, e->lanes[i]);
+            slot_list[j] = sc.cand_go[j] = b;
+        }
+        if (late_here) n_late.fetch_add(late_here, std::memory_order_relaxed);
+        if (wrapped_here) n_wrapped.fetch_add(wrapped_here, std::memory_order_relaxed);
+    });
     markd();
-    std::vector<int> go, late;
-    for (int i : fast) { if (fb[i]) { late.push_back(i); bump_ids(e, cand_slots[i]); } else go.push_back(i); }
+    std::vector<int>& go = sc.go; std::vector<int>& late = sc.late;
+    go.clear(); late.clear();
+    if (n_late.load(std::memory_order_relaxed) == 0) go.assign(fast.begin(), fast.end());
+    else {
+        for (int j = 0; j < nf; ++j) {
+            const int i = fast[j];
+            if (sc.state[i] & kChainLate) { late.push_back(i); bump_ids(e, cand_slots[i]); continue; }
+            const int jj = (int)go.size();
+            if (jj != j) { cores[jj] = cores[j]; fins[jj] = fins[j]; slot_list[jj] = sc.cand_go[jj] = slot_list[j]; sc.lds[jj] = sc.lds[j]; }
+            go.push_back(i);
+        }
+        for (int jj = 0; jj < (int)go.size(); ++jj) {
+            StepCore& a = cores[jj];
+            a.n_copy_blocks = step_copy_blocks(e, a.cs.n > 0 ? a.cs.end[a.cs.n - 1] : 0u, (int)go.size());
+            sc.n_blocks[jj] = a.n_tile_blocks + a.n_weight_blocks + a.n_copy_blocks;
+        }
+    }
     const int ng = (int)go.size();
     DoneSig fast_done{};
     if (ng > 0) {
-        uint8_t* pm = e->h_batch_payload + meta_off;
-        uint8_t* dm = e->d_batch_payload + meta_off;
-        StepCore* cores = reinterpret_cast<StepCore*>(pm);
-        StepFinish* fins = reinterpret_cast<StepFinish*>(pm + part_cores);
-        int32_t* slot_list = reinterpret_cast<int32_t*>(pm + part_cores + part_fins);
-        std::vector<int32_t> cand_go(ng);
         size_t lds = 0; int max_blocks = 0;
-        for (int j = 0; j < ng; ++j) {
-            const int i = go[j];
-            size_t l = 0; int nb = 0;
-            rc = build_step_core(e, e->lanes[i], cur_slots[i], cand_slots[i], ins[i], cores[j], l, nb, ng);
-            if (rc) return rc;
-            lds = std::max(lds, l); max_blocks = std::max(max_blocks, nb);
-            fins[j] = make_step_finish_lane(e, e->lanes[i]);
-            slot_list[j] = cand_go[j] = cand_slots[i];
-        }
+        for (int j = 0; j < ng; ++j) { lds = std::max(lds, sc.lds[j]); max_blocks = std::max(max_blocks, sc.n_blocks[j]); }
+        if (n_wrapped.load(std::memory_order_relaxed) > 0)
+            for (int i : go)
+                if (sc.state[i] & kChainWrapped) HIPCHK(e, hipMemsetAsync(e->lanes[i].d_stamp, 0, e->Gtot * sizeof(uint32_t), e->stream));
         HIPCHK(e, hipMemcpyAsync(e->d_batch_payload, e->h_batch_payload, meta_off + meta_bytes, hipMemcpyHostToDevice, e->stream));
         k_step_core_batch<<<dim3(max_blocks, ng), kBlock, lds, e->stream>>>(reinterpret_cast<const StepCore*>(dm));
         HIPCHK(e, hipGetLastError());
         markd();
         MixCall mix;
-        mix.n = ng; mix.slots = cand_go.data(); mix.d_slots = reinterpret_cast<const int32_t*>(dm + part_cores + part_fins);
+        mix.n = ng; mix.slots = sc.cand_go.data(); mix.d_slots = reinterpret_cast<const int32_t*>(dm + part_cores + part_fins);
         mix.d_fins = reinterpret_cast<const StepFinish*>(dm + part_cores); mix.done_out = &fast_done;
         rc = next_timing_events(e, &mix.ev_a, &mix.ev_b);
         if (rc) return rc;
         rc = launch_mixture(e, mix);
-        for (int j = 0; j < ng; ++j) {
-            const int i = go[j];
-            commit_src_sync(e, cur_slots[i], cand_slots[i], changed_objects ? changed_objects + rows_ptr[i] : nullptr, rows_ptr[i + 1] - rows_ptr[i]);
-            commit_ids_sync(e, cur_slots[i], cand_slots[i], e->batch_moved[i]);
-        }
+        sbe_host::for_chunks(e->pool, ng, light_chunk, [&](int j0, int j1) {
+            for (int j = j0; j < j1; ++j) {
+                const int i = go[j];
+                commit_src_sync(e, cur_slots[i], cand_slots[i], changed_objects ? changed_objects + rows_ptr[i] : nullptr, rows_ptr[i + 1] - rows_ptr[i]);
+                commit_ids_sync(e, cur_slots[i], cand_slots[i], e->batch_moved[i]);
+            }
+        });
         if (rc) return rc;
     }
     static const bool timing_d = getenv("SBE_STEP_TIMING") && atoi(getenv("SBE_STEP_TIMING")) != 0;
     const auto t_enq = std::chrono::steady_clock::now();
     { int wrc = wait_done(e, fast_done); if (wrc) return wrc; }
-    if (timing_d) {
-        const auto t_done = std::chrono::steady_clock::now();
-        auto us = [&](std::chrono::steady_clock::time_point a, std::chrono::steady_clock::time_point b) { return std::chrono::duration<double, std::micro>(b - a).count(); };
-        fprintf(stderr, "[sbe_step_batch_delta] %d chains: %d patched, %d + %d through sbe_step_batch | checks %.1f | plans %.1f | host halves (pool) %.1f | cores + launch %.1f | "
-                        "mixture launches + records %.1f | wait %.1f us\n", n_chains, ng, (int)slow.size(), (int)late.size(), nq > 0 ? us(t_start, tq[0]) : 0.0,
-                nq > 1 ? us(tq[0], tq[1]) : 0.0, nq > 2 ? us(tq[1], tq[2]) : 0.0, nq > 3 ? us(tq[2], tq[3]) : 0.0, nq > 3 ? us(tq[3], t_enq) : 0.0, us(t_enq, t_done));
-    }
+    const auto t_done = std::chrono::steady_clock::now();
+    std::atomic<int> n_flagged{0};
+    sbe_host::for_chunks(e->pool, ng, light_chunk, [&](int j0, int j1) {
+        int flagged = 0;
+        for (int j = j0; j < j1; ++j) {
+            const int i = go[j];
+            if (step_results_flagged(e, e->lanes[i].h_step)) { sc.state[i] |= kChainBad; ++flagged; continue; }
+            copy_step_results(e, e->lanes[i].h_step, cand_slots[i], group_logliks_out + (size_t)i * e->Gtot, mixture_out + i,
+                              changed_groups_out ? changed_groups_out + (size_t)i * e->Gtot : nullptr);
+        }
+        if (flagged) n_flagged.fetch_add(flagged, std::memory_order_relaxed);
+    });
     int first_bad = slow_rc; std::string first_msg = slow_msg;
-    for (int i : go) {
-        rc = read_step_results_lane(e, e->lanes[i].h_step, cand_slots[i], group_logliks_out + (size_t)i * e->Gtot, mixture_out + i,
-                                    changed_groups_out ? changed_groups_out + (size_t)i * e->Gtot : nullptr, "rows", e->lanes[i].d_status, i);
-        if (rc && !first_bad) { first_bad = rc; first_msg = e->last_error; }
-    }
+    if (n_flagged.load(std::memory_order_relaxed) > 0)
+        for (int i : go) {
+            if (!(sc.state[i] & kChainBad)) continue;
+            rc = read_step_results_lane(e, e->lanes[i].h_step, cand_slots[i], group_logliks_out + (size_t)i * e->Gtot, mixture_out + i,
+                                        changed_groups_out ? changed_groups_out + (size_t)i * e->Gtot : nullptr, "rows", e->lanes[i].d_status, i);
+            if (rc && !first_bad) { first_bad = rc; first_msg = e->last_error; }
+        }
     if (!late.empty()) {
         int late_rc = SBE_OK; std::string late_msg;
         run_classic(late, late_rc, late_msg);
         if (late_rc && !first_bad) { first_bad = late_rc; first_msg = late_msg; }
+    }
+    if (timing_d) {
+        const auto t_out = std::chrono::steady_clock::now();
+        auto us = [&](std::chrono::steady_clock::time_point a, std::chrono::steady_clock::time_point b) { return std::chrono::duration<double, std::micro>(b - a).count(); };
+        fprintf(stderr, "[sbe_step_batch_delta] %d chains: %d patched, %d + %d through sbe_step_batch | checks %.1f | plans %.1f | host halves (pool) %.1f | cores + launch %.1f | "
+                        "mixture launches + records %.1f | wait %.1f | results out (+ late chains) %.1f us\n", n_chains, ng, (int)slow.size(), (int)late.size(),
+                nq > 0 ? us(t_start, tq[0]) : 0.0, nq > 1 ? us(tq[0], tq[1]) : 0.0, nq > 2 ? us(tq[1], tq[2]) : 0.0, nq > 3 ? us(tq[2], tq[3]) : 0.0,
+                nq > 3 ? us(tq[3], t_enq) : 0.0, us(t_enq, t_done), us(t_done, t_out));
     }
     if (first_bad) return fail(e, first_bad, "%s", first_msg.c_str());
     return SBE_OK;
@@ -955,7 +1045,7 @@
     }
     CoreInputs in;
     if (prepare_step_delta(e, e->h_step_payload, e->d_step_payload, plan, cur_slot, cand_slot, moved_objects, moved_cluster, n_moved,
-                           changed_objects, n_changed, source_rows, weights, in, e->step_moved)) {
+                           changed_objects, n_changed, source_rows, weights, in, e->step_moved, ++e->epoch_counter)) {
         bump_ids(e, cand_slot);
         return classic();
     }
diff --git a/sbayes_amd/csrc/sbe_step_host.h b/sbayes_amd/csrc/sbe_step_host.h
--- /dev/null
+++ b/sbayes_amd/csrc/sbe_step_host.h
@@ -0,0 +1,109 @@
+#pragma once
+
+#include "sbe_mixture_plan.h"
+#include "sbe_pool.h"
+
+#include <algorithm>
+#include <cstddef>
+#include <cstdint>
+#include <cstdio>
+#include <vector>
+
+namespace sbe_host {
+
+struct DeltaDims { int N, K, F, C, Pmax, max_rows; };
+
+struct DeltaPlan {
+    size_t subset, sub_row, sub_gid0, patch_n, patch_gid, patch_pid, patch_tid, stale, objects, tuple_g, tuple_p, patbits, weights, rows, total;
+};
+
+inline size_t al16(size_t v) { return (v + 15) / 16 * 16; }
+
+inline DeltaPlan plan_delta(const DeltaDims& d, int n_mv, int n_changed, int n_last_ids, int n_last_src, bool reweight) {
+    DeltaPlan p{};
+    const size_t n_sub = (size_t)n_mv + n_changed, n_patch = (size_t)n_mv + n_last_ids;
+    size_t o = 0;
+    p.subset = o;    o = al16(o + n_sub * 4);
+    p.sub_row = o;   o = al16(o + n_sub * 2);
+    p.sub_gid0 = o;  o = al16(o + n_sub * 2);
+    p.patch_n = o;   o = al16(o + n_patch * 4);
+    p.patch_gid = o; o = al16(o + n_patch * 2);
+    p.patch_pid = o; o = al16(o + n_patch);
+    p.patch_tid = o; o = al16(o + n_patch);
+    p.stale = o;     o = al16(o + (size_t)n_last_src * 4);
+    p.objects = o;   o = al16(o + (size_t)n_changed * 4);
+    p.tuple_g = o;   o = al16(o + (size_t)sbe::kMaxTuples * sbe::kMaxComponents * 2);
+    p.tuple_p = o;   o = al16(o + (size_t)sbe::kMaxTuples);
+    p.patbits = o;   o = al16(o + (size_t)d.Pmax * 4);
+    p.weights = o;   o = al16(o + (reweight ? (size_t)d.F * d.C * 4 : 0));
+    p.rows = o;      o = al16(o + (size_t)n_changed * d.F * d.C);
+    p.total = (o + 255) / 256 * 256;
+    return p;
+}
+
+inline size_t payload_offsets(const uint32_t* total, int n, size_t* off) {
+    size_t o = 0;
+    for (int i = 0; i < n; ++i) { off[i] = o; o += total[i]; }
+    off[n] = o;
+    return o;
+}
+
+struct ObjectStamp {
+    std::vector<uint32_t> stamp;
+    uint32_t epoch = 0;
+    void begin(int N) { if ((int)stamp.size() < N || ++epoch == 0) { stamp.assign((size_t)N, 0); epoch = 1; } }
+    bool mark(int n) { const bool was = stamp[n] == epoch; stamp[n] = epoch; return was; }
+    bool marked(int n) const { return stamp[n] == epoch; }
+};
+inline ObjectStamp& worker_stamp() { static thread_local ObjectStamp s; return s; }
+
+inline bool check_chain_lists(const DeltaDims& d, int chain, int nr, const int32_t* changed, bool have_rows, int nm, const int32_t* mv_objects,
+                              const int32_t* mv_cluster, ObjectStamp& st, char* msg, size_t cap) {
+    if (nr < 0 || nr > d.max_rows) { snprintf(msg, cap, "chain %d: %d changed source rows (0..%d per chain in a batched step)", chain, nr, d.max_rows); return false; }
+    if (nm < 0 || nm > d.N) { snprintf(msg, cap, "chain %d: %d moved objects", chain, nm); return false; }
+    if ((nr > 0 && (!changed || !have_rows)) || (nm > 0 && (!mv_objects || !mv_cluster))) { snprintf(msg, cap, "chain %d: delta arrays missing", chain); return false; }
+    st.begin(d.N);
+    for (int k = 0; k < nr; ++k) {
+        const int n = changed[k];
+        if (n < 0 || n >= d.N) { snprintf(msg, cap, "chain %d: object index %d out of range", chain, n); return false; }
+        if (st.mark(n)) { snprintf(msg, cap, "chain %d: object %d listed twice in changed_objects", chain, n); return false; }
+    }
+    st.begin(d.N);
+    for (int k = 0; k < nm; ++k) {
+        const int n = mv_objects[k];
+        if (n < 0 || n >= d.N) { snprintf(msg, cap, "chain %d: moved object index %d out of range", chain, n); return false; }
+        if (mv_cluster[k] < -1 || mv_cluster[k] >= d.K) { snprintf(msg, cap, "chain %d: cluster %d out of range [-1,%d)", chain, mv_cluster[k], d.K); return false; }
+        if (st.mark(n)) { snprintf(msg, cap, "chain %d: object %d listed twice in moved_objects", chain, n); return false; }
+    }
+    return true;
+}
+
+inline int stale_rows(const int32_t* diff, int n_diff, const int32_t* changed, int n_changed, int N, ObjectStamp& st, int32_t* out) {
+    if (n_changed == 0) { std::copy(diff, diff + n_diff, out); return n_diff; }
+    st.begin(N);
+    for (int i = 0; i < n_changed; ++i) st.mark(changed[i]);
+    int ns = 0;
+    for (int i = 0; i < n_diff; ++i) if (!st.marked(diff[i])) out[ns++] = diff[i];
+    return ns;
+}
+
+inline int chunk_chains(int n, int n_threads, int min_chunk) {
+    const int per = n / std::max(1, 4 * n_threads);
+    return std::max(std::max(1, min_chunk), std::min(64, per));
+}
+
+template <class Fn>
+inline void for_chunks(StepPool* pool, int n, int chunk, Fn fn) {
+    if (n <= 0) return;
+    if (!pool || n <= chunk) { fn(0, n); return; }
+    const int n_chunks = (n + chunk - 1) / chunk;
+    pool->run(n_chunks, [&](int c) { fn(c * chunk, std::min(n, (c + 1) * chunk)); });
+}
+
+template <class V>
+inline void assign_if_differs(V& dst, const V& src) { if (dst != src) dst = src; }
+
+template <class T>
+inline void grow(std::vector<T>& v, size_t n) { if (v.size() < n) v.resize(std::max(n, v.size() * 2)); }
+
+}
```
